# mit-han-lab/TinyChatEngine

Measured on AMD Instinct MI355X. Metric: decode tokens/s (W4A16 linears of one token, M=1) + GEMV GB/s vs HBM roofline, higher is better.
Workload: dtype int4 weights x fp16 activations, fp32 accumulate; 1 GPU; W4A16 decode GEMV M=1, llama3-8b (true shapes, model.h:83): 32 blocks x [qkv [4096, 1024, 1024], o 4096, gate/up 14336, down] + lm_head 128256, group 128; parallelism=single GPU, issue=one hipGraph replay per token (129 launches in stream order)

## Files before the change

include/tce_matmul.h:

```cpp
#ifndef TCE_MATMUL_H
#define TCE_MATMUL_H

#include <stddef.h>
#include <stdint.h>

#ifdef __cplusplus
extern "C" {
#endif

#define TCE_API __attribute__((visibility("default")))

#define TCE_VERSION 113

#define TCE_OK 0
#define TCE_ERR_BAD_ARG (-1)
#define TCE_ERR_UNSUPPORTED_GROUP (-2)
#define TCE_ERR_UNSUPPORTED_SHAPE (-3)
#define TCE_ERR_HIP (-4)
#define TCE_ERR_UNSUPPORTED_KIND (-5)
#define TCE_ERR_RCCL (-6)

#define TCE_W4A16_GEMV_MAX_M 8

typedef struct tce_w4a16_desc {
// ... 103 lines not shown
                                                int v_scale_log2, void *stream);
TCE_API int tce_attention_prefill_paged_fp8(const void *qkv, int ld_qkv, void *k_pool, void *v_pool, const int32_t *block_table, int table_rows, int table_stride,
                                            int page_keys, int num_pages, const void *cos_table, const void *sin_table, int causal, void *out, int ld_out, void *workspace,
                                            int heads, int kv_heads, int head_dim, const tce_prefill_segment *segments, int num_segments, int total_rows,
                                            unsigned short alpha_half_bits, int k_scale_log2, int v_scale_log2, void *stream);
TCE_API int tce_kv_pages_scatter_fp8(const void *k_src, const void *v_src, void *k_pool, void *v_pool, const int32_t *table_row, int table_stride, int page_keys,
                                     int num_pages, int kv_heads, int head_dim, int src_max_keys, int key0, int nkeys, int k_scale_log2, int v_scale_log2, void *stream);
TCE_API int tce_kv_pages_gather_fp8(const void *k_pool, const void *v_pool, void *k_dst, void *v_dst, const int32_t *table_row, int table_stride, int page_keys,
                                    int num_pages, int kv_heads, int head_dim, int dst_max_keys, int key0, int nkeys, int k_scale_log2, int v_scale_log2, void *stream);

#define TCE_SPEC_MAX_ROWS 8
TCE_API int tce_attention_decode_step_paged_rows_f16(const void *qkv, void *k_pool, void *v_pool, const int32_t *block_table, int table_stride, int page_keys, int num_pages,
                                                     const void *cos_table, const void *sin_table, void *out, void *workspace, int batch, int rows_per_seq, int heads,
                                                     int kv_heads, int head_dim, const int32_t *pos_device, int pos_bound, unsigned short alpha_half_bits, void *stream);
TCE_API int tce_attention_decode_step_paged_rows_fp8(const void *qkv, void *k_pool, void *v_pool, const int32_t *block_table, int table_stride, int page_keys, int num_pages,
                                                     const void *cos_table, const void *sin_table, void *out, void *workspace, int batch, int rows_per_seq, int heads,
                                                     int kv_heads, int head_dim, const int32_t *pos_device, int pos_bound, unsigned short alpha_half_bits, int k_scale_log2,
                                                     int v_scale_log2, void *stream);

typedef struct tce_sample_row {
    float temp;
    int32_t top_k;
    float top_p;
    float repeat_penalty;
    float alpha_frequency, alpha_presence;
    int32_t repeat_last_n;
    int32_t max_new;
    uint32_t seed_lo, seed_hi;
    uint32_t generated;
    uint32_t ring_pushed;
    int32_t ring[64];
} tce_sample_row;
typedef struct tce_sample_debug {
    int32_t n, k;
    float u;
    int32_t choice;
    int32_t ids[256];
    float logit[256], p[256], final_p[256];
} tce_sample_debug;
typedef struct tce_sample_call {
    const void *logits;
    int32_t ld, vocab, batch, top_k_bound;
    tce_sample_row *rows;
    int32_t *pos_device;
    int32_t pos_bound, log_stride;
    int32_t *next_token;
    int32_t *out_log;
    const float *uniform_override;
    tce_sample_debug *debug;
    void *workspace;
    int32_t stop_ids[4];
    int32_t n_stop, mirostat;
    float tfs_z, typical_p;
} tce_sample_call;
TCE_API size_t tce_sample_workspace_bytes(int batch, int vocab);
TCE_API int tce_sample_f16(const tce_sample_call *call, void *stream);
typedef struct tce_sample_verify_call {
    tce_sample_call s;
    int32_t rows_per_seq, hist_stride;
    const int32_t *row_token, *row_pos;
    int32_t *history;
    int32_t *emitted;
} tce_sample_verify_call;
TCE_API size_t tce_sample_verify_workspace_bytes(int batch, int rows_per_seq, int vocab);
TCE_API int tce_sample_verify_f16(const tce_sample_verify_call *call, void *stream);
TCE_API int tce_draft_ngram(const int32_t *history, const int32_t *script, int hist_stride, const int32_t *pos_device, int pos_bound, int batch, int rows_per_seq, int ngram,
                            int32_t *row_token, int32_t *row_pos, void *stream);
TCE_API int tce_embed_rows_f16(const void *table, int vocab, int hidden, const int32_t *token, void *out, int batch, const int32_t *pos_device, int pos_bound,
                               void *workspace, void *stream);
TCE_API int tce_prefetch(const void *ptr, long long bytes, int workgroups, void *stream);
TCE_API int tce_add_half(const void *a, const void *b, void *c, long long n, void *stream);
TCE_API int tce_rmsnorm_half(const void *x, const float *gamma, void *out, int m, int n, float eps, void *stream);
TCE_API int tce_w4a16_forward_group_rmsnorm(const tce_w4a16_desc *descs, int count, const float *gamma, float eps, void *stream);
TCE_API int tce_silu_mul_half(void *a, const void *b, long long n, void *stream);

TCE_API int tce_w4a16_check_zero_point_8(const void *zeros, long long n_words);
TCE_API int tce_w4a16_check_zero_point_8_async(const void *zeros, long long n_words, int *verdict, void *stream);

TCE_API size_t tce_w4a16_prepack_bytes(int N, int K, int group_size);
TCE_API size_t tce_w4a16_gemm_scratch_bytes(void);
TCE_API int tce_w4a16_gemm_scratch_faults(const void *scratch, void *stream, uint32_t *faults);
TCE_API int tce_w4a16_prepack(const tce_w4a16_desc *d, void *packed, void *stream);

#define TCE_MAX_GROUP 4
TCE_API int tce_w4a16_forward_group(const tce_w4a16_desc *descs, int count, void *stream);
#define TCE_MAX_INDEPENDENT 8
TCE_API int tce_w4a16_forward_independent(const tce_w4a16_desc *descs, int count, int *launches, void *stream);
TCE_API int tce_w4a16_describe_independent(const tce_w4a16_desc *descs, int count, char *buf, int buf_len);

TCE_API int tce_w4a16_awq_fp16acc(int M, int N, int K, int group_size, const void *A, const void *qweight,
                                  const void *scales, void *C, void *stream);
TCE_API size_t tce_w4a16_awq_workspace_bytes(int N, int K, int group_size);
TCE_API int tce_w4a16_gemm_awq(int M, int N, int K, int group_size, const void *A, const void *qweight,
                               const void *scales, void *C, void *workspace, int repack, void *stream);

#define TCE_BIAS_NONE 0
#define TCE_BIAS_INT8 1
#define TCE_BIAS_FP32 2
#define TCE_OUT_INT8 0
#define TCE_OUT_FP32 1

typedef struct tce_w8a8_desc {
    int32_t M, N, K;
    int32_t batch;
    const void *A;
    const void *B;
    const void *bias;
    void *C;
    int64_t strideA, strideB, strideC;
    float alpha, beta;
    int32_t q_min, q_max;
    int32_t bias_kind, out_kind;
    int32_t b_per_row;
    int32_t accumulate;
    int32_t lda, ldb, ldc;
    int32_t reserved2;
} tce_w8a8_desc;

TCE_API int tce_w8a8_matmul(const tce_w8a8_desc *d, void *stream);
typedef struct tce_w8a8_desc_v2 {
    uint32_t struct_size;
    uint32_t reserved0;
    tce_w8a8_desc desc;
    void *scratch;
} tce_w8a8_desc_v2;
TCE_API int tce_w8a8_matmul_v2(const tce_w8a8_desc_v2 *d, void *stream);
TCE_API size_t tce_w8a8_scratch_bytes(void);

TCE_API int tce_opt_softmax_q(const float *scores, const float *mask, void *probs, int heads, int sq, int tgz, int ld_probs, void *stream);
TCE_API int tce_opt_kv_append(const void *k, const void *v, void *k_cache, void *vt_cache, int heads, int hd, int sq, int pos, int max_keys, void *stream);
TCE_API int tce_opt_attention_decode(const void *q, const void *k_new, const void *v_new, void *k_cache, void *vt_cache, const float *mask, void *out, int heads,
                                     int head_dim, int m, int pos, int max_keys, int ld, float alpha_qk, float alpha_pv, void *stream);

TCE_API int tce_layernorm_q(const float *x, const float *weight, const float *bias, void *out, int m, int n, void *stream);

TCE_API int tce_layernorm_q_w8a8_group(const float *x, const float *ln_weight, const float *ln_bias, int m, int k, const tce_w8a8_desc *linears,
                                       int count, void *ln_out, void *stream);

typedef struct tce_plan tce_plan;
TCE_API int tce_plan_create(const tce_w4a16_desc *descs, const int32_t *group_sizes, int n_launches, tce_plan **out);
#define TCE_PLAN_CHAINED 1
#define TCE_PLAN_TAGGED 2
#define TCE_PLAN_OVERLAPPED 4
#define TCE_PLAN_TUNED 8
#define TCE_PLAN_INDEPENDENT 16
TCE_API int tce_plan_create_ex(const tce_w4a16_desc *descs, const int32_t *group_sizes, int n_launches, int flags, tce_plan **out);
TCE_API int tce_plan_is_chained(const tce_plan *plan);
TCE_API int tce_plan_geometry(const tce_plan *plan, int *rows, int *depth, int *waves, int *workgroups);
TCE_API int tce_plan_launch_geometry(const tce_plan *plan, int launch, int *rows, int *waves_n, int *waves_k, int *depth);
TCE_API int tce_plan_status(tce_plan *plan);
TCE_API int tce_plan_launch(tce_plan *plan, void *stream);
TCE_API int tce_plan_n_launches(const tce_plan *plan);
TCE_API void tce_plan_destroy(tce_plan *plan);

typedef struct tce_comm tce_comm;
#define TCE_COMM_HANDLE_BYTES 64
#define TCE_COMM_MAX_RANKS 8
TCE_API int tce_w4a16_shard(const tce_w4a16_desc *full, int rank, int world, tce_w4a16_desc *shard);
TCE_API int tce_comm_create(int rank, int world, int max_vector_elems, int slots, tce_comm **out);
TCE_API int tce_comm_export(tce_comm *comm, void *handle_out );
TCE_API int tce_comm_connect(tce_comm *comm, const void *handles );
TCE_API int tce_comm_connect_local(tce_comm *comm, tce_comm *const *all_ranks );
TCE_API int tce_allgather_f16(tce_comm *comm, int slot, const void *src_slice, void *dst_full, int n_total, void *stream);
TCE_API int tce_w4a16_forward_independent_gather(const tce_w4a16_desc *descs, int count, int gathered, tce_comm *comm, int slot, void *dst_full, int *launches, void *stream);
#define TCE_RCCL_ID_BYTES 128
TCE_API int tce_comm_rccl_unique_id(void *id_out );
// ... 33 lines not shown
```

tinychatengine_amd/capi.py:

```python
from __future__ import annotations

import ctypes as C
import os

_PKG = os.path.dirname(os.path.abspath(__file__))
LIB_PATH = os.environ.get("TCE_LIB_PATH") or os.path.join(_PKG, "lib", "libtce_hip.so")

TCE_OK = 0
TCE_ERR_BAD_ARG = -1
TCE_ERR_UNSUPPORTED_GROUP = -2
TCE_ERR_UNSUPPORTED_SHAPE = -3
TCE_ERR_HIP = -4
TCE_ERR_UNSUPPORTED_KIND = -5
TCE_W4A16_GEMV_MAX_M = 8
TCE_MAX_GROUP = 4
TCE_W4_FORCE_GEMV = 1
TCE_W4_FORCE_GEMM = 2
TCE_W4_SILU_MUL_PAIRS = 8
TCE_W4_ADD_TO_C = 16
TCE_PLAN_CHAINED = 1
TCE_PLAN_TAGGED = 2
TCE_ABI_VERSION = 113
TCE_PLAN_OVERLAPPED = 4
TCE_PLAN_TUNED = 8
TCE_PLAN_INDEPENDENT = 16
TCE_W4_ZERO_POINT_IS_8 = 4
TCE_BIAS_NONE, TCE_BIAS_INT8, TCE_BIAS_FP32 = 0, 1, 2
TCE_OUT_INT8, TCE_OUT_FP32 = 0, 1

EXPORTS = [
    "tce_w4a16_forward", "tce_w4a16_residual_rmsnorm_workspace_bytes", "tce_w4a16_forward_residual_rmsnorm", "tce_w4a16_prepack_bytes", "tce_w4a16_prepack", "tce_w4a16_gemm_scratch_bytes", "tce_w4a16_gemm_scratch_faults", "tce_w4a16_describe_dispatch", "tce_w8a8_describe_dispatch", "tce_reset_last_error", "tce_bmm_f16t", "tce_rope_half", "tce_softmax_half", "tce_attention_decode_f16", "tce_attention_decode_workspace_bytes", "tce_attention_decode_describe", "tce_attention_decode_step_f16", "tce_attention_decode_step_gqa_f16", "tce_attention_decode_describe_gqa", "tce_attention_decode_step_pos_f16", "tce_attention_decode_batch_workspace_bytes", "tce_attention_decode_describe_batch", "tce_attention_decode_step_batch_f16", "tce_kv_pages_pool_bytes", "tce_attention_decode_describe_paged", "tce_attention_decode_step_paged_f16", "tce_kv_pages_scatter_f16", "tce_kv_pages_gather_f16", "tce_kv_block_table_check", "tce_attention_prefill_f16", "tce_attention_prefill_workspace_bytes", "tce_attention_prefill_paged_workspace_bytes", "tce_attention_prefill_paged_f16", "tce_attention_prefill_describe_paged", "tce_kv_pages_pool_bytes_fp8", "tce_attention_decode_step_paged_fp8", "tce_attention_prefill_paged_fp8", "tce_kv_pages_scatter_fp8", "tce_kv_pages_gather_fp8", "tce_sample_workspace_bytes", "tce_sample_f16", "tce_embed_rows_f16", "tce_attention_decode_step_paged_rows_f16", "tce_attention_decode_step_paged_rows_fp8", "tce_sample_verify_workspace_bytes", "tce_sample_verify_f16", "tce_draft_ngram", "tce_opt_attention_decode", "tce_prefetch", "tce_add_half", "tce_silu_mul_half", "tce_rmsnorm_half", "tce_w4a16_forward_group_rmsnorm", "tce_w4a16_forward_group", "tce_w4a16_forward_independent", "tce_w4a16_describe_independent", "tce_w4a16_forward_independent_gather", "tce_w4a16_check_zero_point_8", "tce_w4a16_awq_fp16acc", "tce_w4a16_awq_workspace_bytes",
    "tce_w4a16_gemm_awq", "tce_w4a16_shard", "tce_comm_create", "tce_comm_export", "tce_comm_connect", "tce_comm_connect_local", "tce_allgather_f16", "tce_comm_rccl_unique_id", "tce_comm_rccl_init", "tce_allgather_rows_workspace_bytes", "tce_allgather_rows_f16", "tce_comm_status", "tce_comm_set_timeout_ms", "tce_comm_reset", "tce_comm_device", "tce_comm_destroy", "tce_w8a8_matmul", "tce_opt_softmax_q", "tce_opt_kv_append", "tce_layernorm_q", "tce_layernorm_q_w8a8_group", "tce_plan_create", "tce_plan_create_ex", "tce_plan_is_chained", "tce_plan_geometry", "tce_plan_status", "tce_plan_launch_geometry", "tce_plan_launch", "tce_plan_n_launches",
    "tce_w4a16_forward_v2", "tce_w8a8_matmul_v2", "tce_w8a8_scratch_bytes", "tce_attention_decode_step_deferred_f16", "tce_w4a16_forward_deferred_attention", "tce_plan_destroy", "tce_version", "tce_last_error", "tce_build_info", "tce_w4a16_set_gemv_config", "tce_w4a16_set_gemv_i8",
    "tce_w4a16_set_gemm_config", "tce_w4a16_algorithmic_bytes", "tce_w4a16_gemv_variant", "tce_w4a16_gemm_variant",
    "tce_w4a16_set_debug_mode", "tce_attention_set_tuning", "tce_w8a8_set_tuning", "tce_w4a16_set_debug_buffer", "tce_w4a16_check_zero_point_8_async", "tce_host_alloc", "tce_host_free", "tce_malloc", "tce_free", "tce_memcpy", "tce_synchronize", "tce_device_count",
]


class W4A16Desc(C.Structure):
    _fields_ = [
        ("M", C.c_int32), ("N", C.c_int32), ("K", C.c_int32), ("group_size", C.c_int32),
        ("A", C.c_void_p), ("qweight", C.c_void_p), ("scales", C.c_void_p), ("zeros", C.c_void_p), ("C", C.c_void_p),
        ("lda", C.c_int32), ("ldc", C.c_int32), ("scales_stride", C.c_int32), ("zeros_stride", C.c_int32),
        ("flags", C.c_int32), ("reserved", C.c_int32),
        ("rmsnorm_gamma", C.c_void_p), ("rmsnorm_eps", C.c_float), ("reserved2", C.c_int32),
        ("prepacked", C.c_void_p), ("scratch", C.c_void_p),
    ]


class W8A8Desc(C.Structure):
    _fields_ = [
        ("M", C.c_int32), ("N", C.c_int32), ("K", C.c_int32), ("batch", C.c_int32),
        ("A", C.c_void_p), ("B", C.c_void_p), ("bias", C.c_void_p), ("C", C.c_void_p),
        ("strideA", C.c_int64), ("strideB", C.c_int64), ("strideC", C.c_int64),
        ("alpha", C.c_float), ("beta", C.c_float), ("q_min", C.c_int32), ("q_max", C.c_int32),
        ("bias_kind", C.c_int32), ("out_kind", C.c_int32), ("b_per_row", C.c_int32), ("accumulate", C.c_int32),
        ("lda", C.c_int32), ("ldb", C.c_int32), ("ldc", C.c_int32), ("reserved2", C.c_int32),
    ]


class AttnDeferred(C.Structure):
    _fields_ = [("slots", C.c_int32), ("chunk", C.c_int32), ("heads", C.c_int32), ("stride", C.c_int32), ("part", C.c_void_p)]


class W4A16DescV2(C.Structure):
    _fields_ = [("struct_size", C.c_uint32), ("reserved0", C.c_uint32), ("desc", W4A16Desc)]


class W8A8DescV2(C.Structure):
    _fields_ = [("struct_size", C.c_uint32), ("reserved0", C.c_uint32), ("desc", W8A8Desc), ("scratch", C.c_void_p)]


def w4a16_forward_v2(desc: W4A16Desc, stream: int | None, extra_zero_bytes: int = 0) -> int:
    buf = (C.c_ubyte * (C.sizeof(W4A16DescV2) + extra_zero_bytes))()
    v2 = W4A16DescV2.from_buffer(buf)
    v2.struct_size = C.sizeof(W4A16DescV2) + extra_zero_bytes
    v2.desc = desc
    return lib().tce_w4a16_forward_v2(C.byref(v2), C.c_void_p(stream or 0))


_w8a8_scratch: dict = {}


def w8a8_scratch(device) -> "torch.Tensor":
    import torch
    key = str(device)
    if key not in _w8a8_scratch:
        L = lib()
        L.tce_w8a8_scratch_bytes.restype = C.c_size_t
        _w8a8_scratch[key] = torch.zeros(int(L.tce_w8a8_scratch_bytes()), dtype=torch.uint8, device=device)
    return _w8a8_scratch[key]


def w8a8_matmul_v2(desc: W8A8Desc, stream: int | None, scratch_ptr: int | None = None) -> int:
    v2 = W8A8DescV2(struct_size=C.sizeof(W8A8DescV2), reserved0=0, desc=desc, scratch=scratch_ptr)
    return lib().tce_w8a8_matmul_v2(C.byref(v2), C.c_void_p(stream or 0))


TCE_SAMPLE_MAX_K = 256
TCE_SAMPLE_RING = 64


class SampleRow(C.Structure):
    _fields_ = [("temp", C.c_float), ("top_k", C.c_int32), ("top_p", C.c_float), ("repeat_penalty", C.c_float), ("alpha_frequency", C.c_float), ("alpha_presence", C.c_float),
                ("repeat_last_n", C.c_int32), ("max_new", C.c_int32), ("seed_lo", C.c_uint32), ("seed_hi", C.c_uint32), ("generated", C.c_uint32), ("ring_pushed", C.c_uint32),
                ("ring", C.c_int32 * 64)]


class SampleDebug(C.Structure):
    _fields_ = [("n", C.c_int32), ("k", C.c_int32), ("u", C.c_float), ("choice", C.c_int32), ("ids", C.c_int32 * 256), ("logit", C.c_float * 256), ("p", C.c_float * 256),
                ("final_p", C.c_float * 256)]


class SampleCall(C.Structure):
    _fields_ = [("logits", C.c_void_p), ("ld", C.c_int32), ("vocab", C.c_int32), ("batch", C.c_int32), ("top_k_bound", C.c_int32), ("rows", C.c_void_p), ("pos_device", C.c_void_p),
                ("pos_bound", C.c_int32), ("log_stride", C.c_int32), ("next_token", C.c_void_p), ("out_log", C.c_void_p), ("uniform_override", C.c_void_p), ("debug", C.c_void_p),
                ("workspace", C.c_void_p), ("stop_ids", C.c_int32 * 4), ("n_stop", C.c_int32), ("mirostat", C.c_int32), ("tfs_z", C.c_float), ("typical_p", C.c_float)]


def sample_f16(call: SampleCall, stream: int | None) -> int:
    return lib().tce_sample_f16(C.byref(call), C.c_void_p(stream or 0))


TCE_SPEC_MAX_ROWS = 8


class SampleVerifyCall(C.Structure):
    _fields_ = [("s", SampleCall), ("rows_per_seq", C.c_int32), ("hist_stride", C.c_int32), ("row_token", C.c_void_p), ("row_pos", C.c_void_p), ("history", C.c_void_p),
                ("emitted", C.c_void_p)]


def sample_verify_f16(call: SampleVerifyCall, stream: int | None) -> int:
    return lib().tce_sample_verify_f16(C.byref(call), C.c_void_p(stream or 0))


class TceError(RuntimeError):
    def __init__(self, code: int, msg: str):
        super().__init__(f"libtce_hip error {code}: {msg}")
        self.code = code


_lib = None


def lib() -> C.CDLL:
    global _lib
    if _lib is None:
        if not os.path.exists(LIB_PATH):
            raise RuntimeError(
                f"{LIB_PATH} is missing: build it with `python -m tinychatengine_amd.build` "
                "(hipcc, gfx950).  tinychatengine_amd has no CPU or PyTorch fallback."
            )
        try:
            import torch
        except ImportError:
            pass
        L = C.CDLL(LIB_PATH)
        L.tce_version.restype = C.c_int
        if int(L.tce_version()) != TCE_ABI_VERSION:
            raise RuntimeError(f"{LIB_PATH} reports ABI version {int(L.tce_version())}, this wrapper mirrors {TCE_ABI_VERSION} (include/tce_matmul.h: TCE_VERSION): rebuild with `python -m tinychatengine_amd.build`")
        L.tce_last_error.restype = C.c_char_p
        L.tce_build_info.restype = C.c_char_p
        L.tce_w4a16_forward.argtypes = [C.POINTER(W4A16Desc), C.c_void_p]
        L.tce_w4a16_forward_group.argtypes = [C.POINTER(W4A16Desc), C.c_int, C.c_void_p]
        L.tce_w4a16_forward_independent.argtypes = [C.POINTER(W4A16Desc), C.c_int, C.POINTER(C.c_int), C.c_void_p]
        L.tce_w4a16_describe_independent.argtypes = [C.POINTER(W4A16Desc), C.c_int, C.c_char_p, C.c_int]
        L.tce_w4a16_forward_independent_gather.argtypes = [C.POINTER(W4A16Desc), C.c_int, C.c_int, C.c_void_p, C.c_int, C.c_void_p, C.POINTER(C.c_int), C.c_void_p]
        L.tce_w4a16_prepack_bytes.argtypes = [C.c_int] * 3
        L.tce_w4a16_prepack_bytes.restype = C.c_size_t
        L.tce_w4a16_gemm_scratch_bytes.argtypes = []
        L.tce_w4a16_gemm_scratch_bytes.restype = C.c_size_t
        L.tce_w4a16_prepack.argtypes = [C.POINTER(W4A16Desc), C.c_void_p, C.c_void_p]
        L.tce_prefetch.argtypes = [C.c_void_p, C.c_longlong, C.c_int, C.c_void_p]
        L.tce_bmm_f16t.argtypes = [C.c_void_p, C.c_void_p, C.c_void_p, C.c_int, C.c_int, C.c_int, C.c_int, C.c_ushort, C.c_void_p]
        L.tce_rope_half.argtypes = [C.c_void_p] * 4 + [C.c_int] * 4 + [C.c_void_p]
        L.tce_softmax_half.argtypes = [C.c_void_p, C.c_void_p, C.c_longlong, C.c_int, C.c_void_p]
        L.tce_attention_decode_f16.argtypes = [C.c_void_p] * 5 + [C.c_int] * 3 + [C.c_ushort, C.c_void_p]
        L.tce_attention_decode_workspace_bytes.argtypes = [C.c_int] * 3
        L.tce_attention_decode_workspace_bytes.restype = C.c_size_t
        L.tce_attention_decode_describe.argtypes = [C.c_int, C.c_int, C.c_char_p, C.c_int]
        L.tce_attention_decode_step_f16.argtypes = [C.c_void_p] * 8 + [C.c_int] * 4 + [C.c_ushort, C.c_void_p]
        L.tce_attention_decode_step_gqa_f16.argtypes = [C.c_void_p] * 8 + [C.c_int] * 5 + [C.c_ushort, C.c_void_p]
        L.tce_attention_decode_step_pos_f16.argtypes = [C.c_void_p] * 8 + [C.c_int] * 4 + [C.c_void_p, C.c_int, C.c_ushort, C.c_void_p]
        L.tce_attention_decode_batch_workspace_bytes.argtypes = [C.c_int] * 4
        L.tce_attention_decode_batch_workspace_bytes.restype = C.c_size_t
        L.tce_attention_decode_describe_batch.argtypes = [C.c_int] * 4 + [C.c_char_p, C.c_int]
        L.tce_attention_decode_step_batch_f16.argtypes = [C.c_void_p] * 7 + [C.c_int] * 5 + [C.c_void_p, C.c_int, C.c_ushort, C.c_void_p]
        L.tce_kv_pages_pool_bytes.argtypes = [C.c_int] * 4
        L.tce_kv_pages_pool_bytes.restype = C.c_size_t
        L.tce_attention_decode_describe_paged.argtypes = [C.c_int] * 5 + [C.c_char_p, C.c_int]
        L.tce_attention_decode_step_paged_f16.argtypes = [C.c_void_p] * 4 + [C.c_int] * 3 + [C.c_void_p] * 4 + [C.c_int] * 4 + [C.c_void_p, C.c_int, C.c_ushort, C.c_void_p]
        L.tce_kv_pages_scatter_f16.argtypes = [C.c_void_p] * 5 + [C.c_int] * 8 + [C.c_void_p]
        L.tce_kv_pages_gather_f16.argtypes = [C.c_void_p] * 5 + [C.c_int] * 8 + [C.c_void_p]
        L.tce_kv_block_table_check.argtypes = [C.c_void_p] + [C.c_int] * 4 + [C.c_void_p, C.c_int, C.c_void_p, C.c_void_p]
        L.tce_kv_pages_pool_bytes_fp8.argtypes = [C.c_int] * 4
        L.tce_kv_pages_pool_bytes_fp8.restype = C.c_size_t
        L.tce_attention_decode_step_paged_fp8.argtypes = [C.c_void_p] * 4 + [C.c_int] * 3 + [C.c_void_p] * 4 + [C.c_int] * 4 + [C.c_void_p, C.c_int, C.c_ushort, C.c_int, C.c_int, C.c_void_p]
        L.tce_kv_pages_scatter_fp8.argtypes = [C.c_void_p] * 5 + [C.c_int] * 10 + [C.c_void_p]
        L.tce_kv_pages_gather_fp8.argtypes = [C.c_void_p] * 5 + [C.c_int] * 10 + [C.c_void_p]
        L.tce_attention_decode_step_deferred_f16.argtypes = [C.c_void_p] * 8 + [C.c_int] * 4 + [C.c_void_p, C.c_int, C.c_ushort, C.POINTER(AttnDeferred), C.c_void_p]
        L.tce_w4a16_forward_deferred_attention.argtypes = [C.POINTER(W4A16Desc), C.POINTER(AttnDeferred), C.c_void_p, C.c_int, C.c_void_p]
        L.tce_opt_attention_decode.argtypes = [C.c_void_p] * 7 + [C.c_int] * 6 + [C.c_float, C.c_float, C.c_void_p]
        L.tce_attention_prefill_workspace_bytes.restype = C.c_size_t
        L.tce_attention_prefill_workspace_bytes.argtypes = [C.c_int] * 3
        L.tce_attention_prefill_f16.argtypes = [C.c_void_p, C.c_int, C.c_void_p, C.c_void_p, C.c_void_p, C.c_void_p, C.c_void_p, C.c_int, C.c_int, C.c_void_p, C.c_int, C.c_void_p] + \
            [C.c_int] * 6 + [C.c_ushort, C.c_void_p]
        L.tce_attention_prefill_paged_workspace_bytes.restype = C.c_size_t
        L.tce_attention_prefill_paged_workspace_bytes.argtypes = [C.c_int] * 3
        L.tce_attention_prefill_paged_f16.argtypes = [C.c_void_p, C.c_int, C.c_void_p, C.c_void_p, C.c_void_p] + [C.c_int] * 4 + [C.c_void_p, C.c_void_p, C.c_int, C.c_void_p, C.c_int, C.c_void_p] + \
            [C.c_int] * 3 + [C.c_void_p, C.c_int, C.c_int, C.c_ushort, C.c_void_p]
        L.tce_attention_prefill_paged_fp8.argtypes = [C.c_void_p, C.c_int, C.c_void_p, C.c_void_p, C.c_void_p] + [C.c_int] * 4 + [C.c_void_p, C.c_void_p, C.c_int, C.c_void_p, C.c_int, C.c_void_p] + \
            [C.c_int] * 3 + [C.c_void_p, C.c_int, C.c_int, C.c_ushort, C.c_int, C.c_int, C.c_void_p]
        L.tce_attention_prefill_describe_paged.restype = C.c_char_p
        L.tce_attention_prefill_describe_paged.argtypes = [C.c_int, C.c_int, C.c_int, C.c_void_p, C.c_int]
        L.tce_sample_workspace_bytes.restype = C.c_size_t
        L.tce_sample_workspace_bytes.argtypes = [C.c_int, C.c_int]
        L.tce_sample_f16.argtypes = [C.POINTER(SampleCall), C.c_void_p]
        L.tce_attention_decode_step_paged_rows_f16.argtypes = [C.c_void_p] * 4 + [C.c_int] * 3 + [C.c_void_p] * 4 + [C.c_int] * 5 + [C.c_void_p, C.c_int, C.c_ushort, C.c_void_p]
        L.tce_attention_decode_step_paged_rows_fp8.argtypes = [C.c_void_p] * 4 + [C.c_int] * 3 + [C.c_void_p] * 4 + [C.c_int] * 5 + [C.c_void_p, C.c_int, C.c_ushort, C.c_int, C.c_int, C.c_void_p]
        L.tce_sample_verify_workspace_bytes.restype = C.c_size_t
        L.tce_sample_verify_workspace_bytes.argtypes = [C.c_int, C.c_int, C.c_int]
        L.tce_sample_verify_f16.argtypes = [C.POINTER(SampleVerifyCall), C.c_void_p]
        L.tce_draft_ngram.argtypes = [C.c_void_p, C.c_void_p, C.c_int, C.c_void_p, C.c_int, C.c_int, C.c_int, C.c_int, C.c_void_p, C.c_void_p, C.c_void_p]
        L.tce_embed_rows_f16.argtypes = [C.c_void_p, C.c_int, C.c_int, C.c_void_p, C.c_void_p, C.c_int, C.c_void_p, C.c_int, C.c_void_p, C.c_void_p]
        L.tce_attention_decode_describe_gqa.argtypes = [C.c_int, C.c_int, C.c_int, C.c_char_p, C.c_int]
        L.tce_add_half.argtypes = [C.c_void_p, C.c_void_p, C.c_void_p, C.c_longlong, C.c_void_p]
        L.tce_silu_mul_half.argtypes = [C.c_void_p, C.c_void_p, C.c_longlong, C.c_void_p]
        L.tce_rmsnorm_half.argtypes = [C.c_void_p, C.c_void_p, C.c_void_p, C.c_int, C.c_int, C.c_float, C.c_void_p]
        L.tce_w4a16_forward_group_rmsnorm.argtypes = [C.POINTER(W4A16Desc), C.c_int, C.c_void_p, C.c_float, C.c_void_p]
        L.tce_w4a16_check_zero_point_8.argtypes = [C.c_void_p, C.c_longlong]
        L.tce_w4a16_awq_fp16acc.argtypes = [C.c_int] * 4 + [C.c_void_p] * 5
        L.tce_w4a16_awq_workspace_bytes.argtypes = [C.c_int] * 3
        L.tce_w4a16_awq_workspace_bytes.restype = C.c_size_t
        L.tce_w4a16_gemm_awq.argtypes = [C.c_int] * 4 + [C.c_void_p] * 5 + [C.c_int, C.c_void_p]
        L.tce_w8a8_matmul.argtypes = [C.POINTER(W8A8Desc), C.c_void_p]
        L.tce_opt_softmax_q.argtypes = [C.c_void_p, C.c_void_p, C.c_void_p, C.c_int, C.c_int, C.c_int, C.c_int, C.c_void_p]
        L.tce_opt_kv_append.argtypes = [C.c_void_p] * 4 + [C.c_int] * 5 + [C.c_void_p]
        L.tce_w4a16_shard.argtypes = [C.POINTER(W4A16Desc), C.c_int, C.c_int, C.POINTER(W4A16Desc)]
        L.tce_comm_create.argtypes = [C.c_int, C.c_int, C.c_int, C.c_int, C.POINTER(C.c_void_p)]
        L.tce_comm_export.argtypes = [C.c_void_p, C.c_void_p]
        L.tce_comm_connect.argtypes = [C.c_void_p, C.c_void_p]
        L.tce_comm_connect_local.argtypes = [C.c_void_p, C.POINTER(C.c_void_p)]
        L.tce_allgather_f16.argtypes = [C.c_void_p, C.c_int, C.c_void_p, C.c_void_p, C.c_int, C.c_void_p]
        L.tce_comm_status.argtypes = [C.c_void_p]
        L.tce_comm_set_timeout_ms.argtypes = [C.c_void_p, C.c_int]
        L.tce_comm_reset.argtypes = [C.c_void_p]
        L.tce_comm_device.argtypes = [C.c_void_p]
        L.tce_comm_destroy.argtypes = [C.c_void_p]
        L.tce_comm_destroy.restype = None
        L.tce_layernorm_q.argtypes = [C.c_void_p, C.c_void_p, C.c_void_p, C.c_void_p, C.c_int, C.c_int, C.c_void_p]
        L.tce_layernorm_q_w8a8_group.argtypes = [C.c_void_p, C.c_void_p, C.c_void_p, C.c_int, C.c_int, C.POINTER(W8A8Desc), C.c_int, C.c_void_p, C.c_void_p]
        L.tce_plan_create.argtypes = [C.POINTER(W4A16Desc), C.POINTER(C.c_int32), C.c_int, C.POINTER(C.c_void_p)]
        L.tce_plan_create_ex.argtypes = [C.POINTER(W4A16Desc), C.POINTER(C.c_int32), C.c_int, C.c_int, C.POINTER(C.c_void_p)]
        L.tce_plan_is_chained.argtypes = [C.c_void_p]
        L.tce_plan_status.argtypes = [C.c_void_p]
# ... 285 lines not shown
```

tinychatengine_amd/csrc/tce_capi.hip:

```cpp
#include <hip/hip_runtime.h>

#include <cstdarg>
#include <cstdio>
#include <cstring>
#include <new>
#include <algorithm>
#include <string>
#include <vector>

#include "tce_common.hpp"
#include "w4a16_kernels.hpp"

namespace tce {
int launch_w8a8(const tce_w8a8_desc &d, hipStream_t stream, hipError_t *hip_err, void *scratch = nullptr, char *describe = nullptr, int describe_len = 0);
size_t w8a8_scratch_bytes();
void set_w8a8_xsplit(int xs);
int sample_chunks(int vocab);
size_t sample_workspace_bytes(int batch, int vocab);
int launch_sample_f16(const tce_sample_call &c, hipStream_t stream, hipError_t *hip_err);
int launch_embed_rows_f16(const void *table, int vocab, int hidden, const int32_t *token, void *out, int batch, const int32_t *pos, int pos_bound, void *workspace,
                          hipStream_t stream, hipError_t *hip_err);
size_t sample_verify_workspace_bytes(int batch, int rows_per_seq, int vocab);
int launch_sample_verify_f16(const tce_sample_verify_call &v, hipStream_t stream, hipError_t *hip_err);
int launch_draft_ngram(const int32_t *history, const int32_t *script, int hist_stride, const int32_t *pos, int pos_bound, int batch, int rows_per_seq, int ngram,
                       int32_t *row_token, int32_t *row_pos, hipStream_t stream, hipError_t *hip_err);
}

namespace {

thread_local char g_err[512] = "";
thread_local int g_gemv_rows = 0, g_gemv_wn = 0, g_gemv_wk = 0, g_gemv_depth = 0;
thread_local int g_gemm_mt = 0, g_gemm_nt = 0;
thread_local int g_debug_mode_capi = 0;
void *g_dbg_buf_capi = nullptr;

int fail(int code, const char *fmt, ...) __attribute__((format(printf, 2, 3)));
int fail(int code, const char *fmt, ...) {
    va_list ap;
    va_start(ap, fmt);
    vsnprintf(g_err, sizeof(g_err), fmt, ap);
    va_end(ap);
    return code;
}

int hip_fail(hipError_t e, const char *what) {
    return fail(TCE_ERR_HIP, "%s: %s", what, hipGetErrorString(e));
}

int check_w4a16(const tce_w4a16_desc *d) {
    if (!d) return fail(TCE_ERR_BAD_ARG, "null descriptor");
    if (!d->A || !d->qweight || !d->scales || !d->zeros || !d->C) return fail(TCE_ERR_BAD_ARG, "null data pointer");
    if (d->M <= 0 || d->N <= 0 || d->K <= 0) return fail(TCE_ERR_BAD_ARG, "non-positive M/N/K (%d,%d,%d)", d->M, d->N, d->K);
    if (d->group_size != 128 && d->group_size != 64 && d->group_size != 32)
        return fail(TCE_ERR_UNSUPPORTED_GROUP, "Unsupported group size: %d", d->group_size);
    if (d->K % d->group_size != 0 || d->K % 32 != 0)
        return fail(TCE_ERR_UNSUPPORTED_SHAPE, "K=%d must be a multiple of the group size and of 32", d->K);
    const int lda = d->lda ? d->lda : d->K;
    if (lda % 8 != 0 || reinterpret_cast<uintptr_t>(d->A) % 16 != 0)
        return fail(TCE_ERR_UNSUPPORTED_SHAPE, "A must be 16-byte aligned with lda %% 8 == 0");
    if (reinterpret_cast<uintptr_t>(d->qweight) % 16 != 0) return fail(TCE_ERR_UNSUPPORTED_SHAPE, "qweight must be 16-byte aligned");
    if (d->flags & TCE_W4_SILU_MUL_PAIRS) {
        if (d->N % 2 != 0) return fail(TCE_ERR_UNSUPPORTED_SHAPE, "TCE_W4_SILU_MUL_PAIRS needs an even N (interleaved gate/up rows), got %d", d->N);
        if (d->flags & (TCE_W4_ADD_TO_C | TCE_W4_FORCE_GEMM)) return fail(TCE_ERR_BAD_ARG, "TCE_W4_SILU_MUL_PAIRS cannot be combined with ADD_TO_C / FORCE_GEMM");
    }
    if (d->rmsnorm_gamma && (d->flags & TCE_W4_FORCE_GEMM)) return fail(TCE_ERR_BAD_ARG, "rmsnorm_gamma cannot be combined with TCE_W4_FORCE_GEMM");
    return TCE_OK;
}

}

extern "C" {

int tce_version(void) { return TCE_VERSION; }
const char *tce_last_error(void) { return g_err; }
const char *tce_build_info(void) { return "tce_hip gfx950 wave64 hipcc " __VERSION__; }

int64_t tce_w4a16_algorithmic_bytes(int M, int N, int K, int G) {
    const int64_t nk = (int64_t)N * K;
    return nk / 2 + 2 * nk / G + nk / (2 * (int64_t)G) + 2 * (int64_t)M * K + 2 * (int64_t)M * N;
}

thread_local int g_pk_mode = 0;
constexpr int kPkMinM = 129;

static bool use_pk(const tce_w4a16_desc *d, bool want_gemm) {
    if (!d->prepacked || g_pk_mode == 9 || !want_gemm || d->K % 128 != 0 || d->rmsnorm_gamma) return false;
    if (g_pk_mode >= 1 && g_pk_mode <= 8) return true;
    if (d->M < kPkMinM || g_gemm_mt != 0) return false;
    if (d->flags & TCE_W4_SILU_MUL_PAIRS) return true;
    if (d->group_size != 128) return true;
    const bool has_scratch = d->scratch != nullptr && (reinterpret_cast<uintptr_t>(d->scratch) & 255) == 0;
    return tce::gemm_pk_estimate_us(d->M, d->N, d->K, nullptr, has_scratch, nullptr, d->group_size, (d->flags & TCE_W4_ZERO_POINT_IS_8) != 0) < tce::gemm_dma_estimate_us(d->M, d->N, d->K) + 1.5f;
}

constexpr long long kPersistentMinWeights = 1LL << 62;
constexpr long long kFusedNormPersistentRows = 16384;
thread_local int g_gemv_kernel = 0;
thread_local int g_skinny_enabled = 1;

int tce_w4a16_set_gemv_config(int rows, int wn, int wk, int depth) {
    if (rows == 0 && wn == 0 && wk == 0) {
        g_gemv_rows = g_gemv_wn = g_gemv_wk = g_gemv_depth = 0;
        g_gemv_kernel = 0;
        tce::set_gemv_stream_config(0, 0, 0);
        return TCE_OK;
    }
    if (wk == 0) {
        if ((rows % 10 != 0 && rows % 10 != 1 && rows % 10 != 2 && rows % 10 != 4) || rows < 0 || rows >= 90 || wn < 1 || wn > 16 || (depth != 0 && depth != 2 && depth != 3))
            return fail(TCE_ERR_BAD_ARG, "stream GEMV config rows=%d waves=%d depth=%d is not available", rows, wn, depth);
        tce::set_gemv_stream_config(rows, wn, depth);
        g_gemv_kernel = 2;
        return TCE_OK;
    }
    const int dd = depth ? depth : 2;
    if (!tce::gemv_variant_exists(rows, wn, wk, dd))
        return fail(TCE_ERR_BAD_ARG, "GEMV variant rows=%d wn=%d wk=%d depth=%d was not compiled", rows, wn, wk, dd);
    g_gemv_rows = rows;
    g_gemv_wn = wn;
    g_gemv_wk = wk;
    g_gemv_depth = dd;
    g_gemv_kernel = 1;
    return TCE_OK;
}

int tce_w4a16_set_gemv_i8(int mode, int rows) {
    if (mode < 0 || mode > 1 || rows < 0 || rows > 2) return fail(TCE_ERR_BAD_ARG, "tce_w4a16_set_gemv_i8: mode %d rows %d", mode, rows);
    tce::set_gemv_i8_mode(mode, rows);
    return TCE_OK;
}

int tce_attention_set_tuning(int waves_per_workgroup, int workgroups, int heads_per_workgroup) {
    const bool ok = (waves_per_workgroup == 0 || waves_per_workgroup == 4 || waves_per_workgroup == 8 || waves_per_workgroup == 16) &&
                    (workgroups == 0 || (workgroups >= 32 && workgroups <= 8192)) &&
                    (heads_per_workgroup == 0 || heads_per_workgroup == 1 || heads_per_workgroup == 2 || heads_per_workgroup == 4);
    if (!ok) return fail(TCE_ERR_BAD_ARG, "tce_attention_set_tuning(%d, %d, %d)", waves_per_workgroup, workgroups, heads_per_workgroup);
    tce::set_attention_fast_waves(waves_per_workgroup);
    tce::set_attention_fast_target(workgroups);
    tce::set_attention_fast_fuse(heads_per_workgroup);
    return TCE_OK;
}

int tce_w8a8_set_tuning(int quartets_per_tile, int big_tiles, int deep_pipeline) {
    const bool ok = (quartets_per_tile == 0 || quartets_per_tile == 1 || quartets_per_tile == 2 || quartets_per_tile == 4) &&
                    ((big_tiles >= 0 && big_tiles <= 4) || big_tiles == 9) &&
                    (deep_pipeline == 0 || deep_pipeline == 1 || deep_pipeline == 2 || deep_pipeline == 4 || deep_pipeline == 9);
    if (!ok) return fail(TCE_ERR_BAD_ARG, "tce_w8a8_set_tuning(%d, %d, %d)", quartets_per_tile, big_tiles, deep_pipeline);
    tce::set_w8a8_ksplit(quartets_per_tile);
    tce::set_w8a8_big(big_tiles);
// ... 466 lines not shown
    if ((d->ldc && d->ldc != d->N)) return fail(TCE_ERR_UNSUPPORTED_SHAPE, "tce_w4a16_forward_residual_rmsnorm: the linear must produce the whole residual row (ldc = N)");
    if (!tce::gemv_i8_supports(d, 1)) return fail(TCE_ERR_UNSUPPORTED_SHAPE, "tce_w4a16_forward_residual_rmsnorm needs the packed copy (desc.prepacked, K %% 128 == 0, group 128): it lives in the int8-contraction kernel");
    hipError_t he = hipSuccess;
    const tce::I8ResidualNorm rn{gamma, eps, xn_out, workspace};
    const int rc = tce::launch_w4a16_gemv_i8(d, 1, static_cast<hipStream_t>(stream), &he, nullptr, 0.f, &rn);
    if (rc == TCE_ERR_HIP) return hip_fail(he, "w4a16 gemv (residual + next rmsnorm) launch");
    if (rc == TCE_ERR_UNSUPPORTED_SHAPE && d->K > 16384 && !(d->flags & TCE_W4_ZERO_POINT_IS_8) && d->N % 8 == 0 && d->N <= 16384 && d->group_size == 128) {
        const int rc1 = tce_w4a16_forward(d, stream);
        if (rc1 != TCE_OK) return rc1;
        return tce_rmsnorm_half(d->C, gamma, xn_out, 1, d->N, eps, stream);
    }
    if (rc != TCE_OK) return fail(rc, "tce_w4a16_forward_residual_rmsnorm: unsupported shape (group 128, N %% 8 == 0, N <= 16384)");
    return TCE_OK;
}

int tce_w4a16_forward(const tce_w4a16_desc *d, void *stream) {
    const int rc0 = check_w4a16(d);
    if (rc0 != TCE_OK) return rc0;
    const bool want_gemm = (d->flags & TCE_W4_FORCE_GEMM) ||
                           (d->M > TCE_W4A16_GEMV_MAX_M && !(d->flags & (TCE_W4_FORCE_GEMV | TCE_W4_SILU_MUL_PAIRS)));
    const bool pairs_on_pk = (d->flags & TCE_W4_SILU_MUL_PAIRS) && d->prepacked && d->M >= kPkMinM && !(d->flags & TCE_W4_FORCE_GEMV);
    hipError_t he = hipSuccess;
    if (use_pk(d, want_gemm || pairs_on_pk)) {
        const int rc = tce::launch_w4a16_gemm_pk(*d, d->prepacked, static_cast<hipStream_t>(stream), &he);
        if (rc == TCE_OK) return TCE_OK;
        if (rc == TCE_ERR_HIP) return hip_fail(he, "w4a16 gemm (pre-packed) launch");
        if (rc != TCE_ERR_UNSUPPORTED_SHAPE) return fail(rc, "w4a16 gemm (pre-packed): unsupported configuration");
    }
    if (g_gemv_kernel == 0 && g_debug_mode_capi == 0 && tce::gemv_i8_supports(d, 1)) return tce_w4a16_forward_group(d, 1, stream);
    if (g_skinny_enabled && !(d->flags & (TCE_W4_FORCE_GEMV | TCE_W4_FORCE_GEMM)) && tce::skinny_supports(*d)) {
        const int rc = tce::launch_w4a16_skinny(*d, static_cast<hipStream_t>(stream), &he);
        if (rc == TCE_OK) return TCE_OK;
        if (rc == TCE_ERR_HIP) return hip_fail(he, "w4a16 skinny launch");
        if (rc != TCE_ERR_UNSUPPORTED_SHAPE) return fail(rc, "w4a16 skinny: unsupported configuration");
    }
    if (d->rmsnorm_gamma && d->M != 1) return fail(TCE_ERR_UNSUPPORTED_SHAPE, "the fused RMSNorm prologue is a decode (M = 1) path; use tce_rmsnorm_half for M = %d", d->M);
    if (want_gemm && d->K % 128 == 0 && d->group_size != 128 && d->M > 16 && g_gemm_mt == 0) {
        const int rc = tce::launch_w4a16_gemm_dma(*d, 0, 0, static_cast<hipStream_t>(stream), &he);
        if (rc == TCE_OK) return TCE_OK;
        if (rc == TCE_ERR_HIP) return hip_fail(he, "w4a16 gemm (dma) launch");
        if (rc != TCE_ERR_UNSUPPORTED_SHAPE) return fail(rc, "w4a16 gemm (dma): no kernel variant for this config");
    }
    if (want_gemm && d->K % 128 == 0 && d->group_size == 128) {
        if (g_gemm_mt >= 200 || g_gemm_mt == 0) {
            const int rc = tce::launch_w4a16_gemm_dma(*d, g_gemm_mt ? g_gemm_mt - 200 : 0, g_gemm_mt ? g_gemm_nt : 0, static_cast<hipStream_t>(stream), &he);
            if (rc == TCE_OK) return TCE_OK;
            if (rc == TCE_ERR_HIP) return hip_fail(he, "w4a16 gemm (dma) launch");
            if (rc != TCE_ERR_UNSUPPORTED_SHAPE) return fail(rc, "w4a16 gemm (dma): no kernel variant for this config");
        }
        const int rc = tce::launch_w4a16_gemm(*d, g_gemm_mt >= 200 ? g_gemm_mt - 200 : g_gemm_mt, g_gemm_nt, static_cast<hipStream_t>(stream), &he);
        if (rc == TCE_ERR_HIP) return hip_fail(he, "w4a16 gemm launch");
        if (rc != TCE_OK) return fail(rc, "w4a16 gemm: no kernel variant for this shape/config");
        return TCE_OK;
    }
    return tce_w4a16_forward_group(d, 1, stream);
}

int tce_w4a16_describe_dispatch(const tce_w4a16_desc *d, char *buf, int buf_len) {
    if (!buf || buf_len <= 0) return fail(TCE_ERR_BAD_ARG, "tce_w4a16_describe_dispatch: no buffer");
    const int rc0 = check_w4a16(d);
    if (rc0 != TCE_OK) return rc0;
    const bool want_gemm = (d->flags & TCE_W4_FORCE_GEMM) ||
                           (d->M > TCE_W4A16_GEMV_MAX_M && !(d->flags & (TCE_W4_FORCE_GEMV | TCE_W4_SILU_MUL_PAIRS)));
    const bool pairs_on_pk = (d->flags & TCE_W4_SILU_MUL_PAIRS) && d->prepacked && d->M >= kPkMinM && !(d->flags & TCE_W4_FORCE_GEMV);
    if (use_pk(d, want_gemm || pairs_on_pk)) {
        int form = 1, split = 1;
        tce::gemm_pk_estimate_us(d->M, d->N, d->K, &form, d->scratch != nullptr && (reinterpret_cast<uintptr_t>(d->scratch) & 255) == 0, &split, d->group_size, (d->flags & TCE_W4_ZERO_POINT_IS_8) != 0);
        if (form == 15) std::snprintf(buf, (size_t)buf_len, "gemm-pk tile=128x512 wave=128x64 quartets=2-side-by-side group=%d", d->group_size);
        else if (form == 13 || form == 14) std::snprintf(buf, (size_t)buf_len, "gemm-pk tile=128x192 wave=128x48 quartets=%d group=%d", form - 12, d->group_size);
        else if (form == 10) std::snprintf(buf, (size_t)buf_len, "gemm-pk tile=128x256 wave=128x64 quartets=1 group=%d", d->group_size);
        else if (form == 11) std::snprintf(buf, (size_t)buf_len, "gemm-pk tile=128x256 wave=128x64 quartets=2 group=%d", d->group_size);
        else if (form == 12) std::snprintf(buf, (size_t)buf_len, "gemm-pk tile=128x256 wave=128x64 quartets=1 ksplit=%d group=%d", split, d->group_size);
        else if (form == 4) std::snprintf(buf, (size_t)buf_len, "gemm-pk tile=128x128 quartets=1 ksplit=%d group=%d", split, d->group_size);
        else if (form == 16) std::snprintf(buf, (size_t)buf_len, "gemm-pk tile=128x128 quartets=2 ksplit=2 group=%d", d->group_size);
        else if (form == 5) std::snprintf(buf, (size_t)buf_len, "gemm-pk tile=128x128 quartets=1 ksplit=%d-of-the-tiles-past-256 group=%d", split, d->group_size);
        else if (form == 6) std::snprintf(buf, (size_t)buf_len, "gemm-pk tile=256x128 quartets=1 group=%d", d->group_size);
        else if (form == 7) std::snprintf(buf, (size_t)buf_len, "gemm-pk tile=256x128 quartets=1 ksplit=%d group=%d", split, d->group_size);
        else if (form == 8) std::snprintf(buf, (size_t)buf_len, "gemm-pk tile=256x128 quartets=2 group=%d", d->group_size);
        else if (form == 9) std::snprintf(buf, (size_t)buf_len, "gemm-pk tile=256x256 quartets=2 group=%d", d->group_size);
        else std::snprintf(buf, (size_t)buf_len, "gemm-pk tile=128x%d quartets=%d group=%d", form == 3 ? 256 : 128, form == 1 ? 1 : 2, d->group_size);
        return TCE_OK;
    }
    if (g_gemv_kernel == 0 && g_debug_mode_capi == 0 && tce::gemv_i8_supports(d, 1)) {
        std::snprintf(buf, (size_t)buf_len, "gemv-i8 rows-per-pass=%d group=%d", tce::gemv_i8_rows_per_pass(d->M, d->K, d->group_size), d->group_size);
        return TCE_OK;
    }
    if (g_skinny_enabled && !(d->flags & (TCE_W4_FORCE_GEMV | TCE_W4_FORCE_GEMM)) && tce::skinny_supports(*d)) {
        std::snprintf(buf, (size_t)buf_len, "small-batch slices=%d", (d->M + 15) / 16);
        return TCE_OK;
    }
    if (want_gemm && d->K % 128 == 0 && (d->group_size == 128 || (d->M > 16 && g_gemm_mt == 0))) {
        if (g_gemm_mt == 0 || g_gemm_mt >= 200) {
            int mt = g_gemm_mt ? g_gemm_mt - 200 : 0, nt = g_gemm_nt, ks = 0;
            if (mt == 0) tce::gemm_dma_describe(d->M, d->N, d->group_size == 128, &mt, &nt, &ks);
            std::snprintf(buf, (size_t)buf_len, "gemm-dma tile=%dx%d quartets=%d group=%d", mt * 16, nt * 64, ks, d->group_size);
        } else {
            std::snprintf(buf, (size_t)buf_len, "gemm tile=%dx%d", (g_gemm_mt % 100) * 16, g_gemm_nt * 64);
        }
        return TCE_OK;
    }
    const bool persistent = g_gemv_kernel == 2 || (d->rmsnorm_gamma ? (g_gemv_kernel == 0 && d->N >= kFusedNormPersistentRows)
                                                                     : (g_gemv_kernel == 0 && d->M == 1 && (long long)d->N * d->K >= kPersistentMinWeights && g_debug_mode_capi == 0));
    std::snprintf(buf, (size_t)buf_len, "gemv passes=%d kernel=%s", (d->M + 3) / 4, persistent && d->M == 1 ? "persistent" : "row-block");
    return TCE_OK;
}

size_t tce_w4a16_prepack_bytes(int N, int K, int G) { return tce::prepack_bytes(N, K, G); }

size_t tce_w4a16_gemm_scratch_bytes(void) { return tce::gemm_pk_scratch_bytes(); }

int tce_w4a16_gemm_scratch_faults(const void *scratch, void *stream, uint32_t *faults) {
    if (!scratch || !faults) return fail(TCE_ERR_BAD_ARG, "tce_w4a16_gemm_scratch_faults: null argument");
    hipError_t e = hipStreamSynchronize(static_cast<hipStream_t>(stream));
    if (e != hipSuccess) return hip_fail(e, "hipStreamSynchronize");
    e = hipMemcpy(faults, static_cast<const unsigned char *>(scratch) + 4096 - 4, sizeof(uint32_t), hipMemcpyDeviceToHost);
    if (e != hipSuccess) return hip_fail(e, "hipMemcpy");
    return TCE_OK;
}

int tce_w4a16_prepack(const tce_w4a16_desc *d, void *packed, void *stream) {
    if (!d || !packed) return fail(TCE_ERR_BAD_ARG, "tce_w4a16_prepack: null argument");
    if (!d->qweight || !d->scales || !d->zeros || d->N <= 0 || d->K <= 0) return fail(TCE_ERR_BAD_ARG, "tce_w4a16_prepack: null weights / non-positive N, K");
    if (d->group_size != 128 && d->group_size != 64 && d->group_size != 32) return fail(TCE_ERR_UNSUPPORTED_GROUP, "Unsupported group size: %d", d->group_size);
    if (d->K % 128 != 0) return fail(TCE_ERR_UNSUPPORTED_SHAPE, "tce_w4a16_prepack: K=%d must be a multiple of 128", d->K);
    if (reinterpret_cast<uintptr_t>(packed) % 256 != 0) return fail(TCE_ERR_UNSUPPORTED_SHAPE, "tce_w4a16_prepack: the packed buffer must be 256-byte aligned");
    hipError_t he = hipSuccess;
    const int rc = tce::launch_w4a16_prepack(*d, packed, static_cast<hipStream_t>(stream), &he);
    if (rc == TCE_ERR_HIP) return hip_fail(he, "prepack launch");
    if (rc != TCE_OK) return fail(rc, "tce_w4a16_prepack: unsupported shape");
    return TCE_OK;
}

int tce_w4a16_check_zero_point_8(const void *zeros, long long n_words) {
    if (!zeros || n_words <= 0) return fail(TCE_ERR_BAD_ARG, "tce_w4a16_check_zero_point_8: bad argument");
    hipError_t he = hipSuccess;
    const int rc = tce::check_zero_point_8(zeros, n_words, &he);
    return rc == TCE_ERR_HIP ? hip_fail(he, "zero-point check") : rc;
}

int tce_w4a16_check_zero_point_8_async(const void *zeros, long long n_words, int *verdict, void *stream) {
    if (!zeros || n_words <= 0 || !verdict) return fail(TCE_ERR_BAD_ARG, "tce_w4a16_check_zero_point_8_async: bad argument");
    hipError_t he = hipSuccess;
    const int rc = tce::check_zero_point_8_async(zeros, n_words, verdict, static_cast<hipStream_t>(stream), &he);
    return rc == TCE_ERR_HIP ? hip_fail(he, "zero-point check (async)") : rc;
}

int tce_w4a16_awq_fp16acc(int M, int N, int K, int G, const void *A, const void *qweight, const void *scales, void *C,
                          void *stream) {
    if (!A || !qweight || !scales || !C || M <= 0 || N <= 0 || K <= 0) return fail(TCE_ERR_BAD_ARG, "bad argument");
    if (G <= 0 || K % G != 0 || N % 8 != 0) return fail(TCE_ERR_UNSUPPORTED_SHAPE, "need K %% G == 0 and N %% 8 == 0");
    hipError_t he = hipSuccess;
    const int rc = tce::launch_awq_fp16acc(M, N, K, G, A, qweight, scales, C, static_cast<hipStream_t>(stream), &he);
    return rc == TCE_ERR_HIP ? hip_fail(he, "awq fp16acc launch") : rc;
}

size_t tce_w4a16_awq_workspace_bytes(int N, int K, int G) {
    if (N <= 0 || K <= 0 || (G != 128 && G != 64 && G != 32)) return 0;
    const size_t zw = (size_t)tce::zeros_width(K, G);
    return (size_t)N * (K / 8) * 4 + (size_t)N * zw * 4 + (size_t)N * zw * 8 * 2;
}

int tce_w4a16_gemm_awq(int M, int N, int K, int G, const void *A, const void *qweight, const void *scales, void *C,
                       void *workspace, int repack, void *stream) {
    if (!A || !qweight || !scales || !C || !workspace || M <= 0 || N <= 0 || K <= 0) return fail(TCE_ERR_BAD_ARG, "bad argument");
    if (G != 128 && G != 64 && G != 32) return fail(TCE_ERR_UNSUPPORTED_GROUP, "Unsupported group size: %d", G);
    if (K % G != 0 || K % 32 != 0 || N % 8 != 0 || ((size_t)N * (K / 8)) % 4 != 0)
        return fail(TCE_ERR_UNSUPPORTED_SHAPE, "need K %% G == 0, K %% 32 == 0, N %% 8 == 0");
    hipError_t he = hipSuccess;
    if (repack) {
        const int rc = tce::launch_awq_repack(N, K, G, qweight, scales, workspace, static_cast<hipStream_t>(stream), &he);
        if (rc != TCE_OK) return rc == TCE_ERR_HIP ? hip_fail(he, "awq repack launch") : rc;
    }
    const int zw = tce::zeros_width(K, G);
    tce_w4a16_desc d;
    std::memset(&d, 0, sizeof(d));
    d.M = M;
    d.N = N;
    d.K = K;
    d.group_size = G;
    d.A = A;
    d.qweight = workspace;
    d.zeros = static_cast<const unsigned *>(workspace) + (size_t)N * (K / 8);
    d.scales = static_cast<const unsigned *>(d.zeros) + (size_t)N * zw;
    d.C = C;
    return tce_w4a16_forward(&d, stream);
}

int tce_layernorm_q(const float *x, const float *weight, const float *bias, void *out, int m, int n, void *stream) {
    if (!x || !weight || !bias || !out || m <= 0 || n <= 0) return fail(TCE_ERR_BAD_ARG, "tce_layernorm_q: bad argument");
    if (n % 4 != 0 || n > 8192 || reinterpret_cast<uintptr_t>(x) % 16 != 0)
        return fail(TCE_ERR_UNSUPPORTED_SHAPE, "tce_layernorm_q: n %% 4 == 0, n <= 8192 and x 16-byte aligned");
    hipError_t he = hipSuccess;
    const int rc = tce::launch_layernorm_q(x, weight, bias, out, m, n, static_cast<hipStream_t>(stream), &he);
    return rc == TCE_ERR_HIP ? hip_fail(he, "layernorm_q launch") : rc;
}

int tce_opt_softmax_q(const float *scores, const float *mask, void *probs, int heads, int sq, int tgz, int ld_probs, void *stream) {
    if (!scores || !mask || !probs || heads <= 0 || sq <= 0 || tgz <= 0) return fail(TCE_ERR_BAD_ARG, "tce_opt_softmax_q: bad argument");
    if (ld_probs == 0) ld_probs = tgz;
    if (ld_probs < tgz) return fail(TCE_ERR_BAD_ARG, "tce_opt_softmax_q: ld_probs < tgz");
    if (tgz > 8000) return fail(TCE_ERR_UNSUPPORTED_SHAPE, "tce_opt_softmax_q: rows of at most 8192 keys (five rows in LDS per workgroup)");
    hipError_t he = hipSuccess;
    const int rc = tce::launch_opt_softmax_q(scores, mask, probs, heads, sq, tgz, ld_probs, static_cast<hipStream_t>(stream), &he);
    return rc == TCE_ERR_HIP ? hip_fail(he, "opt softmax launch") : rc;
}

int tce_opt_kv_append(const void *k, const void *v, void *k_cache, void *vt_cache, int heads, int hd, int sq, int pos, int max_keys, void *stream) {
    if (!k || !v || !k_cache || !vt_cache || heads <= 0 || hd <= 0 || sq <= 0 || pos < 0 || pos + sq > max_keys)
        return fail(TCE_ERR_BAD_ARG, "tce_opt_kv_append: bad argument (need pos + sq <= max_keys)");
    hipError_t he = hipSuccess;
    const int rc = tce::launch_opt_kv_append(k, v, k_cache, vt_cache, heads, hd, sq, pos, max_keys, static_cast<hipStream_t>(stream), &he);
    return rc == TCE_ERR_HIP ? hip_fail(he, "opt kv append launch") : rc;
// ... 1162 lines not shown
```

tinychatengine_amd/csrc/w4a16_gemm_pk.hip:

```cpp
#include "tce_common.hpp"
#include "w4a16_kernels.hpp"
#include "w4a16_mfma_layout.hpp"

namespace tce {

namespace {

struct PrepackArgs {
    const unsigned *qweight;
    const half_t *scales;
    const unsigned *zeros;
    unsigned *words;
    uint2_t *consts;
    float *last;
    half_t *dscales;
    unsigned *dzeros;
    int N, K, log2g, scales_stride, zeros_stride;
};

__global__ __launch_bounds__(64) void prepack_words_kernel(const PrepackArgs a) {
    const int jt = blockIdx.x, kb = blockIdx.y, lane = threadIdx.x;
    const int q = lane >> 4, n16 = lane & 15;
    const int n = jt * 16 + n16;
    const bool live = n < a.N;
// ... 932 lines not shown
template <int LG, int ABL = 0>
hipError_t launch_pkw(PkGemmArgs &g, hipStream_t stream) {
    const size_t lds = (size_t)4 * pk::kHalfBytes;
    auto kfn = w4a16_gemm_pkw_kernel<LG, ABL>;
    hipError_t e = hipFuncSetAttribute(reinterpret_cast<const void *>(kfn), hipFuncAttributeMaxDynamicSharedMemorySize, (int)lds);
    if (e != hipSuccess) return e;
    const int per = 8 * g.m_per * g.n_per;
    hipLaunchKernelGGL(kfn, dim3(g.split_s > 1 ? per + (per - 8 * g.full_slots) * (g.split_s - 1) : per), dim3(256), lds, stream, g);
    return hipGetLastError();
}
template <int LG, int ABL = 0>
hipError_t launch_pkwx2(PkGemmArgs &g, hipStream_t stream) {
    const size_t lds = (size_t)2 * 4 * pk::kHalfBytes;
    auto kfn = w4a16_gemm_pkwx2_kernel<LG, ABL>;
    hipError_t e = hipFuncSetAttribute(reinterpret_cast<const void *>(kfn), hipFuncAttributeMaxDynamicSharedMemorySize, (int)lds);
    if (e != hipSuccess) return e;
    hipLaunchKernelGGL(kfn, dim3(8 * g.m_per * g.n_per), dim3(512), lds, stream, g);
    return hipGetLastError();
}

hipError_t launch_pkw512(PkGemmArgs &g, hipStream_t stream) {
    const size_t lds = (size_t)128 * 512 * 2;
    auto kfn = w4a16_gemm_pkw512_kernel<7, 0>;
    hipError_t e = hipFuncSetAttribute(reinterpret_cast<const void *>(kfn), hipFuncAttributeMaxDynamicSharedMemorySize, (int)lds);
    if (e != hipSuccess) return e;
    hipLaunchKernelGGL(kfn, dim3(8 * g.m_per * g.n_per), dim3(512), lds, stream, g);
    return hipGetLastError();
}

template <int KS>
hipError_t launch_pkw3(PkGemmArgs &g, hipStream_t stream) {
    const size_t lds = (size_t)KS * 4 * pk::kHalfBytes;
    hipError_t e;
    if constexpr (KS == 2) {
        auto kfn = w4a16_gemm_pkw3x2_kernel<7, 0>;
        e = hipFuncSetAttribute(reinterpret_cast<const void *>(kfn), hipFuncAttributeMaxDynamicSharedMemorySize, (int)lds);
        if (e != hipSuccess) return e;
        hipLaunchKernelGGL(kfn, dim3(8 * g.m_per * g.n_per), dim3(512), lds, stream, g);
    } else {
        auto kfn = w4a16_gemm_pkw3_kernel<7, 0>;
        e = hipFuncSetAttribute(reinterpret_cast<const void *>(kfn), hipFuncAttributeMaxDynamicSharedMemorySize, (int)lds);
        if (e != hipSuccess) return e;
        hipLaunchKernelGGL(kfn, dim3(8 * g.m_per * g.n_per), dim3(256), lds, stream, g);
    }
    return hipGetLastError();
}

template <int LG, int ABL = 0>
hipError_t launch_pk256(PkGemmArgs &g, hipStream_t stream) {
    const size_t lds = (size_t)4 * 256 * pk::kHalfK * 2;
    auto kfn = w4a16_gemm_pk256_kernel<LG, ABL>;
    hipError_t e = hipFuncSetAttribute(reinterpret_cast<const void *>(kfn), hipFuncAttributeMaxDynamicSharedMemorySize, (int)lds);
    if (e != hipSuccess) return e;
    const int per = 8 * g.m_per * g.n_per;
    hipLaunchKernelGGL(kfn, dim3(g.split_s > 1 ? per + (per - 8 * g.full_slots) * (g.split_s - 1) : per), dim3(256), lds, stream, g);
    return hipGetLastError();
}

}

#ifdef TCE_LAB
void set_gemm_pk_ablation(int abl) { g_pk_abl = abl; }
#else
void set_gemm_pk_ablation(int) { g_pk_abl = 0; }
#endif
void set_gemm_pk256_auto(int on) { g_pk256_auto = on ? 1 : 0; }
void set_gemm_pk_wide_auto(int on) { g_pk_wide_auto = on ? 1 : 0; }
void set_gemm_pk_form16_auto(int on) { g_pk_form16_auto = on ? 1 : 0; }
void set_gemm_pk_handoff(int on) { g_pk_handoff = on ? 1 : 0; }
void set_gemm_pk_prio(int on) { g_pk_prio = on >= 0 && on <= 4 ? on : -1; }
void set_gemm_pk_handoff_delta(int d) { g_pk_handoff_delta = d >= 0 && d <= 8 ? d : 2; }
void set_gemm_pk_split(int s) { g_pk_split_force = s >= 2 && s <= 4 ? s : 0; }

void set_gemm_pk_mode(int form, int xm) {
    g_pk_ks = (form >= 1 && form <= 16) ? form : 0;
    g_pk_xm = (xm == 1 || xm == 2 || xm == 4 || xm == 8) ? xm : 0;
}

size_t prepack_bytes(int N, int K, int G) {
    if (N <= 0 || K <= 0 || K % 128 != 0 || (G != 128 && G != 64 && G != 32)) return 0;
    return pk::total_bytes(N, K, G);
}

int launch_w4a16_prepack(const tce_w4a16_desc &d, void *out, hipStream_t stream, hipError_t *hip_err) {
    if (d.K % 128 != 0) return TCE_ERR_UNSUPPORTED_SHAPE;
    const int zw = zeros_width(d.K, d.group_size);
    PrepackArgs a{};
    a.qweight = static_cast<const unsigned *>(d.qweight);
    a.scales = static_cast<const half_t *>(d.scales);
    a.zeros = static_cast<const unsigned *>(d.zeros);
    unsigned char *base = static_cast<unsigned char *>(out);
    a.words = reinterpret_cast<unsigned *>(base);
    a.consts = reinterpret_cast<uint2_t *>(base + pk::consts_offset(d.N, d.K));
    a.last = reinterpret_cast<float *>(base + pk::last_offset(d.N, d.K, d.group_size));
    a.dscales = reinterpret_cast<half_t *>(base + pk::dscales_offset(d.N, d.K, d.group_size));
    a.dzeros = reinterpret_cast<unsigned *>(base + pk::dzeros_offset(d.N, d.K, d.group_size));
    a.N = d.N;
    a.K = d.K;
    a.log2g = d.group_size == 128 ? 7 : (d.group_size == 64 ? 6 : 5);
    a.scales_stride = d.scales_stride ? d.scales_stride : zw * 8;
    a.zeros_stride = d.zeros_stride ? d.zeros_stride : zw;
    const int nt = pk::nt16(d.N);
    hipLaunchKernelGGL(prepack_words_kernel, dim3(nt, d.K >> 7), dim3(64), 0, stream, a);
    hipLaunchKernelGGL(prepack_consts_kernel, dim3((nt * 16 + 63) / 64), dim3(64), 0, stream, a);
    hipLaunchKernelGGL(prepack_decode_kernel, dim3((unsigned)(((long long)nt * (d.K / d.group_size) + 63) / 64)), dim3(64), 0, stream, a);
    const hipError_t e = hipGetLastError();
    if (e != hipSuccess) {
        if (hip_err) *hip_err = e;
        return TCE_ERR_HIP;
    }
    return TCE_OK;
}

constexpr int kPkSplitMaxUnits = 512;

size_t gemm_pk_scratch_bytes() { return 4096 + (size_t)kPkSplitMaxUnits * 65536; }

static int pk_split_factor(long tiles1, int nkb, bool has_scratch, float *cost_out) {
    int best_s = 1;
    float best = 1e30f;
    if (has_scratch && tiles1 <= 1024)
        for (int s = 2; s <= 4; ++s) {
            if (tiles1 * s > kPkSplitMaxUnits || nkb / s < 4 || (g_pk_split_force && s != g_pk_split_force)) continue;
            const float run = (float)((nkb + s - 1) / s);
            float c = (tiles1 * s <= 256 ? run * 1.06f : 1.8f * run + 1.5f) + 8.0f + 1.3f * (float)s;
            if (s == 2 && g_pk_handoff && nkb >= 6) c = (tiles1 * s <= 256 ? (run + 1.f) * 1.06f : 1.8f * (run + 1.f) + 1.5f) + 3.0f + kPkHandoffUs;
            if (c < best) best = c, best_s = s;
        }
    if (cost_out) *cost_out = best;
    return best_s;
}

float gemm_pk_estimate_us(int M, int N, int K, int *form_out, bool has_scratch, int *split_out, int group_size, bool zero_point_8) {
    const long mt = (M + 127) / 128;
    const long tiles1 = mt * ((N + 127) / 128), tiles3 = mt * ((N + 255) / 256);
    const float nkb = (float)(K / 128);
    auto rounds = [](long tiles, long slots) {
        const float r = (float)tiles / (float)slots;
        return r <= 3.f ? (float)(int)(r + 0.999f) : r + 0.5f;
    };
    auto load = [](long waves) { return waves >= 2048 ? 1.0f : (float)waves / 2048.f; };
    const float cost1 = (tiles1 <= 256 ? nkb * 1.06f : 0.5f * rounds(tiles1, 256) * nkb * (1.25f + 0.73f * load(tiles1 * 4))) + 3.0f;
    const float cost2 = rounds(tiles1, 256) * (nkb * 0.5f) * (1.7f + 0.4f * load(tiles1 * 8)) + 3.0f;
    const float cost3 = rounds(tiles3, 256) * nkb * (1.5f + 0.4f * load(tiles3 * 8)) + 3.0f;
    float cost4 = 1e30f;
    int split = pk_split_factor(tiles1, (int)nkb, has_scratch, &cost4);
    float cost5 = 1e30f;
    int split5 = 1;
    if (has_scratch && tiles1 > 256 && tiles1 <= 256 + kPkSplitMaxUnits / 2) {
        const long tail = tiles1 - 256;
        for (int s5 = 2; s5 <= 4; ++s5) {
            if ((tail + 7) / 8 * 8 * s5 > 256 || (int)nkb / s5 < 4 || (g_pk_split_force && s5 != g_pk_split_force)) continue;
            const float run = (float)(((int)nkb + s5 - 1) / s5);
            const float c = run * 1.9f + (nkb - run) * 1.06f + 4.0f;
            if (c < cost5) cost5 = c, split5 = s5;
        }
    }
    int form = 1;
    float best = cost1;
    if (cost2 < best) best = cost2, form = 2;
    if (cost3 < best) best = cost3, form = 3;
    if (cost4 < best) best = cost4, form = 4;
    if (cost5 < best) best = cost5, form = 5;
    const long mt6 = (M + 255) / 256;
    const long tiles6 = mt6 * ((N + 127) / 128);
    float cost6 = 1e30f, cost7 = 1e30f;
    int split7 = 1;
    if (M > 128 && group_size == 128) {
        cost6 = rounds(tiles6, 256) * nkb * kPk256UsPerKBlock + 4.0f;
        if (has_scratch)
            for (int s7 = 2; s7 <= 4; ++s7) {
                if (tiles6 * s7 * 2 > kPkSplitMaxUnits || (int)nkb / s7 < 4 || (g_pk_split_force && s7 != g_pk_split_force)) continue;
                const float run = (float)(((int)nkb + s7 - 1) / s7);
                const float c = rounds(tiles6 * s7, 256) * run * kPk256UsPerKBlock + 9.0f + 2.0f * (float)s7;
                if (c < cost7) cost7 = c, split7 = s7;
            }
    }
    float cost9 = 1e30f;
    const long tiles9 = mt6 * ((N + 255) / 256);
    if (M > 128 && group_size == 128) cost9 = rounds(tiles9, 256) * nkb * kPk256wUsPerKBlock + 5.0f;
    float cost8 = 1e30f;
    if (M > 128 && group_size == 128 && nkb >= 2.f && ((int)nkb & 1) == 0) cost8 = rounds(tiles6, 256) * (float)(((int)nkb + 1) / 2) * kPk256x2UsPerPair + 5.0f;
    if (g_pk256_auto && cost8 < best) best = cost8, form = 8;
    const long tilesw = mt * ((N + 255) / 256);
    float cost10 = 1e30f, cost11 = 1e30f, cost12 = 1e30f;
    int split12 = 1;
    if (M > 128 && group_size == 128 && zero_point_8) {
        cost10 = (tilesw <= 256 ? nkb * kPkWideAloneUs : 0.5f * rounds(tilesw, 256) * nkb * kPkWidePairUs) + 3.5f;
        if (((int)nkb & 1) == 0 && nkb >= 2.f) cost11 = rounds(tilesw, 256) * (nkb * 0.5f) * kPkWideX2PairUs + 4.5f;
        if (has_scratch)
            for (int s = 2; s <= 4; ++s) {
                if (tilesw * s * 2 > kPkSplitMaxUnits || (int)nkb / s < 4 || (g_pk_split_force && s != g_pk_split_force)) continue;
                const float run = (float)(((int)nkb + s - 1) / s);
                const float c = (tilesw * s <= 256 ? run * kPkWideAloneUs : 0.5f * rounds(tilesw * s, 256) * run * kPkWidePairUs) + 9.0f + 2.0f * (float)s;
                if (c < cost12) cost12 = c, split12 = s;
            }
    }
    const long tilesw3 = mt * ((N + 191) / 192);
    float cost13 = 1e30f, cost14 = 1e30f;
    if (M > 128 && group_size == 128 && zero_point_8) {
        cost13 = (tilesw3 <= 256 ? nkb * kPkWideAloneUs : 0.5f * rounds(tilesw3, 256) * nkb * kPkWidePairUs) * 0.78f + 3.5f;
        if (((int)nkb & 1) == 0 && nkb >= 2.f) cost14 = rounds(tilesw3, 256) * (nkb * 0.5f) * kPkWideX2PairUs * 0.78f + 4.5f;
    }
    const long tilesw512 = mt * ((N + 511) / 512);
    float cost15 = 1e30f;
    if (M > 128 && group_size == 128 && zero_point_8) cost15 = rounds(tilesw512, 256) * nkb * kPkWide512Us + 5.0f;
    if (g_pk_wide_auto) {
        if (cost15 < best) best = cost15, form = 15;
        if (cost13 < best) best = cost13, form = 13;
        if (cost14 < best) best = cost14, form = 14;
        if (cost10 < best) best = cost10, form = 10;
        if (cost11 < best) best = cost11, form = 11;
        if (cost12 < best) best = cost12, form = 12;
    }
    float cost16 = 1e30f;
    if (has_scratch && tiles1 * 2 <= 256 && nkb >= 8.f && g_pk_handoff && group_size == 128)
        cost16 = (float)(((int)nkb / 2 + 1 + 1) / 2) * (1.7f + 0.4f * load(tiles1 * 2 * 8)) + 3.0f + kPkHandoffUs + kPk16ExtraUs;
    if (g_pk_form16_auto && cost16 < best) best = cost16, form = 16;
    if (g_pk_ks) {
        form = g_pk_ks;
        if (form == 16 && cost16 > 1e29f) form = 2;
        if (form == 4 && split == 1) form = split5 > 1 ? 5 : 1;
        if (form == 7 && split7 == 1) form = 6;
        if ((form >= 6 && form <= 9) && (M <= 128 || group_size != 128)) form = 1;
        if (form == 8 && (nkb < 2.f || ((int)nkb & 1))) form = 6;
        if (form >= 10 && form <= 15 && (M <= 128 || group_size != 128 || !zero_point_8)) form = 1;
        if (form == 11 && (nkb < 2.f || ((int)nkb & 1))) form = 10;
        if (form == 12 && split12 == 1) form = 10;
        if (form == 14 && (nkb < 2.f || ((int)nkb & 1))) form = 13;
        if (form == 16) best = cost16;
        else if (form >= 10) best = form == 10 ? cost10 : (form == 11 ? cost11 : (form == 12 ? cost12 : (form == 13 ? cost13 : (form == 14 ? cost14 : cost15))));
        else
        best = form == 1 ? cost1 : (form == 2 ? cost2 : (form == 3 ? cost3 : (form == 4 ? cost4 : (form == 5 ? cost5 : (form == 6 ? cost6 : (form == 7 ? cost7 : (form == 8 ? cost8 : cost9)))))));
    }
    if (form_out) *form_out = form;
    if (split_out) *split_out = form == 4 ? split : (form == 5 ? split5 : (form == 7 ? split7 : (form == 12 ? split12 : (form == 16 ? 2 : 1))));
    return best;
}

int launch_w4a16_gemm_pk(const tce_w4a16_desc &d, const void *packed, hipStream_t stream, hipError_t *hip_err) {
    if (d.K % 128 != 0 || !packed) return TCE_ERR_UNSUPPORTED_SHAPE;
    const int lda = d.lda ? d.lda : d.K;
    if ((lda * 2) % 16 != 0 || (reinterpret_cast<uintptr_t>(d.A) & 15)) return TCE_ERR_UNSUPPORTED_SHAPE;
    if ((unsigned long long)d.M * (unsigned long long)lda * 2ull >= (1ull << 32)) return TCE_ERR_UNSUPPORTED_SHAPE;
    PkGemmArgs g{};
    const unsigned char *base = static_cast<const unsigned char *>(packed);
    g.A = static_cast<const half_t *>(d.A);
    g.words = reinterpret_cast<const uint4_t *>(base);
    g.consts = reinterpret_cast<const uint2_t *>(base + pk::consts_offset(d.N, d.K));
    g.C = static_cast<half_t *>(d.C);
    g.M = d.M;
    g.N = d.N;
    g.K = d.K;
    g.lda = lda;
    g.pairs = (d.flags & TCE_W4_SILU_MUL_PAIRS) ? 1 : 0;
    g.ldc = d.ldc ? d.ldc : (g.pairs ? d.N / 2 : d.N);
    g.add_to_c = (d.flags & TCE_W4_ADD_TO_C) ? 1 : 0;
    int form = 1, split = 1;
    const bool has_scratch = d.scratch != nullptr && (reinterpret_cast<uintptr_t>(d.scratch) & 255) == 0;
    gemm_pk_estimate_us(d.M, d.N, d.K, &form, has_scratch, &split, d.group_size, (d.flags & TCE_W4_ZERO_POINT_IS_8) != 0);
    const bool cut_tail_only = form == 5;
    const bool rows256 = form >= 6 && form <= 9;
    const bool rows256x2 = form == 8, rows256w = form == 9;
    const bool two_quartets_cut = form == 16;
    const bool wide = form >= 10 && form <= 15, widex2 = form == 11, wide3 = form == 13 || form == 14, wide512 = form == 15;
    const bool handoff_form = (form == 4 || form == 16) && split == 2 && g_pk_handoff;
    g.prio = g_pk_prio >= 0 ? g_pk_prio : ((form == 10 || form == 12) ? 1 : 0);
    if (form == 4 || form == 5 || form == 7 || form == 12 || form == 16) {
        form = two_quartets_cut ? 2 : 1;
        g.split_s = split;
        g.handoff = handoff_form ? 1 + g_pk_handoff_delta : 0;
        g.counters = static_cast<unsigned *>(d.scratch);
        g.partials = reinterpret_cast<float4_t *>(static_cast<unsigned char *>(d.scratch) + 4096);
    } else {
        g.split_s = 1;
    }
    const int bn = wide512 ? 512 : (wide3 ? 192 : ((form == 3 || form == 9 || wide) ? 256 : 128));
    g.n_blocks = (d.N + bn - 1) / bn;
    g.m_blocks = rows256 ? (d.M + 255) / 256 : (d.M + 127) / 128;
    int best_xm = 1;
    long best_grid = -1;
    for (int xm = 8; xm >= 1; xm >>= 1) {
        const long grid = 8L * ((g.m_blocks + xm - 1) / xm) * ((g.n_blocks + 8 / xm - 1) / (8 / xm));
        if (best_grid < 0 || grid < best_grid) {
            best_grid = grid;
            best_xm = xm;
        }
    }
    g.xm = g_pk_xm ? g_pk_xm : best_xm;
    g.m_per = (g.m_blocks + g.xm - 1) / g.xm;
    g.n_per = (g.n_blocks + 8 / g.xm - 1) / (8 / g.xm);
    if (g.split_s > 1) {
        g.full_slots = cut_tail_only ? 32 : 0;
        const int cut_wgs = 8 * (g.m_per * g.n_per - g.full_slots);
        if (cut_wgs <= 0 || (long)cut_wgs * g.split_s * ((rows256 || wide) ? 2 : 1) > kPkSplitMaxUnits || cut_wgs > 1024) g.split_s = 1;
    }
    const int ks = form;
    hipError_t e;
    const int lg = d.group_size == 128 ? 7 : (d.group_size == 64 ? 6 : 5);
#ifdef TCE_LAB
    if (wide && lg == 7 && g_pk_abl && !widex2 && !wide3 && !wide512) {
        switch (g_pk_abl) {
#define TCE_ABL(X) case X: e = launch_pkw<7, X>(g, stream); break;
            TCE_ABL(1) TCE_ABL(2) TCE_ABL(4) TCE_ABL(8) TCE_ABL(16) TCE_ABL(32) TCE_ABL(7) TCE_ABL(55) TCE_ABL(128) TCE_ABL(256)
#undef TCE_ABL
            default: return TCE_ERR_BAD_ARG;
        }
        if (e != hipSuccess) {
            if (hip_err) *hip_err = e;
            return TCE_ERR_HIP;
        }
        return TCE_OK;
    }
#endif
#ifdef TCE_LAB
    if (g_pk_abl && lg == 7 && !rows256 && !wide) {
        switch (g_pk_abl) {
#define TCE_ABL(X) case X: e = launch_pk<1, 7, X>(g, stream); break;
            TCE_ABL(1) TCE_ABL(2) TCE_ABL(4) TCE_ABL(8) TCE_ABL(16) TCE_ABL(32) TCE_ABL(6) TCE_ABL(7) TCE_ABL(23) TCE_ABL(55) TCE_ABL(47) TCE_ABL(48) TCE_ABL(64)
#undef TCE_ABL
            default: return TCE_ERR_BAD_ARG;
        }
        if (e != hipSuccess) {
            if (hip_err) *hip_err = e;
            return TCE_ERR_HIP;
        }
        return TCE_OK;
    }
#endif
    if (wide512) e = launch_pkw512(g, stream);
    else if (wide3) e = form == 14 ? launch_pkw3<2>(g, stream) : launch_pkw3<1>(g, stream);
    else if (wide) e = widex2 ? launch_pkwx2<7>(g, stream) : launch_pkw<7>(g, stream);
// ... 25 lines not shown
```

tinychatengine_amd/csrc/w4a16_gemv_i8.hip:

```cpp
#include "tce_common.hpp"
#include "w4a16_kernels.hpp"
#include "w4a16_mfma_layout.hpp"

namespace tce {

namespace {

struct I8SegHead {
    const void *words;
    const half_t *dscales;
    int bytes_w, bytes_s, N;
    int block_begin;
};
struct I8SegRest {
    half_t *C;
    const unsigned *dzeros;
    int ldc, epilogue, bytes_z, pad_;
};
struct I8Tail {
    I8SegRest rest[TCE_MAX_GROUP];
    I8SegHead head[TCE_MAX_GROUP - 1];
    const float *gamma;
    float eps;
    float out_eps;
    const float *out_gamma;
    half_t *xn_out;
    float *ws;
    const float *comb_part;
    const int *comb_pos_dev;
    int comb_pos, comb_slots, comb_chunk, comb_stride, comb_heads;
    unsigned long long *dbg;
};

struct I8Stamps {
    unsigned long long t[7];
};

struct I8Seg {
    const void *words;
    const half_t *dscales;
    const unsigned *dzeros;
    half_t *C;
    int N, ldc, epilogue;
    int bytes_w, bytes_s, bytes_z;
    int block_begin;
};

constexpr int kI8MixMax = 8;
struct I8MixSeg {
    const half_t *A;
    int lda, K;
    I8Seg seg;
};
struct I8MixArgs {
    int nseg, M;
    const float *gamma = nullptr;
    float eps = 0.f;
    const float *out_gamma = nullptr;
    float out_eps = 0.f;
    half_t *xn_out = nullptr;
    float *ws = nullptr;
    const float *comb_part = nullptr;
    const int *comb_pos_dev = nullptr;
    int comb_pos = 0, comb_slots = 0, comb_chunk = 0, comb_stride = 0, comb_heads = 0;
    int g_seg = -1;
    unsigned g_tiles = 0;
    PeerGatherEpi g;
    I8MixSeg s[kI8MixMax];
};

template <int DPP_CTRL, int ROW_MASK = 0xF>
__device__ __forceinline__ unsigned dpp_max_u32(unsigned v) {
    const unsigned t = (unsigned)__builtin_amdgcn_update_dpp(0, (int)v, DPP_CTRL, ROW_MASK, 0xF, false);
    return v > t ? v : t;
}
template <int DPP_CTRL>
__device__ __forceinline__ float dpp_add_f32(float v) {
    const int t = __builtin_amdgcn_update_dpp(0, __builtin_bit_cast(int, v), DPP_CTRL, 0xF, 0xF, false);
    return v + __builtin_bit_cast(float, t);
}

template <typename T>
__device__ __forceinline__ void keep_scalar(T &v) {
    asm volatile("" : "+s"(v));
}

template <int MB, int GPU, int ROWS, int UW, bool Z8, bool NORM, bool RNORM, int COMB, bool MIX, typename ARGS, bool STAMPS = false>
__device__ __forceinline__ void w4a16_gemv_i8_body(const ARGS &args, unsigned char *smem, int tid, const int WK, const int U, const int K_, const int lda_, int M_, const half_t *A_,
                                                   I8Seg seg, const int tile0, const bool gathers, const unsigned g_epoch, I8Stamps *st = nullptr) {
    static_assert(!MIX || (MB == 1 && GPU == 1 && ROWS == 1 && UW == 8 && !NORM && !RNORM && !COMB), "the mixed launch: one decode row, groups of 128, one tile per wave group");
    static_assert(!COMB || (MB == 1 && ROWS == 1 && GPU == 1 && UW == 8 && !NORM && !RNORM), "the deferred-attention prologue: one decode row, groups of 128, K a multiple of 1024");
    static_assert(MB * GPU <= 4, "sixteen output columns: rows x groups-per-unit x 4 planes");
    static_assert(!RNORM || (MB == 1 && ROWS == 1 && !NORM), "the residual + next-norm epilogue: one decode row, one tile per workgroup");
    static_assert(!NORM || MB == 1, "the fused RMSNorm prologue is a decode (M = 1) feature");
    constexpr int UPP = 4 / (MB * GPU);
    static_assert(UW % UPP == 0 && UW % 4 == 0, "whole passes; whole 16-byte x loads per lane");
    constexpr int NP = UW / UPP;
    constexpr int XC = UW / 4;
    constexpr int SPG = 4 / GPU;
    const int NG = U * GPU;
    const int lane = tid & 63;
    const int wk = __builtin_amdgcn_readfirstlane(tid >> 6);
    const int u0 = wk * UW;
    const int kq = lane >> 4, j = lane & 15;
    const int m0 = blockIdx.y * MB;
    const int ntiles = (seg.N + 15) >> 4;
    auto tile_of = [&](int r) { return tile0 + r < ntiles ? tile0 + r : ntiles - 1; };

    const __amdgpu_buffer_rsrc_t rs_w = __builtin_amdgcn_make_buffer_rsrc(const_cast<void *>(seg.words), 0, seg.bytes_w, 0x00020000);
    const __amdgpu_buffer_rsrc_t rs_s = __builtin_amdgcn_make_buffer_rsrc(const_cast<half_t *>(seg.dscales), 0, seg.bytes_s, 0x00020000);
    const __amdgpu_buffer_rsrc_t rs_z = __builtin_amdgcn_make_buffer_rsrc(const_cast<unsigned *>(seg.dzeros), 0, seg.bytes_z, 0x00020000);
    const __amdgpu_buffer_rsrc_t rs_none = __builtin_amdgcn_make_buffer_rsrc(const_cast<void *>(seg.words), 0, 0, 0x00020000);

    const int p_l = j & 3;
    const int m_l = (j >> 2) % MB;
    const int gi_l = ((j >> 2) / MB) % GPU;
    const int uu_l = (j >> 2) / (MB * GPU);

    uint4_t xv[MB][XC];
    int nact = 1;
    if constexpr (COMB) {
        const int pos = args.comb_pos_dev ? __builtin_amdgcn_readfirstlane(*args.comb_pos_dev) : args.comb_pos;
        nact = (pos + args.comb_chunk) / args.comb_chunk;
        nact = nact < args.comb_slots ? nact : args.comb_slots;
    }
    constexpr int kSlots = COMB ? COMB : 1;
    uint2_t cml[COMB ? XC : 1][kSlots];
    uint4_t co[COMB ? XC : 1][kSlots][2];
    if constexpr (COMB) {
        if (nact > 1) {
            const __amdgpu_buffer_rsrc_t rs_p = __builtin_amdgcn_make_buffer_rsrc(const_cast<float *>(args.comb_part), 0, args.comb_heads * args.comb_slots * args.comb_stride * 4, 0x00020000);
#pragma unroll
            for (int c = 0; c < XC; ++c) {
                const int kpos = u0 * 128 + (lane + 64 * c) * 8;
                const int hbase = ((kpos >> 7) * args.comb_slots) * args.comb_stride * 4 + (kpos & 127) * 4;
#pragma unroll
                for (int i = 0; i < kSlots; ++i) {
                    const int ii = i < nact ? i : 0;
                    const unsigned char *src = reinterpret_cast<const unsigned char *>(args.comb_part) + hbase + ii * args.comb_stride * 4;
                    cml[c][i] = *reinterpret_cast<const uint2_t *>(src - (kpos & 127) * 4);
                    co[c][i][0] = *reinterpret_cast<const uint4_t *>(src + 16);
                    co[c][i][1] = *reinterpret_cast<const uint4_t *>(src + 32);
                }
                (void)rs_p;
            }
        }
    }
#pragma unroll
    for (int m = 0; m < MB; ++m) {
        if (COMB && nact > 1) break;
        int mrow = m0 + m;
        mrow = mrow < M_ ? mrow : M_ - 1;
        const __amdgpu_buffer_rsrc_t rs_x = __builtin_amdgcn_make_buffer_rsrc(const_cast<half_t *>(A_ + (size_t)mrow * lda_), 0, K_ * 2, 0x00020000);
#pragma unroll
        for (int c = 0; c < XC; ++c) xv[m][c] = __builtin_amdgcn_raw_buffer_load_b128(rs_x, u0 * 256 + (lane + 64 * c) * 16, 0, 0);
    }
    float4_t gm[NORM ? XC : 1][2];
    if constexpr (NORM) {
        const __amdgpu_buffer_rsrc_t rs_g = __builtin_amdgcn_make_buffer_rsrc(const_cast<float *>(args.gamma), 0, K_ * 4, 0x00020000);
#pragma unroll
        for (int c = 0; c < XC; ++c) {
            gm[c][0] = __builtin_bit_cast(float4_t, __builtin_amdgcn_raw_buffer_load_b128(rs_g, u0 * 512 + (lane + 64 * c) * 32, 0, 0));
            gm[c][1] = __builtin_bit_cast(float4_t, __builtin_amdgcn_raw_buffer_load_b128(rs_g, u0 * 512 + (lane + 64 * c) * 32 + 16, 0, 0));
        }
    }
    uint2_t sc[ROWS][NP];
    unsigned zq[ROWS][(NP + 1) / 2];
#pragma unroll
    for (int r = 0; r < ROWS; ++r)
#pragma unroll
        for (int ps = 0; ps < NP; ++ps) {
            const int g = (ps * UPP + uu_l) * GPU + gi_l;
// ... 61 lines not shown
        const int nc = pieces >= 1024 ? 16 : (pieces + 63) >> 6;
        if (pieces <= 1024 && (pieces & 63) == 0) {
            const float *sl = slots + lane;
            for (int c = 0; c < nc; ++c) tot += sl[c * 64];
        } else {
            for (int c = 0; c < nc; ++c) {
                const int q = c * 64 + lane;
                float slot = 0.f;
                slot += q < pieces ? slots[q] : 0.f;
                if (q + 1024 < pieces) slot += slots[q + 1024];
                tot += slot;
            }
        }
        tot = wave_sum_dpp_lane63(tot);
        tot = __builtin_bit_cast(float, __builtin_amdgcn_readlane(__builtin_bit_cast(int, tot), 63));
        const float rs = 1.0f / sqrtf(tot / (float)K_ + args.eps);
#pragma unroll
        for (int c = 0; c < XC; ++c) {
            const half8_t v = __builtin_bit_cast(half8_t, xv[0][c]);
            half8_t y;
#pragma unroll
            for (int e = 0; e < 8; ++e) {
                const float f = ((float)v[e] * rs) * (e < 4 ? gm[c][0][e] : gm[c][1][e - 4]);
                y[e] = (half_t)__builtin_amdgcn_fmed3f(f, -(65504.f - 1000.f), 65504.f - 1000.f);
            }
            xv[0][c] = __builtin_bit_cast(uint4_t, y);
        }
    }
    int sh[MB];
    bool bad[MB];
#pragma unroll
    for (int m = 0; m < MB; ++m) {
        unsigned mx = 0;
#pragma unroll
        for (int c = 0; c < XC; ++c)
#pragma unroll
            for (int q = 0; q < 4; ++q) {
                const unsigned v = xv[m][c][q] & 0x7FFF7FFFu;
                const unsigned v2 = v << 16;
                const unsigned m2 = v > v2 ? v : v2;
                mx = mx > m2 ? mx : m2;
            }
        mx = dpp_max_u32<0x111>(mx);
        mx = dpp_max_u32<0x112>(mx);
        mx = dpp_max_u32<0x114>(mx);
        mx = dpp_max_u32<0x118>(mx);
        mx = dpp_max_u32<0x142, 0xA>(mx);
        mx = dpp_max_u32<0x143, 0xC>(mx);
        const int E = (int)((unsigned)__builtin_amdgcn_readlane((int)mx, 63) >> 26);
        bad[m] = E == 31;
        sh[m] = 44 - E;
        const float scale = __builtin_bit_cast(float, (unsigned)(127 + sh[m]) << 23);
#pragma unroll
        for (int c = 0; c < XC; ++c) {
            unsigned d[8];
#pragma unroll
            for (int q = 0; q < 4; ++q) {
                const half_t lo = __builtin_bit_cast(half_t, (unsigned short)(xv[m][c][q] & 0xFFFFu));
                const half_t hi = __builtin_bit_cast(half_t, (unsigned short)(xv[m][c][q] >> 16));
                d[2 * q] = ((unsigned)(int)__builtin_fmaf((float)lo, scale, 0.0f) + 0x00808080u) ^ 0x00808080u;
                d[2 * q + 1] = ((unsigned)(int)__builtin_fmaf((float)hi, scale, 0.0f) + 0x00808080u) ^ 0x00808080u;
            }
            const int cc = lane + 64 * c;
            const int tu = cc >> 4, s = (cc >> 2) & 3, q4 = cc & 3;
#pragma unroll
            for (int h = 0; h < 2; ++h) {
                const unsigned a0 = d[2 * h], a1 = d[2 * h + 4], a2 = d[2 * h + 1], a3 = d[2 * h + 5];
                const unsigned t0 = __builtin_amdgcn_perm(a1, a0, 0x05010400u);
                const unsigned t1 = __builtin_amdgcn_perm(a1, a0, 0x07030602u);
                const unsigned t2 = __builtin_amdgcn_perm(a3, a2, 0x05010400u);
                const unsigned t3 = __builtin_amdgcn_perm(a3, a2, 0x07030602u);
                const int base = ((((tu * 2 + h) * MB + m) * 4) * 4 + q4) * 4 + s;
                planes[base + 0] = __builtin_amdgcn_perm(t2, t0, 0x05040100u);
                planes[base + 16] = __builtin_amdgcn_perm(t2, t0, 0x07060302u);
                planes[base + 32] = __builtin_amdgcn_perm(t3, t1, 0x05040100u);
                planes[base + 48] = __builtin_amdgcn_perm(t3, t1, 0x07060302u);
            }
        }
    }
    __builtin_amdgcn_fence(__ATOMIC_RELEASE, "wavefront");
    __builtin_amdgcn_wave_barrier();
    if constexpr (STAMPS) st->t[2] = __builtin_amdgcn_s_memrealtime();

    half_t c_old = (half_t)0.0f;
    if constexpr (!RNORM) {
        if (wk == 0 && (seg.epilogue & TCE_W4_ADD_TO_C) && tid < ROWS * MB * 16) {
            const int i16 = tid & 15, m = (tid >> 4) % MB, r = tid / (16 * MB);
            const int row = (tile0 + r) * 16 + i16;
            if (m0 + m < M_ && row < seg.N) c_old = seg.C[(size_t)(m0 + m) * seg.ldc + row];
        }
    }

    int4_t B[UPP][2];
#pragma unroll
    for (int uu = 0; uu < UPP; ++uu) B[uu][0] = B[uu][1] = int4_t{0, 0, 0, 0};
    auto read_b = [&](int ps) {
#pragma unroll
        for (int uu = 0; uu < UPP; ++uu)
#pragma unroll
            for (int gi = 0; gi < GPU; ++gi)
                if (uu_l == uu && gi_l == gi) {
#pragma unroll
                    for (int h = 0; h < 2; ++h) {
                        const unsigned *src = planes + ((((((ps * UPP + uu) * 2 + h) * MB + m_l) * 4 + p_l) * 4 + kq) * 4 + gi * SPG);
                        if constexpr (GPU == 1) {
                            B[uu][h] = __builtin_bit_cast(int4_t, *reinterpret_cast<const uint4_t *>(src));
                        } else if constexpr (GPU == 2) {
                            const uint2_t v = *reinterpret_cast<const uint2_t *>(src);
                            B[uu][h][gi * 2] = (int)v[0];
                            B[uu][h][gi * 2 + 1] = (int)v[1];
                        } else {
                            B[uu][h][gi] = (int)*src;
                        }
                    }
                }
    };
    read_b(0);

    float acc[ROWS][4];
#pragma unroll
    for (int r = 0; r < ROWS; ++r)
#pragma unroll
        for (int q = 0; q < 4; ++q) acc[r][q] = 0.f;
    const int4_t zero4 = int4_t{0, 0, 0, 0};
    const int4_t sixteens = int4_t{0x10101010, 0x10101010, 0x10101010, 0x10101010};
#pragma unroll
    for (int ps = 0; ps < NP; ++ps) {
        if constexpr (!Z8) __builtin_amdgcn_sched_barrier(0);
        int4_t dd[ROWS][2];
#pragma unroll
        for (int r = 0; r < ROWS; ++r) dd[r][0] = dd[r][1] = zero4;
        int4_t dz = zero4;
#pragma unroll
        for (int uu = 0; uu < UPP; ++uu) {
            const int t = ps * UPP + uu;
            if constexpr (!Z8) {
                dz = __builtin_amdgcn_mfma_i32_16x16x64_i8(sixteens, B[uu][0], dz, 0, 0, 0);
                dz = __builtin_amdgcn_mfma_i32_16x16x64_i8(sixteens, B[uu][1], dz, 0, 0, 0);
            }
#pragma unroll
            for (int r = 0; r < ROWS; ++r) {
                int4_t alo, ahi;
#pragma unroll
                for (int q = 0; q < 4; ++q) {
                    const unsigned wq = w[r][t][q];
                    ahi[q] = (int)((wq & 0xF0F0F0F0u) ^ 0x80808080u);
                    alo[q] = (int)(((wq << 4) & 0xF0F0F0F0u) ^ 0x80808080u);
                }
                dd[r][0] = __builtin_amdgcn_mfma_i32_16x16x64_i8(alo, B[uu][0], dd[r][0], 0, 0, 0);
                if constexpr (Z8) dd[r][1] = __builtin_amdgcn_mfma_i32_16x16x64_i8(ahi, B[uu][1], dd[r][1], 0, 0, 0);
                else dd[r][0] = __builtin_amdgcn_mfma_i32_16x16x64_i8(ahi, B[uu][1], dd[r][0], 0, 0, 0);
            }
        }
#pragma unroll
        for (int r = 0; r < ROWS; ++r) {
            const half_t s0 = __builtin_bit_cast(half_t, (unsigned short)(sc[r][ps][0] & 0xFFFFu));
            const half_t s1 = __builtin_bit_cast(half_t, (unsigned short)(sc[r][ps][0] >> 16));
            const half_t s2 = __builtin_bit_cast(half_t, (unsigned short)(sc[r][ps][1] & 0xFFFFu));
            const half_t s3 = __builtin_bit_cast(half_t, (unsigned short)(sc[r][ps][1] >> 16));
            int4_t tot = dd[r][0] + dd[r][1];
            if constexpr (!Z8) {
#pragma unroll
                for (int q = 0; q < 4; ++q) tot[q] += __mul24(8 - (int)((zq[r][ps >> 1] >> (16 * (ps & 1) + 4 * q)) & 0xFu), dz[q]);
            }
            acc[r][0] = __builtin_fmaf((float)tot[0], (float)s0, acc[r][0]);
            acc[r][1] = __builtin_fmaf((float)tot[1], (float)s1, acc[r][1]);
            acc[r][2] = __builtin_fmaf((float)tot[2], (float)s2, acc[r][2]);
            acc[r][3] = __builtin_fmaf((float)tot[3], (float)s3, acc[r][3]);
        }
        if (ps + 1 < NP) read_b(ps + 1);
    }

    if constexpr (STAMPS) {
        asm volatile("" ::"v"(acc[ROWS - 1][3]));
        st->t[3] = __builtin_amdgcn_s_memrealtime();
    }
    int sh_l = sh[0];
    bool bad_l = bad[0];
#pragma unroll
    for (int m = 1; m < MB; ++m) {
        sh_l = m_l == m ? sh[m] : sh_l;
        bad_l = m_l == m ? bad[m] : bad_l;
    }
    const float cj = bad_l ? __builtin_nanf("") : __builtin_bit_cast(float, (unsigned)(127 + 8 * p_l - sh_l - 4) << 23);
    float *red = reinterpret_cast<float *>(smem + (size_t)WK * UW * MB * 512);
#pragma unroll
    for (int r = 0; r < ROWS; ++r)
#pragma unroll
        for (int q = 0; q < 4; ++q) {
            float v = acc[r][q] * cj;
            v = dpp_add_f32<0xB1>(v);
            v = dpp_add_f32<0x4E>(v);
            if constexpr (MB <= 2) v = dpp_add_f32<0x128>(v);
            if constexpr (MB == 1) v = dpp_add_f32<0x124>(v);
            if (p_l == 0 && (j >> 2) < MB) red[((wk * ROWS + r) * MB + m_l) * 16 + kq * 4 + q] = v;
        }
    keep_scalar(seg.C);
    keep_scalar(seg.ldc);
    keep_scalar(seg.epilogue);
    keep_scalar(seg.N);
    keep_scalar(M_);
    float *ws_ = nullptr, *out_gamma_ = nullptr;
    half_t *xn_out_ = nullptr;
    unsigned out_eps_ = 0, last_wg_ = 0;
    if constexpr (RNORM) {
        ws_ = args.ws;
        out_gamma_ = const_cast<float *>(args.out_gamma);
        xn_out_ = args.xn_out;
        out_eps_ = __builtin_bit_cast(unsigned, args.out_eps);
        last_wg_ = gridDim.x - 1;
        keep_scalar(ws_);
        keep_scalar(out_gamma_);
        keep_scalar(xn_out_);
        keep_scalar(out_eps_);
        keep_scalar(last_wg_);
    }
    __syncthreads();
    if (tid < ROWS * MB * 16) {
        float part[16];
#pragma unroll
        for (int k2 = 0; k2 < 16; ++k2) part[k2] = red[(k2 < WK ? k2 : 0) * (ROWS * MB * 16) + tid];
        float v = 0.f;
#pragma unroll
        for (int k2 = 0; k2 < 16; ++k2) v += k2 < WK ? part[k2] : 0.f;
        const int i16 = tid & 15, m = (tid >> 4) % MB, r = tid / (16 * MB);
        const int row = (tile0 + r) * 16 + i16;
        const half_t y = (half_t)v;
        const half_t y_other = __builtin_bit_cast(half_t, (unsigned short)__builtin_amdgcn_update_dpp(0, (int)__builtin_bit_cast(unsigned short, y), 0xB1, 0xF, 0xF, false));
        half_t hnew = (half_t)0.0f;
        (void)hnew;
        if (m0 + m < M_ && row < seg.N) {
            half_t *crow = seg.C + (size_t)(m0 + m) * seg.ldc;
            if (seg.epilogue & TCE_W4_SILU_MUL_PAIRS) {
                if ((i16 & 1) == 0) crow[row >> 1] = silu_mul_half(y, y_other);
            } else if (seg.epilogue & TCE_W4_ADD_TO_C) {
                if constexpr (RNORM) hnew = crow[row] + y;
                else crow[row] = c_old + y;
            } else {
                crow[row] = y;
            }
            if constexpr (MIX) {
                if (gathers) {
                    const half_t outv = (seg.epilogue & TCE_W4_ADD_TO_C) ? (half_t)(c_old + y) : y;
                    const size_t off = ((size_t)args.g.slot * 2 + (g_epoch & 1u)) * args.g.vec_bytes + ((size_t)args.g.rank * args.g.slice_elems + (size_t)row) * 2;
#pragma unroll
                    for (int p = 0; p < kCommMaxRanks; ++p)
                        if (p < args.g.world)
                            __hip_atomic_store(reinterpret_cast<unsigned short *>(args.g.peer[p] + off), __builtin_bit_cast(unsigned short, outv), __ATOMIC_RELAXED, __HIP_MEMORY_SCOPE_SYSTEM);
                }
            }
        }
        if constexpr (RNORM) {
            if (row < seg.N) __hip_atomic_store(reinterpret_cast<unsigned short *>(seg.C) + row, __builtin_bit_cast(unsigned short, hnew), __ATOMIC_RELAXED, __HIP_MEMORY_SCOPE_SYSTEM);
            const float hf = row < seg.N ? (float)hnew : 0.f;
            float s0 = 0.f, s1 = 0.f;
#pragma unroll
            for (int e = 0; e < 8; ++e) {
                const float v0 = __builtin_bit_cast(float, __builtin_amdgcn_readlane(__builtin_bit_cast(int, hf), e));
                const float v1 = __builtin_bit_cast(float, __builtin_amdgcn_readlane(__builtin_bit_cast(int, hf), 8 + e));
                s0 = __builtin_fmaf(v0, v0, s0);
                s1 = __builtin_fmaf(v1, v1, s1);
            }
            if (tid < 2) __hip_atomic_store(ws_ + 2 * tile0 + tid, tid == 0 ? s0 : s1, __ATOMIC_RELAXED, __HIP_MEMORY_SCOPE_SYSTEM);
        }
    }
    if constexpr (STAMPS) {
        if (tid < 64 && args.dbg) {
            asm volatile("s_waitcnt vmcnt(0)" ::: "memory");
            st->t[4] = __builtin_amdgcn_s_memrealtime();
#pragma unroll
            for (int i = 0; i < 7; ++i)
                if (tid == i) args.dbg[(size_t)blockIdx.x * 8 + i] = st->t[i];
        }
    }
    if constexpr (MIX) {
        if (gathers && tid < 64) {
            asm volatile("s_waitcnt vmcnt(0)" ::: "memory");
            unsigned *const counter = args.g.epochs + args.g.slots + 1 + args.g.slot;
            unsigned last = 0;
            if (tid == 0) last = __hip_atomic_fetch_add(counter, 1u, __ATOMIC_RELAXED, __HIP_MEMORY_SCOPE_AGENT) == args.g_tiles - 1u ? 1u : 0u;
            last = (unsigned)__builtin_amdgcn_readfirstlane((int)last);
            if (last) {
                const unsigned e = g_epoch, par = e & 1u;
                __threadfence_system();
                if (tid < args.g.world) {
                    unsigned *flag = reinterpret_cast<unsigned *>(args.g.peer[tid] + args.g.flags_off) + (((size_t)args.g.slot * 2 + par) * kCommMaxRanks + args.g.rank) * kCommFlagStride;
                    __hip_atomic_store(flag, e, __ATOMIC_RELAXED, __HIP_MEMORY_SCOPE_SYSTEM);
                }
                if (tid < args.g.world) {
                    const unsigned *flag = reinterpret_cast<const unsigned *>(args.g.peer[args.g.rank] + args.g.flags_off) + (((size_t)args.g.slot * 2 + par) * kCommMaxRanks + tid) * kCommFlagStride;
                    const unsigned long long t0 = wall_clock64();
                    const bool dead = __hip_atomic_load(args.g.epochs + args.g.slots, __ATOMIC_RELAXED, __HIP_MEMORY_SCOPE_AGENT) != 0u;
                    while (!dead && (int)(__hip_atomic_load(flag, __ATOMIC_RELAXED, __HIP_MEMORY_SCOPE_SYSTEM) - e) < 0) {
                        __builtin_amdgcn_s_sleep(8);
                        if (wall_clock64() - t0 > args.g.timeout_ticks) {
                            __hip_atomic_store(args.g.epochs + args.g.slots, 1u, __ATOMIC_RELAXED, __HIP_MEMORY_SCOPE_AGENT);
                            break;
                        }
                    }
                }
                __builtin_amdgcn_wave_barrier();
                __threadfence_system();
                const unsigned char *full = args.g.peer[args.g.rank] + ((size_t)args.g.slot * 2 + par) * args.g.vec_bytes;
                const unsigned total16 = args.g.slice_elems * (unsigned)args.g.world / 8u;
                for (unsigned base = 0; base < total16; base += 64 * 8) {
                    uint4_t v[8];
#pragma unroll
                    for (int q = 0; q < 8; ++q) {
                        const unsigned i = base + q * 64 + tid;
                        const unsigned ic = i < total16 ? i : total16 - 1;
                        asm volatile("global_load_dwordx4 %0, %1, off sc0 sc1" : "=v"(v[q]) : "v"(full + (size_t)ic * 16) : "memory");
                    }
                    asm volatile("s_waitcnt vmcnt(0)" ::: "memory");
#pragma unroll
                    for (int q = 0; q < 8; ++q) {
                        const unsigned i = base + q * 64 + tid;
                        if (i < total16) reinterpret_cast<uint4_t *>(args.g.dst)[i] = v[q];
                    }
                }
                if (tid == 0) {
                    __hip_atomic_store(counter, 0u, __ATOMIC_RELAXED, __HIP_MEMORY_SCOPE_AGENT);
                    __hip_atomic_store(args.g.epochs + args.g.slot, e, __ATOMIC_RELAXED, __HIP_MEMORY_SCOPE_AGENT);
                }
            }
        }
    }
    if constexpr (RNORM) {
        unsigned *flag = reinterpret_cast<unsigned *>(smem);
        if (tid < 64) {
            asm volatile("s_waitcnt vmcnt(0)" ::: "memory");
            if (tid == 0) {
                const unsigned old = __hip_atomic_fetch_add(reinterpret_cast<unsigned *>(ws_) + 2048, 1u, __ATOMIC_RELAXED, __HIP_MEMORY_SCOPE_AGENT);
                flag[0] = old == last_wg_ ? 1u : 0u;
            }
        }
        __syncthreads();
        if (flag[0] == 0u) return;
        if (tid == 0) reinterpret_cast<unsigned *>(ws_)[2048] = 0u;
        const int n = seg.N, pieces = n >> 3;
        auto sys_load_f32 = [](const float *p) { return __hip_atomic_load(p, __ATOMIC_RELAXED, __HIP_MEMORY_SCOPE_SYSTEM); };
        float tot = 0.f;
#pragma unroll
        for (int c = 0; c < 16; ++c) {
            const int q = c * 64 + lane;
            float slot = 0.f;
            slot += q < pieces ? sys_load_f32(ws_ + q) : 0.f;
            if (q + 1024 < pieces) slot += sys_load_f32(ws_ + q + 1024);
            tot += slot;
        }
        tot = wave_sum_dpp_lane63(tot);
        tot = __builtin_bit_cast(float, __builtin_amdgcn_readlane(__builtin_bit_cast(int, tot), 63));
        const float rs = 1.0f / sqrtf(tot / (float)n + __builtin_bit_cast(float, out_eps_));
        const half_t *hrow = seg.C;
        for (int p = tid; p < pieces; p += WK * 64) {
            uint4_t raw;
            asm volatile("global_load_dwordx4 %0, %1, off sc0 sc1\n\ts_waitcnt vmcnt(0)" : "=v"(raw) : "v"(hrow + p * 8) : "memory");
            const half8_t hv = __builtin_bit_cast(half8_t, raw);
            const float4_t g0 = *reinterpret_cast<const float4_t *>(out_gamma_ + p * 8), g1 = *reinterpret_cast<const float4_t *>(out_gamma_ + p * 8 + 4);
            half8_t o;
#pragma unroll
            for (int e = 0; e < 4; ++e) {
                o[e] = rmsnorm_out(hv[e], rs, g0[e]);
                o[4 + e] = rmsnorm_out(hv[4 + e], rs, g1[e]);
            }
            *reinterpret_cast<half8_t *>(xn_out_ + p * 8) = o;
        }
    }
}

template <int MB, int GPU, int ROWS, int UW, bool Z8, int MAXT, bool NORM = false, bool RNORM = false, int COMB = 0, bool STAMPS = false>
__global__ __launch_bounds__(MAXT) void w4a16_gemv_i8_kernel(const void *words, int bytes_w, int U, const void *A_, int lda, int K, const void *dscales_, int bytes_s, int N, int M,
                                                            int geom, const I8Tail t) {
    const half_t *A = static_cast<const half_t *>(A_), *dscales = static_cast<const half_t *>(dscales_);
    extern __shared__ __attribute__((aligned(16))) unsigned char smem_wg[];
    I8Stamps st;
    if constexpr (STAMPS) {
        st.t[0] = __builtin_amdgcn_s_memrealtime();
        st.t[5] = __builtin_amdgcn_s_memtime();
        __builtin_amdgcn_sched_barrier(0);
    }
    const int WK = geom & 0xFF, nseg = geom >> 8;
    int si = 0, block_begin = 0;
    if (nseg > 1) {
        static_assert(TCE_MAX_GROUP == 4, "the batch below names three further linears");
        I8SegHead h[TCE_MAX_GROUP - 1] = {t.head[0], t.head[1], t.head[2]};
        asm volatile("" : "+s"(h[0].words), "+s"(h[0].dscales), "+s"(h[0].bytes_w), "+s"(h[0].bytes_s), "+s"(h[0].N), "+s"(h[0].block_begin),
                          "+s"(h[1].words), "+s"(h[1].dscales), "+s"(h[1].bytes_w), "+s"(h[1].bytes_s), "+s"(h[1].N), "+s"(h[1].block_begin),
                          "+s"(h[2].words), "+s"(h[2].dscales), "+s"(h[2].bytes_w), "+s"(h[2].bytes_s), "+s"(h[2].N), "+s"(h[2].block_begin));
#pragma unroll
        for (int s = 1; s < TCE_MAX_GROUP; ++s) {
            const bool mine = s < nseg && (int)blockIdx.x >= h[s - 1].block_begin;
            si = mine ? s : si;
            words = mine ? h[s - 1].words : words;
            dscales = mine ? h[s - 1].dscales : dscales;
            bytes_w = mine ? h[s - 1].bytes_w : bytes_w;
            bytes_s = mine ? h[s - 1].bytes_s : bytes_s;
            N = mine ? h[s - 1].N : N;
            block_begin = mine ? h[s - 1].block_begin : block_begin;
        }
    }
    const I8SegRest &r = t.rest[si];
    const I8Seg seg{words, dscales, r.dzeros, r.C, N, r.ldc, r.epilogue, bytes_w, bytes_s, r.bytes_z, block_begin};
    w4a16_gemv_i8_body<MB, GPU, ROWS, UW, Z8, NORM, RNORM, COMB, false, I8Tail, STAMPS>(t, smem_wg, (int)threadIdx.x, WK, U, K, lda, M, A, seg, ((int)blockIdx.x - block_begin) * ROWS, false, 0u, &st);
}

template <bool Z8>
__global__ __launch_bounds__(1024) void w4a16_gemv_i8_mixed_kernel(const I8MixArgs args) {
    extern __shared__ __attribute__((aligned(16))) unsigned char smem_wg[];
    unsigned char *smem = smem_wg;
    int tid = threadIdx.x;
    int si = 0;
#pragma unroll
    for (int s = 1; s < kI8MixMax; ++s)
        if (s < args.nseg && (int)blockIdx.x >= args.s[s].seg.block_begin) si = s;
    const half_t *A_ = args.s[si].A;
    const int lda_ = args.s[si].lda;
    const int K_ = args.s[si].K;
    const I8Seg seg = args.s[si].seg;
    const int U = K_ >> 7;
    const int wl = blockDim.x >> 6;
    const int WK = (U + 8 - 1) / 8;
    const int nsub = wl / WK;
    const int sub = __builtin_amdgcn_readfirstlane(tid >> 6) / WK;
    const int tile0 = ((int)blockIdx.x - seg.block_begin) * nsub + sub;
    if (sub >= nsub || tile0 >= ((seg.N + 15) >> 4)) return;
    tid -= sub * WK * 64;
    smem += (size_t)sub * ((size_t)WK * 8 * 512 + (size_t)WK * 16 * sizeof(float));
    const bool gathers = si == args.g_seg;
    unsigned g_epoch = 0;
    if (gathers) g_epoch = __hip_atomic_load(args.g.epochs + args.g.slot, __ATOMIC_RELAXED, __HIP_MEMORY_SCOPE_AGENT) + 1u;
    w4a16_gemv_i8_body<1, 1, 1, 8, Z8, false, false, 0, true>(args, smem, tid, WK, U, K_, lda_, args.M, A_, seg, tile0, gathers, g_epoch);
}

static int i8_units_per_wave(int U) { return U <= 128 ? 8 : (U <= 256 ? 16 : 0); }
thread_local int g_i8_mode = 0;
thread_local int g_i8_rows = 0;
thread_local unsigned long long *g_i8_stamps = nullptr;

struct I8Launch {
    const void *words;
    const half_t *dscales, *A;
    int bytes_w, bytes_s, U, lda, K, N, M, nseg;
    I8Tail t;
};

template <int MB, int GPU, int ROWS, int UW, bool Z8, int MAXT, bool NORM = false, bool RNORM = false, int COMB = 0, bool STAMPS = false>
hipError_t launch_i8(const I8Launch &a, int blocks, int m_blocks, int wk, hipStream_t stream) {
    const size_t lds = (size_t)wk * UW * MB * 512 + (size_t)wk * ROWS * MB * 16 * sizeof(float) + (NORM ? (size_t)(a.K >> 3) * sizeof(float) + 1024 : 0);
    auto kfn = w4a16_gemv_i8_kernel<MB, GPU, ROWS, UW, Z8, MAXT, NORM, RNORM, COMB, STAMPS>;
    if (lds > 64 * 1024) {
        const hipError_t e = hipFuncSetAttribute(reinterpret_cast<const void *>(kfn), hipFuncAttributeMaxDynamicSharedMemorySize, (int)lds);
        if (e != hipSuccess) return e;
    }
    hipLaunchKernelGGL(kfn, dim3(blocks, m_blocks, 1), dim3(64 * wk, 1, 1), lds, stream, a.words, a.bytes_w, a.U, static_cast<const void *>(a.A), a.lda, a.K, static_cast<const void *>(a.dscales), a.bytes_s, a.N, a.M, wk | (a.nseg << 8), a.t);
    return hipGetLastError();
}

}

int gemv_i8_rows_per_pass(int M, int K, int group_size) {
    const int U = K / 128, gpu = 128 / group_size;
    const int uw = i8_units_per_wave(U);
    const int wk = (U + uw - 1) / uw;
    int mb = M >= 3 ? 4 : M;
    while (mb > 1 && (mb * gpu > 4 || (size_t)wk * uw * mb * 512 > 72 * 1024)) mb >>= 1;
    return mb;
}

void set_gemv_i8_stamps(void *buf) { g_i8_stamps = static_cast<unsigned long long *>(buf); }

void set_gemv_i8_mode(int mode, int rows) {
    g_i8_mode = mode == 1 ? 1 : 0;
    g_i8_rows = rows == 1 || rows == 2 ? rows : 0;
}


bool gemv_i8_supports(const tce_w4a16_desc *descs, int count, bool with_norm) {
    if (g_i8_mode == 1) return false;
    const tce_w4a16_desc &d0 = descs[0];
    if (d0.M < 1 || d0.M > 4 || d0.K % 128 != 0) return false;
    if ((d0.rmsnorm_gamma || with_norm) && (d0.M != 1 || d0.group_size != 128 || d0.K > 16384)) return false;
    if (d0.group_size != 128 && d0.M > (d0.group_size == 64 ? 2 : 1)) return false;
    const int uw = i8_units_per_wave(d0.K / 128);
    if (uw == 0 || (uw == 16 && (d0.M > 1 || d0.group_size != 128))) return false;
    for (int i = 0; i < count; ++i) {
        const tce_w4a16_desc &d = descs[i];
        if (!d.prepacked || (reinterpret_cast<uintptr_t>(d.prepacked) & 255)) return false;
        if ((long long)pk::nt16(d.N) * (d.K / 2) * 16 >= (1LL << 31)) return false;
        if (d.flags & TCE_W4_FORCE_GEMM) return false;
    }
    return true;
}

int launch_w4a16_gemv_i8(const tce_w4a16_desc *descs, int count, hipStream_t stream, hipError_t *hip_err, const float *gamma, float eps, const I8ResidualNorm *rn,
                         const AttnDeferred *comb, const int *comb_pos_dev, int comb_pos) {
    const tce_w4a16_desc &d0 = descs[0];
    if (!gamma && d0.rmsnorm_gamma) {
        gamma = static_cast<const float *>(d0.rmsnorm_gamma);
        eps = d0.rmsnorm_eps;
    }
    I8Launch a{};
    a.t.gamma = gamma;
    a.t.eps = eps;
    a.A = static_cast<const half_t *>(d0.A);
    a.lda = d0.lda ? d0.lda : d0.K;
    a.M = d0.M;
    a.K = d0.K;
    a.U = d0.K / 128;
    a.nseg = count;
    const int gpu = 128 / d0.group_size;
    const int uw = i8_units_per_wave(a.U);
    const int wk = (a.U + uw - 1) / uw;
    bool z8 = true;
    long long total_tiles = 0;
    for (int i = 0; i < count; ++i) {
        z8 = z8 && (descs[i].flags & TCE_W4_ZERO_POINT_IS_8);
        total_tiles += pk::nt16(descs[i].N);
    }
    const int mb = gemv_i8_rows_per_pass(d0.M, d0.K, d0.group_size);
    const int m_blocks = (d0.M + mb - 1) / mb;
    int rows = 1;
    const bool two_ok = mb == 1 && gpu == 1 && uw == 8 && wk <= 8;
    const long long resident = 256LL * (20 / wk);
    if (gamma && two_ok && total_tiles > resident && total_tiles * 5 <= resident * 6) rows = 2;
    if (g_i8_rows && two_ok) rows = g_i8_rows;
    int blocks = 0;
    for (int i = 0; i < count; ++i) {
        const tce_w4a16_desc &d = descs[i];
        const unsigned char *base = static_cast<const unsigned char *>(d.prepacked);
        I8SegHead h{};
        h.words = base;
        h.dscales = reinterpret_cast<const half_t *>(base + pk::dscales_offset(d.N, d.K, d.group_size));
        h.bytes_w = (int)pk::words_bytes(d.N, d.K);
        h.bytes_s = (int)pk::dscales_bytes(d.N, d.K, d.group_size);
        h.N = d.N;
        h.block_begin = blocks;
        if (i == 0) {
            a.words = h.words;
            a.dscales = h.dscales;
            a.bytes_w = h.bytes_w;
            a.bytes_s = h.bytes_s;
            a.N = h.N;
        } else {
            a.t.head[i - 1] = h;
        }
        I8SegRest &r = a.t.rest[i];
        r.C = static_cast<half_t *>(d.C);
        r.dzeros = reinterpret_cast<const unsigned *>(base + pk::dzeros_offset(d.N, d.K, d.group_size));
        r.epilogue = d.flags & (TCE_W4_SILU_MUL_PAIRS | TCE_W4_ADD_TO_C);
        r.ldc = d.ldc ? d.ldc : ((r.epilogue & TCE_W4_SILU_MUL_PAIRS) ? d.N / 2 : d.N);
        r.bytes_z = (int)pk::dzeros_bytes(d.N, d.K, d.group_size);
        blocks += (pk::nt16(d.N) + rows - 1) / rows;
    }
    for (int i = count; i < TCE_MAX_GROUP; ++i) {
        a.t.rest[i] = a.t.rest[0];
        a.t.head[i - 1] = I8SegHead{a.words, a.dscales, a.bytes_w, a.bytes_s, a.N, 0};
    }
    hipError_t e = hipErrorInvalidConfiguration;
    if (rn) {
        if (count != 1 || gamma || mb != 1 || gpu != 1 || d0.M != 1 || !(d0.flags & TCE_W4_ADD_TO_C) || d0.N > 16384 || d0.N % 8 != 0) return TCE_ERR_UNSUPPORTED_SHAPE;
        a.t.out_gamma = rn->gamma;
        a.t.out_eps = rn->eps;
        a.t.xn_out = static_cast<half_t *>(rn->xn_out);
        a.t.ws = static_cast<float *>(rn->workspace);
        if (uw == 8) e = z8 ? launch_i8<1, 1, 1, 8, true, 1024, false, true>(a, blocks, m_blocks, wk, stream) : launch_i8<1, 1, 1, 8, false, 1024, false, true>(a, blocks, m_blocks, wk, stream);
        else if (z8) e = launch_i8<1, 1, 1, 16, true, 1024, false, true>(a, blocks, m_blocks, wk, stream);
        else return TCE_ERR_UNSUPPORTED_SHAPE;
        if (e != hipSuccess) {
            if (hip_err) *hip_err = e;
            return TCE_ERR_HIP;
        }
        return TCE_OK;
    }
    if (comb && comb->slots > 1) {
        if (count != 1 || gamma || mb != 1 || gpu != 1 || uw != 8 || d0.M != 1 || d0.K != comb->heads * 128 || d0.K % 1024 != 0 || comb->slots > kAttnDeferMaxSlots || comb->stride != 132)
            return TCE_ERR_UNSUPPORTED_SHAPE;
        a.t.comb_part = comb->part;
        a.t.comb_pos_dev = comb_pos_dev;
        a.t.comb_pos = comb_pos;
        a.t.comb_slots = comb->slots;
        a.t.comb_chunk = comb->chunk;
        a.t.comb_stride = comb->stride;
        a.t.comb_heads = comb->heads;
        if (wk > 4) return TCE_ERR_UNSUPPORTED_SHAPE;
        if (comb->slots <= 4) e = z8 ? launch_i8<1, 1, 1, 8, true, 256, false, false, 4>(a, blocks, m_blocks, wk, stream) : launch_i8<1, 1, 1, 8, false, 256, false, false, 4>(a, blocks, m_blocks, wk, stream);
        else e = z8 ? launch_i8<1, 1, 1, 8, true, 256, false, false, 8>(a, blocks, m_blocks, wk, stream) : launch_i8<1, 1, 1, 8, false, 256, false, false, 8>(a, blocks, m_blocks, wk, stream);
        if (e != hipSuccess) {
            if (hip_err) *hip_err = e;
            return TCE_ERR_HIP;
        }
        return TCE_OK;
    }
    if (gamma) {
        if (mb != 1 || gpu != 1 || uw != 8) return TCE_ERR_UNSUPPORTED_SHAPE;
        if (rows == 2) e = z8 ? launch_i8<1, 1, 2, 8, true, 512, true>(a, blocks, m_blocks, wk, stream) : launch_i8<1, 1, 2, 8, false, 512, true>(a, blocks, m_blocks, wk, stream);
        else e = z8 ? launch_i8<1, 1, 1, 8, true, 1024, true>(a, blocks, m_blocks, wk, stream) : launch_i8<1, 1, 1, 8, false, 1024, true>(a, blocks, m_blocks, wk, stream);
        if (e != hipSuccess) {
            if (hip_err) *hip_err = e;
            return TCE_ERR_HIP;
        }
        return TCE_OK;
    }
#ifdef TCE_LAB
    if (g_i8_stamps && z8 && mb == 1 && gpu == 1 && rows == 1 && uw == 8) {
        a.t.dbg = g_i8_stamps;
        e = launch_i8<1, 1, 1, 8, true, 1024, false, false, 0, true>(a, blocks, m_blocks, wk, stream);
        if (e != hipSuccess) {
            if (hip_err) *hip_err = e;
            return TCE_ERR_HIP;
        }
        return TCE_OK;
    }
#endif
#define TCE_I8(MB_, GPU_, ROWS_, UW_, MAXT_)                                                                                        \
    if (mb == MB_ && gpu == GPU_ && rows == ROWS_ && uw == UW_) {                                                                   \
        e = z8 ? launch_i8<MB_, GPU_, ROWS_, UW_, true, MAXT_>(a, blocks, m_blocks, wk, stream)                                     \
               : launch_i8<MB_, GPU_, ROWS_, UW_, false, MAXT_>(a, blocks, m_blocks, wk, stream);                                   \
    } else
    TCE_I8(1, 1, 1, 8, 1024)
    TCE_I8(1, 1, 2, 8, 512)
    TCE_I8(1, 1, 1, 16, 1024)
    TCE_I8(2, 1, 1, 8, 1024)
    TCE_I8(4, 1, 1, 8, 1024)
    TCE_I8(1, 2, 1, 8, 1024)
    TCE_I8(2, 2, 1, 8, 1024)
    TCE_I8(1, 4, 1, 8, 1024)
    return TCE_ERR_UNSUPPORTED_SHAPE;
#undef TCE_I8
    if (e != hipSuccess) {
        if (hip_err) *hip_err = e;
        return TCE_ERR_HIP;
    }
    return TCE_OK;
}

static_assert(kI8MixMax == TCE_MAX_INDEPENDENT, "include/tce_matmul.h");

bool gemv_i8_mixed_supports(const tce_w4a16_desc *descs, int count) {
    if (g_i8_mode == 1 || count < 1 || count > kI8MixMax) return false;
    for (int i = 0; i < count; ++i) {
        const tce_w4a16_desc &d = descs[i];
        if (d.M != 1 || d.group_size != 128 || d.K % 128 != 0 || d.K > 16384 || d.rmsnorm_gamma) return false;
        if (!d.prepacked || (reinterpret_cast<uintptr_t>(d.prepacked) & 255)) return false;
        if ((long long)pk::nt16(d.N) * (d.K / 2) * 16 >= (1LL << 31)) return false;
        if (d.flags & TCE_W4_FORCE_GEMM) return false;
    }
    return true;
}

thread_local int g_i8_mix_waves = 0;
void set_gemv_i8_mixed_waves(int w) { g_i8_mix_waves = w >= 1 && w <= 16 ? w : 0; }

void gemv_i8_mixed_geometry(const tce_w4a16_desc *descs, int count, int *waves, int *workgroups) {
    struct Memo {
        int count = 0, forced = -1, n[kI8MixMax], k[kI8MixMax], waves = 0, workgroups = 0;
    };
    thread_local Memo memo;
    bool hit = memo.count == count && memo.forced == g_i8_mix_waves;
    for (int i = 0; i < count && hit; ++i) hit = memo.n[i] == descs[i].N && memo.k[i] == descs[i].K;
    if (hit) {
        *waves = memo.waves;
        *workgroups = memo.workgroups;
        return;
    }
    int need = 1;
    for (int i = 0; i < count; ++i) need = need > (descs[i].K / 128 + 7) / 8 ? need : (descs[i].K / 128 + 7) / 8;
    auto blocks_at = [&](int wl) {
        int blocks = 0;
        for (int i = 0; i < count; ++i) {
            const int nsub = wl / ((descs[i].K / 128 + 7) / 8);
            blocks += (pk::nt16(descs[i].N) + nsub - 1) / nsub;
        }
        return blocks;
    };
    auto max_load = [&](int wl) {
        int load[256] = {0};
        int b0 = 0;
        for (int i = 0; i < count; ++i) {
            const int wk = (descs[i].K / 128 + 7) / 8, nsub = wl / wk, tiles = pk::nt16(descs[i].N);
            const int n = (tiles + nsub - 1) / nsub, units = nsub * wk, last_units = (tiles - (n - 1) * nsub) * wk;
            const int every = n / 256, extra = n % 256;
            for (int c = 0; c < 256; ++c) load[c] += every * units;
            for (int e = 0; e < extra; ++e) load[(b0 + every * 256 + e) & 255] += units;
            load[(b0 + n - 1) & 255] -= units - last_units;
            b0 += n;
        }
        int worst = 0;
        for (int c = 0; c < 256; ++c) worst = worst > load[c] ? worst : load[c];
        return worst;
    };
    int best_load = 1 << 30;
    for (int w = need; w <= 16; ++w) best_load = best_load < max_load(w) ? best_load : max_load(w);
    int wl = need;
    long best_blocks = 1L << 40;
    for (int w = need; w <= 16; ++w)
        if (max_load(w) * 20 <= best_load * 21 && blocks_at(w) < best_blocks) best_blocks = blocks_at(w), wl = w;
    if (g_i8_mix_waves >= need) wl = g_i8_mix_waves;
    *waves = wl;
    *workgroups = blocks_at(wl);
    memo.count = count;
    memo.forced = g_i8_mix_waves;
    for (int i = 0; i < count; ++i) memo.n[i] = descs[i].N, memo.k[i] = descs[i].K;
    memo.waves = wl;
    memo.workgroups = *workgroups;
}

int launch_w4a16_gemv_i8_mixed(const tce_w4a16_desc *descs, int count, hipStream_t stream, hipError_t *hip_err, const PeerGatherEpi *gather, int gathered) {
    if (!gemv_i8_mixed_supports(descs, count)) return TCE_ERR_UNSUPPORTED_SHAPE;
    I8MixArgs a{};
    a.nseg = count;
    a.M = 1;
    if (gather) {
        if (gathered < 0 || gathered >= count) return TCE_ERR_BAD_ARG;
        const tce_w4a16_desc &dg = descs[gathered];
        if ((dg.flags & TCE_W4_SILU_MUL_PAIRS) || (unsigned)dg.N != gather->slice_elems) return TCE_ERR_UNSUPPORTED_SHAPE;
        a.g = *gather;
        a.g_seg = gathered;
        a.g_tiles = (unsigned)pk::nt16(dg.N);
    }
    int wl = 1, total = 0;
    gemv_i8_mixed_geometry(descs, count, &wl, &total);
    bool z8 = true;
    int blocks = 0;
    for (int i = 0; i < count; ++i) {
        const tce_w4a16_desc &d = descs[i];
        z8 = z8 && (d.flags & TCE_W4_ZERO_POINT_IS_8);
        I8MixSeg &m = a.s[i];
        m.A = static_cast<const half_t *>(d.A);
        m.lda = d.lda ? d.lda : d.K;
        m.K = d.K;
        I8Seg &s = m.seg;
        const unsigned char *base = static_cast<const unsigned char *>(d.prepacked);
        s.words = base;
        s.dscales = reinterpret_cast<const half_t *>(base + pk::dscales_offset(d.N, d.K, d.group_size));
        s.dzeros = reinterpret_cast<const unsigned *>(base + pk::dzeros_offset(d.N, d.K, d.group_size));
        s.C = static_cast<half_t *>(d.C);
        s.N = d.N;
        s.epilogue = d.flags & (TCE_W4_SILU_MUL_PAIRS | TCE_W4_ADD_TO_C);
        s.ldc = d.ldc ? d.ldc : ((s.epilogue & TCE_W4_SILU_MUL_PAIRS) ? d.N / 2 : d.N);
        s.bytes_w = (int)pk::words_bytes(d.N, d.K);
        s.bytes_s = (int)pk::dscales_bytes(d.N, d.K, d.group_size);
        s.bytes_z = (int)pk::dzeros_bytes(d.N, d.K, d.group_size);
        s.block_begin = blocks;
        const int nsub = wl / ((d.K / 128 + 7) / 8);
        blocks += (pk::nt16(d.N) + nsub - 1) / nsub;
    }
    for (int i = count; i < kI8MixMax; ++i) a.s[i] = a.s[0];
    const size_t lds = (size_t)wl * 8 * 512 + (size_t)wl * 16 * sizeof(float);
    auto launch = [&](auto kfn) -> hipError_t {
        if (lds > 64 * 1024) {
            const hipError_t e = hipFuncSetAttribute(reinterpret_cast<const void *>(kfn), hipFuncAttributeMaxDynamicSharedMemorySize, (int)lds);
            if (e != hipSuccess) return e;
        }
        hipLaunchKernelGGL(kfn, dim3(blocks, 1, 1), dim3(64 * wl, 1, 1), lds, stream, a);
        return hipGetLastError();
    };
    const hipError_t e = z8 ? launch(w4a16_gemv_i8_mixed_kernel<true>) : launch(w4a16_gemv_i8_mixed_kernel<false>);
    if (e != hipSuccess) {
        if (hip_err) *hip_err = e;
        return TCE_ERR_HIP;
    }
    return TCE_OK;
}

}
```

tinychatengine_amd/csrc/w4a16_gemv_i8_token.hip:

```cpp
#include "tce_common.hpp"
#include "w4a16_kernels.hpp"
#include "w4a16_mfma_layout.hpp"

#include <new>
#include <vector>

namespace tce {

namespace {

constexpr int kTokWaves = 16;
constexpr int kTokMaxChunks = 15;
constexpr int kTokMaxUnits = 512;
constexpr int kTokMaxTiles = 128;

struct TokSeg {
    const void *words;
    const half_t *dscales;
    half_t *C;
    unsigned *C_tag;
    int N, epilogue, tile_begin, bytes_w, bytes_s, pad;
};
static_assert(sizeof(TokSeg) == 56, "record layout");
struct TokStage {
// ... 347 lines not shown
                        const unsigned w1 = tok_dpp_u32<0x101>(word), w2 = tok_dpp_u32<0x102>(word), w3 = tok_dpp_u32<0x103>(word);
                        if (lane < 16 && (lane & 3) == 0 && row + 3 < N) {
                            __builtin_amdgcn_raw_buffer_store_b128(uint4_t{word, w1, w2, w3}, rs_c, idx * 4, 0,  17);
                        } else if (lane < 16 && row < N && !(((row & ~3) + 3) < N)) {
                            __hip_atomic_store(C_tag + idx, word, __ATOMIC_RELAXED, __HIP_MEMORY_SCOPE_AGENT);
                        }
                    }
                }
            }
            u_cur += kTokWaves;
            if (u_cur < nunits) request(u_cur);
        }
    }
}

__global__ void i8_token_epoch_kernel(unsigned *epoch) { *epoch = *epoch % 65535u + 1u; }

int tok_num_cus() {
    int dev = 0, cus = 0;
    if (hipGetDevice(&dev) != hipSuccess) return 0;
    if (hipDeviceGetAttribute(&cus, hipDeviceAttributeMultiprocessorCount, dev) != hipSuccess) return 0;
    return cus;
}

thread_local unsigned long long *g_tok_stamps = nullptr;
thread_local int g_tok_mode = 0;
thread_local int g_tok_max_units = kTokMaxUnits;

}

struct I8TokenPlan {
    TokStage *stages = nullptr;
    unsigned *sync = nullptr;
    unsigned *shadow = nullptr;
    int n = 0, blocks = 0;
    unsigned long long *stamps = nullptr;
};

void set_i8_token_stamps(void *buf) { g_tok_stamps = static_cast<unsigned long long *>(buf); }
void set_i8_token_mode(int mode) { g_tok_mode = mode == 1 ? 1 : 0; }
void set_i8_token_max_units(int u) { g_tok_max_units = u >= 1 && u <= kTokMaxUnits ? u : kTokMaxUnits; }

void i8_token_plan_destroy(I8TokenPlan *tp) {
    if (!tp) return;
    if (tp->stages) (void)hipFree(tp->stages);
    if (tp->sync) (void)hipFree(tp->sync);
    if (tp->shadow) (void)hipFree(tp->shadow);
    delete tp;
}

int i8_token_plan_stages(const I8TokenPlan *tp) { return tp ? tp->n : 0; }
int i8_token_plan_blocks(const I8TokenPlan *tp) { return tp ? tp->blocks : 0; }

int i8_token_plan_create(const tce_w4a16_desc *descs, const int32_t *groups, int n_launches, I8TokenPlan **out, int *n_taken, hipError_t *hip_err) {
    if (g_tok_mode == 1) return TCE_ERR_UNSUPPORTED_SHAPE;
    const int cus = tok_num_cus();
    if (cus == 0) return TCE_ERR_HIP;
#ifdef TCE_LAB
    const void *kfn = g_tok_stamps ? reinterpret_cast<const void *>(w4a16_gemv_i8_token_kernel<true>) : reinterpret_cast<const void *>(w4a16_gemv_i8_token_kernel<false>);
#else
    const void *kfn = reinterpret_cast<const void *>(w4a16_gemv_i8_token_kernel<false>);
#endif
    hipError_t e = hipFuncSetAttribute(kfn, hipFuncAttributeMaxDynamicSharedMemorySize, kLdsBytes);
    int per_cu = 0;
    if (e == hipSuccess) e = hipOccupancyMaxActiveBlocksPerMultiprocessor(&per_cu, kfn, 64 * kTokWaves, kLdsBytes);
    if (e != hipSuccess) {
        if (hip_err) *hip_err = e;
        return TCE_ERR_HIP;
    }
    if (per_cu < 1) return TCE_ERR_UNSUPPORTED_SHAPE;
    const int P = cus;

    std::vector<TokStage> host;
    std::vector<int> first_desc;
    for (int l = 0, off = 0; l < n_launches; off += groups[l], ++l) {
        const tce_w4a16_desc &d0 = descs[off];
        bool ok = d0.M == 1 && d0.group_size == 128 && d0.K % 128 == 0 && d0.K >= 128 && (d0.K + 1023) / 1024 <= kTokMaxChunks && !d0.rmsnorm_gamma &&
                  (d0.lda == 0 || d0.lda == d0.K) && groups[l] <= TCE_MAX_GROUP;
        TokStage st{};
        int tiles = 0;
        for (int i = 0; i < groups[l] && ok; ++i) {
            const tce_w4a16_desc &d = descs[off + i];
            ok = d.M == 1 && d.K == d0.K && d.group_size == 128 && d.A == d0.A && d.prepacked && !(reinterpret_cast<uintptr_t>(d.prepacked) & 255) && (d.flags & TCE_W4_ZERO_POINT_IS_8) &&
                 !(d.flags & TCE_W4_FORCE_GEMM) && !d.rmsnorm_gamma && (long long)pk::nt16(d.N) * (d.K / 2) * 16 < (1LL << 31) && !(d.flags & ~(TCE_W4_ZERO_POINT_IS_8 | TCE_W4_SILU_MUL_PAIRS | TCE_W4_ADD_TO_C));
            if ((d.flags & TCE_W4_SILU_MUL_PAIRS) && (d.N % 2 != 0 || (d.flags & TCE_W4_ADD_TO_C))) ok = false;
            if (!ok) break;
            TokSeg &sg = st.seg[i];
            const unsigned char *base = static_cast<const unsigned char *>(d.prepacked);
            sg.words = base;
            sg.dscales = reinterpret_cast<const half_t *>(base + pk::dscales_offset(d.N, d.K, d.group_size));
            sg.C = static_cast<half_t *>(d.C);
            sg.C_tag = nullptr;
            sg.N = d.N;
            sg.epilogue = d.flags & (TCE_W4_SILU_MUL_PAIRS | TCE_W4_ADD_TO_C);
            sg.tile_begin = tiles;
            sg.bytes_w = (int)pk::words_bytes(d.N, d.K);
            sg.bytes_s = (int)pk::dscales_bytes(d.N, d.K, d.group_size);
            tiles += pk::nt16(d.N);
        }
        if (ok) {
            st.A = static_cast<const half_t *>(d0.A);
            st.A_tag = nullptr;
            st.K = d0.K;
            st.U = d0.K / 128;
            st.nch = (st.U + 7) / 8;
            st.nseg = groups[l];
            st.ntiles = tiles;
            for (int i = groups[l]; i < TCE_MAX_GROUP; ++i) st.seg[i] = st.seg[0];
            const int tiles_wg = (tiles + P - 1) / P;
            ok = tiles_wg <= kTokMaxTiles && tiles_wg * st.nch <= g_tok_max_units;
        }
        if (!ok) break;
        host.push_back(st);
        first_desc.push_back(off);
    }
    const int n = (int)host.size();
    if (n < 2) return TCE_ERR_UNSUPPORTED_SHAPE;

    I8TokenPlan *tp = new (std::nothrow) I8TokenPlan();
    if (!tp) return TCE_ERR_BAD_ARG;
    tp->n = n;
    tp->blocks = P;
#ifdef TCE_LAB
    tp->stamps = g_tok_stamps;
#endif
    auto n_out_of = [&](const TokStage &L, int i) { return (L.seg[i].epilogue & TCE_W4_SILU_MUL_PAIRS) ? L.seg[i].N / 2 : L.seg[i].N; };
    size_t words = 0;
    std::vector<size_t> base((size_t)n * TCE_MAX_GROUP, 0);
    for (int l = 0; l < n; ++l)
        for (int i = 0; i < host[l].nseg; ++i) {
            base[(size_t)l * TCE_MAX_GROUP + i] = words;
            words += ((size_t)n_out_of(host[l], i) + 63) & ~(size_t)63;
        }
    e = hipMalloc(reinterpret_cast<void **>(&tp->shadow), words * sizeof(unsigned));
    if (e == hipSuccess) e = hipMemset(tp->shadow, 0, words * sizeof(unsigned));
    std::vector<int> producer(n, -1);
    std::vector<std::vector<char>> consumed((size_t)n, std::vector<char>(TCE_MAX_GROUP, 0));
    bool refuse = false;
    for (int l = 0; l < n && e == hipSuccess && !refuse; ++l) {
        TokStage &L = host[l];
        const char *a0 = reinterpret_cast<const char *>(L.A), *a1 = a0 + (size_t)L.K * 2;
        for (int q = l - 1; q >= 0 && producer[l] < 0 && !refuse; --q)
            for (int i = 0; i < host[q].nseg; ++i) {
                const char *c0 = reinterpret_cast<const char *>(host[q].seg[i].C), *c1 = c0 + (size_t)n_out_of(host[q], i) * 2;
                if (a0 >= c0 && a1 <= c1) {
                    if ((a0 - c0) % 16 != 0) {
                        refuse = true;
                        break;
                    }
                    L.A_tag = tp->shadow + base[(size_t)q * TCE_MAX_GROUP + i] + (a0 - c0) / 2;
                    producer[l] = q;
                    consumed[q][i] = 1;
                    break;
                }
                if (a0 < c1 && a1 > c0) {
                    refuse = true;
                    break;
                }
            }
    }
    for (int l = 0; l < n; ++l)
        for (int i = 0; i < host[l].nseg; ++i) host[l].seg[i].C_tag = tp->shadow + base[(size_t)l * TCE_MAX_GROUP + i];
    if (e == hipSuccess && !refuse) {
        const size_t nw64 = ((size_t)n + 63) / 64;
        std::vector<uint64_t> anc((size_t)n * nw64, 0);
        for (int l = 0; l < n; ++l)
            if (producer[l] >= 0) {
                const int q = producer[l];
                for (size_t k = 0; k < nw64; ++k) anc[l * nw64 + k] = anc[q * nw64 + k];
                anc[l * nw64 + (size_t)q / 64] |= 1ull << (q % 64);
            }
        for (int l = 1; l < n && !refuse; ++l)
            for (int i = 0; i < host[l].nseg && !refuse; ++i) {
// ... 72 lines not shown
```

tinychatengine_amd/csrc/w4a16_kernels.hpp:

```cpp
#pragma once
#include "tce_common.hpp"

namespace tce {

struct GemvSeg {
    const uint4_t *qweight;
    const half_t *scales;
    const unsigned *zeros;
    half_t *C;
    int N, ldc, scales_stride, zeros_stride;
    int bytes_w, bytes_s, bytes_z;
    int block_begin;
    int epilogue;
};

struct GemvArgs {
    const half_t *A;
    int lda, M, K, log2g;
    int nseg;
    unsigned long long *dbg;
    int zeros_are_8;
    const float *gamma;
    float eps;
    int shared_xsum;
    GemvSeg seg[TCE_MAX_GROUP];
};

#define TCE_GEMV_VARIANTS(X) \
    X(1, 4, 1, 1)            \
    X(2, 4, 1, 1)            \
    X(4, 4, 1, 1)            \
    X(1, 4, 1, 2)            \
    X(2, 4, 1, 2)            \
    X(4, 4, 1, 2)            \
    X(2, 4, 1, 3)            \
    X(3, 4, 1, 1)            \
    X(3, 4, 1, 2)            \
    X(2, 8, 1, 2)            \
    X(4, 8, 1, 1)            \
    X(1, 2, 2, 1)            \
    X(2, 2, 2, 1)            \
    X(2, 2, 2, 2)            \
    X(1, 2, 4, 1)

bool gemv_variant_exists(int rows, int wn, int wk, int depth);
void set_gemv_debug_mode(int mode);
void set_gemv_order(int force);
void set_w8a8_deep(int d);
void set_w8a8_rows32(int r);
void set_w8a8_kslice(int code);
void set_w8a8_big(int b);
void set_lnq_stamps(void *p);
void set_lnq_form(int f);
void set_gemv_shared_xsum(int on);
void set_gemv_debug_buffer(void *p);

struct StreamLaunch {
    const half_t *A;
    int K, log2g;
    int nseg;
    int n_rg;
    GemvSeg seg[TCE_MAX_GROUP];
    const float *gamma;
    float eps;
    const unsigned *A_tag;
    unsigned *C_tag[TCE_MAX_GROUP];
};
void set_gemv_stream_config(int rows, int nw, int depth);
void set_gemv_stream_debug(int mode, void *buf);
bool gemv_stream_supports(const tce_w4a16_desc *descs, int count);
int launch_w4a16_gemv_stream(const tce_w4a16_desc *descs, int count, hipStream_t stream, hipError_t *hip_err,
                             const float *gamma = nullptr, float eps = 0.f);
struct TokenPlan;
int token_plan_create(const tce_w4a16_desc *descs, const int32_t *groups, int n_launches, TokenPlan **out, hipError_t *hip_err, int mode = 0);
int token_plan_mode(const TokenPlan *tp);
struct OvlGeom {
    int wn, xb, depth, rows_per_block, grid, per_cu;
    bool z8;
    size_t lds;
};
int ovl_chains();
int ovl_geometry(const tce_w4a16_desc *descs, int count, int cus, int chains, OvlGeom *g, hipError_t *hip_err);
hipError_t ovl_enqueue(const StreamLaunch *L, const OvlGeom &g, const unsigned *epoch, unsigned *status, int launch_index, hipStream_t stream);
void set_gemv_ovl_config(int depth, int chains);
void set_gemv_ovl_stamps(void *buf);
int token_plan_enqueue(TokenPlan *tp, hipStream_t stream, hipError_t *hip_err);
int token_plan_status(TokenPlan *tp, unsigned *status, hipError_t *hip_err);
void token_plan_geometry(const TokenPlan *tp, int *rows, int *depth, int *waves, int *blocks);
void token_plan_destroy(TokenPlan *tp);
int launch_w4a16_gemv(const tce_w4a16_desc *descs, int count, int forced_rows, int forced_wn, int forced_wk,
                      int forced_depth, hipStream_t stream, hipError_t *hip_err, const float *gamma = nullptr, float eps = 0.f);

bool gemv_i8_supports(const tce_w4a16_desc *descs, int count, bool with_norm = false);
int gemv_i8_rows_per_pass(int M, int K, int group_size);
void set_gemv_i8_mode(int mode, int rows);
struct I8ResidualNorm {
    const float *gamma;
    float eps;
    void *xn_out;
    void *workspace;
};
struct AttnDeferred;
int launch_w4a16_gemv_i8(const tce_w4a16_desc *descs, int count, hipStream_t stream, hipError_t *hip_err, const float *gamma = nullptr, float eps = 0.f, const I8ResidualNorm *rn = nullptr,
                         const AttnDeferred *comb = nullptr, const int *comb_pos_dev = nullptr, int comb_pos = 0);

struct PeerGatherEpi;
bool gemv_i8_mixed_supports(const tce_w4a16_desc *descs, int count);
void gemv_i8_mixed_geometry(const tce_w4a16_desc *descs, int count, int *waves, int *workgroups);
void set_gemv_i8_mixed_waves(int w);
int launch_w4a16_gemv_i8_mixed(const tce_w4a16_desc *descs, int count, hipStream_t stream, hipError_t *hip_err, const PeerGatherEpi *gather = nullptr, int gathered = -1);
struct I8TokenPlan;
int i8_token_plan_create(const tce_w4a16_desc *descs, const int32_t *groups, int n_launches, I8TokenPlan **out, int *n_taken, hipError_t *hip_err);
int i8_token_plan_enqueue(I8TokenPlan *tp, hipStream_t stream, hipError_t *hip_err);
int i8_token_plan_status(I8TokenPlan *tp, unsigned *status, hipError_t *hip_err);
int i8_token_plan_stages(const I8TokenPlan *tp);
int i8_token_plan_blocks(const I8TokenPlan *tp);
void i8_token_plan_destroy(I8TokenPlan *tp);
void set_gemv_i8_stamps(void *buf);
void set_i8_token_stamps(void *buf);
void set_i8_token_max_units(int u);
void set_i8_token_mode(int mode);

#define TCE_GEMM_VARIANTS(X) \
    X(8, 1)                  \
    X(8, 2)                  \
    X(4, 2)                  \
    X(4, 1)                  \
    X(2, 2)                  \
    X(4, 4)                  \
    X(2, 4)
bool gemm_variant_exists(int m_tiles, int n_tiles);
void set_gemm_xcd_rows(int xm);
void set_gemm_dma_xcd_rows(int xm);
float gemm_dma_estimate_us(int M, int N, int K);
void gemm_dma_describe(int M, int N, bool g128, int *mt, int *nt, int *ks);
void set_gemm_dma_mode(int mode);
void set_w8a8_ksplit(int ks);
int launch_w4a16_gemm_dma(const tce_w4a16_desc &d, int m_tiles, int n_tiles, hipStream_t stream, hipError_t *hip_err);
int launch_w4a16_gemm(const tce_w4a16_desc &d, int forced_mt, int forced_nt, hipStream_t stream, hipError_t *hip_err);

size_t prepack_bytes(int N, int K, int G);
int launch_w4a16_prepack(const tce_w4a16_desc &d, void *out, hipStream_t stream, hipError_t *hip_err);
int launch_w4a16_gemm_pk(const tce_w4a16_desc &d, const void *packed, hipStream_t stream, hipError_t *hip_err);
void set_gemm_pk256_auto(int on);
void set_gemm_pk_wide_auto(int on);
void set_gemm_pk_form16_auto(int on);
void set_gemm_pk_handoff_delta(int d);
void set_gemm_pk_prio(int on);
void set_gemm_pk_handoff(int on);
float gemm_pk_estimate_us(int M, int N, int K, int *form_out, bool has_scratch = false, int *split_out = nullptr, int group_size = 128, bool zero_point_8 = false);
size_t gemm_pk_scratch_bytes();
void set_gemm_pk_split(int s);
void set_gemm_pk_mode(int ks, int xm);
void set_gemm_pk_ablation(int abl);

int check_zero_point_8(const void *zeros, long long n_words, hipError_t *hip_err);
int check_zero_point_8_async(const void *zeros, long long n_words, int *verdict, hipStream_t stream, hipError_t *hip_err);

int launch_awq_fp16acc(int M, int N, int K, int G, const void *A, const void *qweight, const void *scales, void *C,
                       hipStream_t stream, hipError_t *hip_err);
int launch_awq_repack(int N, int K, int G, const void *qweight, const void *scales, void *workspace, hipStream_t stream,
                      hipError_t *hip_err);

bool skinny_supports(const tce_w4a16_desc &d);
void set_skinny_config(int ks);
void set_skinny_max_m(int m);
int launch_w4a16_skinny(const tce_w4a16_desc &d, hipStream_t stream, hipError_t *hip_err);

int launch_layernorm_q(const float *x, const float *w, const float *b, void *out, int m, int n, hipStream_t stream, hipError_t *hip_err);
int launch_lnq_w8a8_group(const float *x, const float *ln_w, const float *ln_b, int m, int k, const tce_w8a8_desc *lin, int count, void *ln_out,
                          hipStream_t stream, hipError_t *hip_err);
int launch_opt_softmax_q(const float *scores, const float *mask, void *probs, int heads, int sq, int tgz, int ldp, hipStream_t stream, hipError_t *hip_err);
int launch_opt_kv_append(const void *k, const void *v, void *kc, void *vt, int heads, int hd, int sq, int pos, int max_keys, hipStream_t stream, hipError_t *hip_err);
int launch_rmsnorm_half(const void *x, const float *gamma, void *out, int m, int n, float eps, hipStream_t stream, hipError_t *hip_err);
int launch_bmm_f16t(const void *A, const void *B, void *C, int batch, int M, int N, int K, unsigned short alpha_bits, hipStream_t stream, hipError_t *hip_err);
int launch_attention_decode(const void *q, const void *K, const void *Vt, const void *mask, void *out, int heads, int t, int hd, unsigned short alpha_bits,
                            hipStream_t stream, hipError_t *hip_err);
struct Comm;
int comm_create(int rank, int world, int max_vector_elems, int slots, Comm **out, hipError_t *he);
int comm_export(Comm *c, void *handle64, hipError_t *he);
int comm_connect_ipc(Comm *c, const void *handles, hipError_t *he);
int comm_connect_local(Comm *c, Comm *const *all, hipError_t *he);
int comm_set_timeout_ms(Comm *c, int ms);
int comm_reset(Comm *c, hipError_t *he);
int comm_device(const Comm *c);
int comm_status(Comm *c, hipError_t *he);
void comm_destroy(Comm *c);
int launch_allgather_f16(Comm *c, int slot, const void *src_slice, void *dst_full, int n_total, hipStream_t stream, hipError_t *he);
int comm_world_of(const Comm *c);
constexpr int kCommMaxRanks = 8, kCommFlagStride = 16;
struct PeerGatherEpi {
    unsigned char *peer[8];
    unsigned *epochs;
    void *dst;
    int rank, world, slot, slots;
    unsigned slice_elems;
    size_t vec_bytes, flags_off;
    unsigned long long timeout_ticks;
};
int comm_peer_gather_epi(Comm *c, int slot, void *dst_full, int n_total, PeerGatherEpi *out);
int comm_rccl_unique_id(void *id128);
int comm_rccl_init(Comm *c, const void *id128);
bool comm_has_rccl(const Comm *c);
const char *comm_rccl_last_error();
bool comm_peer_regime(const Comm *c, int n_total);
int launch_allgather_rccl(Comm *c, const void *src_slice, void *dst_full, size_t n_per_rank, hipStream_t stream);
size_t allgather_rows_workspace_bytes(int M, int n_total);
int launch_allgather_rows_f16(Comm *c, int slot, const void *src, void *dst, int M, int n_total, int ldd, void *workspace, hipStream_t stream, hipError_t *he);
void set_attention_fast_target(int wgs);
void set_attention_fast_waves(int nw);
void set_attention_fast_fuse(int r);
void set_attention_fast_probe_no_combine(int on);
void describe_attention_decode_fast(int heads, int keys, int *chunk, int *chunks, int *waves, int kv_heads = 0);
size_t attention_decode_workspace_bytes(int heads, int max_keys, int hd);
int launch_opt_attention_decode(const void *q, const void *kn, const void *vn, void *kc, void *vtc, const float *mask, void *out, int heads, int hd, int m, int pos,
                                int max_keys, int ld, float a_qk, float a_pv, hipStream_t stream, hipError_t *hip_err);
size_t attention_prefill_workspace_bytes(int heads, int m, int hd);
void set_attention_prefill_waves(int w);
int launch_attention_prefill(const void *qkv, int ld_qkv, void *kc, void *vc, const void *cosv, const void *sinv, const void *mask, int ld_mask, int causal,
                             void *out, int ld_out, void *workspace, int heads, int kv_heads, int max_keys, int pos, int m, float alpha, hipStream_t stream,
                             hipError_t *hip_err);
size_t attention_prefill_paged_workspace_bytes(int heads, int total_rows, int hd);
int describe_attention_prefill_paged(int heads, int causal, const int *segments, int nseg, int *form, int *pair, int *nblocks, int *workgroups);
int launch_attention_prefill_paged(const void *qkv, int ld_qkv, void *k_pool, void *v_pool, const int *table, int table_stride, int page_keys, const void *cosv,
                                   const void *sinv, int causal, void *out, int ld_out, void *workspace, int heads, int kv_heads, const int *segments, int nseg,
// ... 45 lines not shown
```

tinychatengine_amd/csrc/w4a16_mfma_layout.hpp:

```cpp
#pragma once
#include <stddef.h>
#include <stdint.h>

#if defined(__HIPCC__)
#define TCE_HD __host__ __device__ inline
#else
#define TCE_HD inline
#endif

namespace tce {
namespace pk {

constexpr int kBM = 128;
constexpr int kHalfK = 64;
constexpr int kHalfBytes = kBM * kHalfK * 2;

TCE_HD int nt16(int N) { return (N + 15) / 16; }
TCE_HD size_t words_bytes(int N, int K) { return (size_t)nt16(N) * (K / 128) * 64 * 4 * 4; }
TCE_HD size_t consts_bytes(int N, int K, int G) { return (size_t)nt16(N) * (K / G) * 16 * 8; }
TCE_HD size_t last_bytes(int N) { return (size_t)nt16(N) * 16 * 4; }
TCE_HD size_t align256(size_t x) { return (x + 255) & ~(size_t)255; }
TCE_HD size_t consts_offset(int N, int K) { return align256(words_bytes(N, K)); }
TCE_HD size_t last_offset(int N, int K, int G) { return consts_offset(N, K) + align256(consts_bytes(N, K, G)); }
TCE_HD size_t dscales_bytes(int N, int K, int G) { return (size_t)nt16(N) * (K / G) * 16 * 2; }
TCE_HD size_t dzeros_bytes(int N, int K, int G) { return (size_t)nt16(N) * (K / G) * 8; }
TCE_HD size_t dscales_offset(int N, int K, int G) { return last_offset(N, K, G) + align256(last_bytes(N)); }
TCE_HD size_t dzeros_offset(int N, int K, int G) { return dscales_offset(N, K, G) + align256(dscales_bytes(N, K, G)); }
TCE_HD size_t total_bytes(int N, int K, int G) { return dzeros_offset(N, K, G) + align256(dzeros_bytes(N, K, G)); }

TCE_HD size_t word_index(int n, int k, int K) {
    const int jt = n >> 4, n16 = n & 15, kb = k >> 7, kk = k & 127;
    const int s = kk >> 5, q = (kk >> 3) & 3;
    return (((size_t)jt * (K >> 7) + kb) * 64 + (q * 16 + n16)) * 4 + s;
}
TCE_HD int nibble_index(int k) {
    const int e = k & 7;
    return (e >> 1) + 4 * (e & 1);
}
TCE_HD void unpack_word_codes(uint32_t w, int out[8]) {
    const uint32_t sh = w >> 8;
    const uint32_t d0 = w & 0x000F000Fu, d1 = w & 0x00F000F0u, d2 = sh & 0x000F000Fu, d3 = sh & 0x00F000F0u;
    out[0] = d0 & 0xFFFF;          out[1] = d0 >> 16;
    out[2] = (d1 & 0xFFFF) >> 4;   out[3] = d1 >> 20;
    out[4] = d2 & 0xFFFF;          out[5] = d2 >> 16;
    out[6] = (d3 & 0xFFFF) >> 4;   out[7] = d3 >> 20;
}
TCE_HD size_t const_index(int n, int g, int K, int G) { return ((size_t)(n >> 4) * (K / G) + g) * 16 + (n & 15); }
TCE_HD uint32_t zc_word(unsigned z) { return ((0xD400u | (z << 4)) << 16) | (0xE400u | z); }

TCE_HD int swz(int row) { return (row >> 1) & 7; }
TCE_HD int lds_piece_offset(int row, int p) { return row * 128 + ((p ^ swz(row)) << 4); }
TCE_HD int dma_row(int w, int ii, int lane, int nw = 4) { return (ii * nw + w) * 8 + (lane >> 3); }
TCE_HD int dma_src_piece(int row, int lane) { return (lane & 7) ^ swz(row); }
TCE_HD int dma_lds_base(int w, int ii, int nw = 4) { return (ii * nw + w) * 1024; }
TCE_HD int frag_offset(int i, int n16, int q, int sl) { return lds_piece_offset(i * 16 + n16, sl * 4 + q); }

}
}
```

tinychatengine_amd/decode.py:

```python
from __future__ import annotations

import os
from dataclasses import dataclass

import torch

from . import capi, quantize
from .linear import Linear_half_int4
from .matmul import _stream


@dataclass(frozen=True)
class ModelShape:
    name: str
    hidden: int
    qkv: tuple[int, ...]
    ffn: int
    vocab: int
    layers: int


SHAPES = {
    "baseline-named": ModelShape("baseline-named (Llama-2-7B-shaped, as BASELINE.json spells it)", 4096, (12288,), 11008, 32000, 32),
    "llama3-8b": ModelShape("llama3-8b (true shapes, model.h:83)", 4096, (4096, 1024, 1024), 14336, 128256, 32),
    "llama2-13b": ModelShape("llama2-13b (model.h:72)", 5120, (15360,), 13824, 32000, 40),
    "tiny": ModelShape("tiny (tests)", 256, (256, 128, 128), 512, 1024, 2),
}


def _synthetic_linear(n: int, k: int, seed: int, device, group_size: int, rank: int, world: int, std: float = 0.02) -> Linear_half_int4:
    n_loc = n // world
    blocks = 8 if (n % 8 == 0 and 8 % world == 0) else 1
    if blocks == 1:
        g = torch.Generator(device=device).manual_seed(seed)
        w = torch.empty((n, k), dtype=torch.float32, device=device).normal_(0.0, std, generator=g)[rank * n_loc:(rank + 1) * n_loc]
    else:
        rows = n // blocks
        per_rank = blocks // world
        w = torch.empty((n_loc, k), dtype=torch.float32, device=device)
        for j in range(per_rank):
            g = torch.Generator(device=device).manual_seed(seed * 8 + rank * per_rank + j)
            w[j * rows:(j + 1) * rows].normal_(0.0, std, generator=g)
    lin = Linear_half_int4.from_float(w.contiguous(), group_size)
    del w
    return lin


class DecodeLinears:

    def __init__(self, shape: ModelShape, device="cuda", group_size: int = 128, rank: int = 0, world: int = 1,
                 m: int = 1, seed: int = 1234, layers: int | None = None, dataflow: bool = False, prepack: bool = False):
        self.shape, self.rank, self.world, self.m, self.group_size = shape, rank, world, m, group_size
        self.dataflow = dataflow
        if dataflow and (world != 1 or m != 1 or shape.qkv[0] < shape.hidden):
            raise ValueError("dataflow wiring: world 1, M = 1, and a first qkv linear at least `hidden` wide")
        self.device = torch.device(device)
        self._host_ok = self.device.type != "cuda"
        L = shape.layers if layers is None else layers
        self.n_layers = L
        h, f = shape.hidden, shape.ffn
        for n in (*shape.qkv, h, f, shape.vocab):
            if n % world or (n // world) % 16:
                raise ValueError(f"N={n} does not shard {world}-way into multiples of 16 rows")
        mk = lambda n, k, s: _synthetic_linear(n, k, seed + s, self.device, group_size, rank, world, std=(k ** -0.5 if dataflow else 0.02))
        self.blocks = []
        for li in range(L):
            s = li * 16
            self.blocks.append(dict(
                qkv=[mk(n, h, s + i) for i, n in enumerate(shape.qkv)],
                o=mk(h, h, s + 4), gate=mk(f, h, s + 5), up=mk(f, h, s + 6), down=mk(h, f, s + 7)))
        self.lm_head = mk(shape.vocab, h, 999_983)
        self.prepacked = bool(prepack)
        if prepack:
            for l in self.all_linears():
                l.prepack()
        gx = torch.Generator(device=self.device).manual_seed(4321)
        rnd = lambda *sz: torch.empty(sz, dtype=torch.float32, device=self.device).normal_(0, 1, generator=gx).to(torch.float16)
        self.x = rnd(m, h)
        self.attn = rnd(m, h)
        self.h2 = rnd(m, h)
        self.act = rnd(m, f)
        W = world
        e = lambda n: torch.empty((m, n), dtype=torch.float16, device=self.device)
        self.out_qkv = [e(n // W) for n in shape.qkv]
        self.out_o, self.out_gate, self.out_up, self.out_down = e(h // W), e(f // W), e(f // W), e(h // W)
        self.logits = e(shape.vocab // W)
        if dataflow:
            self.attn, self.h2, self.act = self.out_qkv[0][:, :h], self.out_o, self.out_gate
        if W > 1 or os.environ.get("TCE_FORCE_GATHER_BUFFERS"):
            self.g_qkv = [e(n) for n in shape.qkv]
            self.g_o, self.g_gate, self.g_up, self.g_down, self.g_logits = e(h), e(f), e(f), e(h), e(shape.vocab)

    def block_launches(self, li: int) -> list[list[capi.W4A16Desc]]:
        b = self.blocks[li]
        x = self.out_down if self.dataflow and li > 0 else self.x
        return [
            [l.desc(x, o, allow_host=self._host_ok) for l, o in zip(b["qkv"], self.out_qkv)],
            [b["o"].desc(self.attn, self.out_o, allow_host=self._host_ok)],
            [b["gate"].desc(self.h2, self.out_gate, allow_host=self._host_ok), b["up"].desc(self.h2, self.out_up, allow_host=self._host_ok)],
            [b["down"].desc(self.act, self.out_down, allow_host=self._host_ok)],
        ]

    def token_launches(self, grouped: bool = True) -> list[list[capi.W4A16Desc]]:
        out = []
        for li in range(self.n_layers):
            out += self.block_launches(li)
        out.append([self.lm_head.desc(self.out_down if self.dataflow else self.x, self.logits, allow_host=self._host_ok)])
        if not grouped:
            out = [[d] for g in out for d in g]
        return out

    def all_linears(self) -> list[Linear_half_int4]:
        ls = []
        for b in self.blocks:
            ls += [*b["qkv"], b["o"], b["gate"], b["up"], b["down"]]
        return ls + [self.lm_head]

    def token_bytes(self) -> int:
        return sum(capi.algorithmic_bytes(self.m, l.out_features, l.in_features, self.group_size) for l in self.all_linears())

    def token_launches_one_per_block(self) -> list[list[capi.W4A16Desc]]:
        if self.dataflow:
            raise ValueError("the data-flow wiring orders the linears of a block: they are not independent")
        return [[d for g in self.block_launches(li) for d in g] for li in range(self.n_layers)] + \
               [[self.lm_head.desc(self.x, self.logits, allow_host=self._host_ok)]]

    def make_plan(self, grouped: bool = True, tagged: bool = False, overlapped: bool = False, tuned: bool = False, one_launch_per_block: bool = False) -> capi.Plan:
        if one_launch_per_block:
            return capi.Plan(self.token_launches_one_per_block(), independent=True)
        return capi.Plan(self.token_launches(grouped), tagged=tagged, overlapped=overlapped, tuned=tuned)

    @staticmethod
    def _hip_launch(group: list[capi.W4A16Desc]) -> None:
        st = _stream()
        capi.check(capi.w4a16_forward_group(group, st) if len(group) > 1 else capi.w4a16_forward(group[0], st))

    @staticmethod
    def _hip_launch_independent(group: list[capi.W4A16Desc]) -> None:
        capi.w4a16_forward_independent(group, _stream())

    def run_block(self, li: int, launch=None) -> None:
        launch = launch or self._hip_launch
        for g in self.block_launches(li):
            launch(g)

    def run_lm_head(self, launch=None) -> None:
        (launch or self._hip_launch)([self.lm_head.desc(self.x, self.logits, allow_host=self._host_ok)])

    def attach_peer_comm(self, exchange) -> None:
        n_max = max(*self.shape.qkv, self.shape.hidden, self.shape.ffn, self.shape.vocab)
        self.comm = capi.Comm(self.rank, self.world, n_max * self.m, slots=8)
        self.comm.connect(exchange(self.comm.export()))

    def _rows_workspace(self, full: torch.Tensor) -> torch.Tensor:
        if getattr(self, "_rows_ws", None) is None or self._rows_ws.numel() < full.numel():
            n_max = max(*self.shape.qkv, self.shape.hidden, self.shape.ffn, self.shape.vocab)
# ... 63 lines not shown
```

tinychatengine_amd/linear.py:

```python
from __future__ import annotations

import torch

from . import capi, quantize
from .matmul import MatmulOperator, matmul_params, matrix, _ptr, _stream


_gemm_scratch: dict = {}


def gemm_scratch(device) -> torch.Tensor:
    key = str(device)
    if key not in _gemm_scratch:
        _gemm_scratch[key] = torch.zeros(int(capi.lib().tce_w4a16_gemm_scratch_bytes()), dtype=torch.uint8, device=device)
    return _gemm_scratch[key]


class Linear_half_int4:

    def __init__(self, qweight: torch.Tensor, scales: torch.Tensor, zeros: torch.Tensor, group_size: int = quantize.QK4_6):
        self.weight, self.scale, self.zero_point = qweight, scales, zeros
        self.out_features, self.in_features = qweight.shape[0], qweight.shape[1] * 8
        self.group_size = group_size
        zw = quantize.calculate_zeros_width(self.in_features, group_size)
        if tuple(scales.shape) != (self.out_features, zw * 8) or tuple(zeros.shape) != (self.out_features, zw):
            raise ValueError("scales/zeros do not have the padded q4_6 shapes (quantize_methods.py:431-440)")
        self.zeros_are_8 = bool((zeros == -2004318072).all().item())
        self.packed = None
        self._op = MatmulOperator()

    def prepack(self) -> "Linear_half_int4":
        if self.packed is None:
            need = int(capi.lib().tce_w4a16_prepack_bytes(self.out_features, self.in_features, self.group_size))
            if need:
                buf = torch.empty(need + 256, dtype=torch.uint8, device=self.weight.device)
                off = (-buf.data_ptr()) % 256
                self._packed_storage = buf
                self.packed = buf[off:off + need]
                d = capi.W4A16Desc(M=1, N=self.out_features, K=self.in_features, group_size=self.group_size, qweight=_ptr(self.weight),
                                   scales=_ptr(self.scale), zeros=_ptr(self.zero_point))
                capi.check(capi.lib().tce_w4a16_prepack(d, self.packed.data_ptr(), _stream()))
        return self

    @classmethod
    def from_float(cls, w: torch.Tensor, group_size: int = quantize.QK4_6):
        return cls(*quantize.quantize_q4_6(w, group_size), group_size=group_size)

    @classmethod
    def load(cls, dirname: str, out_features: int, in_features: int, group_size: int = quantize.QK4_6, device="cuda"):
        return cls(*quantize.load_linear_q4_6(dirname, out_features, in_features, group_size, device), group_size=group_size)

    def desc(self, x: torch.Tensor, out: torch.Tensor, ldc: int = 0, flags: int = 0, gamma: torch.Tensor | None = None, eps: float = 0.0,
             allow_host: bool = False) -> capi.W4A16Desc:
        m = x.numel() // self.in_features
        pairs = bool(flags & capi.TCE_W4_SILU_MUL_PAIRS)
        n_out = self.out_features // 2 if pairs else self.out_features
        for name, t, dt in (("x", x, torch.float16), ("out", out, torch.float16), ("gamma", gamma, torch.float32)):
            if t is None:
                continue
            if t.dtype != dt:
                raise ValueError(f"{name} must be {dt}, got {t.dtype}")
            if not t.is_contiguous():
                raise ValueError(f"{name} must be contiguous")
            if not allow_host and not t.is_cuda:
                raise ValueError(f"{name} must be a device tensor (no CPU fallback)")
        if x.numel() != m * self.in_features or m < 1:
            raise ValueError("x is not [M][in_features]")
        if out.numel() < (m - 1) * (ldc or n_out) + n_out:
            raise ValueError("out is too small for [M][N] with this ldc")
        if gamma is not None and gamma.numel() != self.in_features:
            raise ValueError("gamma must be fp32 [in_features]")
        return capi.W4A16Desc(M=m, N=self.out_features, K=self.in_features, group_size=self.group_size, A=x.data_ptr(),
                              qweight=self.weight.data_ptr(), scales=self.scale.data_ptr(), zeros=self.zero_point.data_ptr(),
                              C=out.data_ptr(), ldc=ldc, flags=flags | (capi.TCE_W4_ZERO_POINT_IS_8 if self.zeros_are_8 else 0),
                              rmsnorm_gamma=gamma.data_ptr() if gamma is not None else None, rmsnorm_eps=float(eps),
                              prepacked=self.packed.data_ptr() if self.packed is not None else None,
                              scratch=gemm_scratch(self.weight.device).data_ptr() if self.packed is not None and m > 128 else None)

    @classmethod
    def interleave(cls, gate: "Linear_half_int4", up: "Linear_half_int4") -> "Linear_half_int4":
        assert gate.weight.shape == up.weight.shape and gate.group_size == up.group_size
        il = lambda a, b: torch.stack((a, b), dim=1).reshape(2 * a.shape[0], *a.shape[1:]).contiguous()
        return cls(il(gate.weight, up.weight), il(gate.scale, up.scale), il(gate.zero_point, up.zero_point), gate.group_size)

    def forward_silu_mul(self, x: torch.Tensor, out: torch.Tensor | None = None) -> torch.Tensor:
        if out is None:
            out = torch.empty((*x.shape[:-1], self.out_features // 2), dtype=torch.float16, device=x.device)
        capi.check(capi.w4a16_forward(self.desc(x, out, flags=capi.TCE_W4_SILU_MUL_PAIRS), _stream()))
        return out

    def forward_add(self, x: torch.Tensor, residual_inout: torch.Tensor) -> torch.Tensor:
        capi.check(capi.w4a16_forward(self.desc(x, residual_inout, flags=capi.TCE_W4_ADD_TO_C), _stream()))
        return residual_inout

    def forward(self, x: torch.Tensor, out: torch.Tensor | None = None) -> torch.Tensor:
        m = x.numel() // self.in_features
        assert self.out_features > 8 and self.out_features % 16 == 0
        if out is None:
            out = torch.empty((*x.shape[:-1], self.out_features), dtype=torch.float16, device=x.device)
        if self.packed is not None:
            capi.check(capi.w4a16_forward(self.desc(x, out), _stream()))
            return out
        p = matmul_params(A=matrix(m, self.in_features, x), B=matrix(self.in_features // 8, self.out_features, self.weight),
                          C=matrix(m, self.out_features, out), half_scales=self.scale,
                          int32_zero_point=self.zero_point, block_size=self.group_size)
        self._op.gemv_forward_cuda(p)
        return out

    __call__ = forward

    def shard(self, rank: int, world: int) -> "Linear_half_int4":
        n = self.out_features
        if n % world or (n // world) % 16:
            raise ValueError(f"N={n} does not shard {world}-way into multiples of 16 rows (Linear_half_int4::forward's own requirement)")
        lo, hi = rank * (n // world), (rank + 1) * (n // world)
        return Linear_half_int4(self.weight[lo:hi].contiguous(), self.scale[lo:hi].contiguous(),
                                self.zero_point[lo:hi].contiguous(), self.group_size)

    def weight_bytes(self) -> int:
        return capi.algorithmic_bytes(1, self.out_features, self.in_features, self.group_size)


def forward_group(linears: list[Linear_half_int4], x: torch.Tensor, outs: list[torch.Tensor]) -> None:
    capi.check(capi.w4a16_forward_group([l.desc(x, o) for l, o in zip(linears, outs)], _stream()))


def rmsnorm_half(x: torch.Tensor, gamma: torch.Tensor, eps: float, out: torch.Tensor | None = None) -> torch.Tensor:
    if out is None:
        out = torch.empty_like(x)
    n = x.shape[-1]
    if x.dtype != torch.float16 or out.dtype != torch.float16 or gamma.dtype != torch.float32 or gamma.numel() != n:
        raise ValueError("rmsnorm_half: x / out fp16 [..., n], gamma fp32 [n]")
    capi.check(capi.lib().tce_rmsnorm_half(_ptr(x), _ptr(gamma), _ptr(out), x.numel() // n, n, float(eps), _stream()))
    return out


def forward_group_rmsnorm(linears: list[Linear_half_int4], x: torch.Tensor, outs: list[torch.Tensor], gamma: torch.Tensor, eps: float) -> None:
    import ctypes as C
    descs = [l.desc(x, o) for l, o in zip(linears, outs)]
    arr = (capi.W4A16Desc * len(descs))(*descs)
    if gamma.dtype != torch.float32 or gamma.numel() != x.shape[-1]:
        raise ValueError("gamma must be fp32 [in_features]")
    capi.check(capi.lib().tce_w4a16_forward_group_rmsnorm(arr, len(descs), _ptr(gamma), float(eps), C.c_void_p(_stream() or 0)))


class W8A8B8O8Linear:

    def __init__(self, weight: torch.Tensor, bias_int8: torch.Tensor, alpha: float, beta: float, relu: bool = False):
        self.weight, self.bias, self.alpha, self.beta = weight, bias_int8, float(alpha), float(beta)
        self.q_min = 0 if relu else -128
        self._op = MatmulOperator()

    def forward(self, x: torch.Tensor) -> torch.Tensor:
        n, k = self.weight.shape
        m = x.numel() // k
        out = torch.empty((*x.shape[:-1], n), dtype=torch.int8, device=x.device)
        p = matmul_params(A=matrix(m, k, x), B=matrix(k, n, self.weight), C=matrix(m, n, out), bias=matrix(1, n, self.bias),
# ... 60 lines not shown
```

Baseline: 1079 tokens/s.

## Prepack grouped linears (qkv, gate/up) into one contiguous packed copy

Adds a group prepack that lays q/k/v and gate/up weights into a single packed buffer with shared tile indexing, and teaches the GEMV/GEMM/token kernels to address members by first tile and total rows. A grouped GEMV can then treat members as one contiguous matrix, with a per-tile lookup picking each member's output pointer and epilogue. The aim is to cut per-member segment overhead and keep weight streaming contiguous across members. It adds per-row member selection logic to the kernel epilogue and changes how packed offsets are computed, which could cost registers.

```diff
diff --git a/include/tce_matmul.h b/include/tce_matmul.h
--- a/include/tce_matmul.h
+++ b/include/tce_matmul.h
@@ -209,6 +209,9 @@
 TCE_API int tce_w4a16_gemm_scratch_faults(const void *scratch, void *stream, uint32_t *faults);
 TCE_API int tce_w4a16_prepack(const tce_w4a16_desc *d, void *packed, void *stream);
 
+TCE_API size_t tce_w4a16_prepack_group_bytes(const tce_w4a16_desc *descs, int count);
+TCE_API int tce_w4a16_prepack_group(const tce_w4a16_desc *descs, int count, void *packed, void *stream);
+
 #define TCE_MAX_GROUP 4
 TCE_API int tce_w4a16_forward_group(const tce_w4a16_desc *descs, int count, void *stream);
 #define TCE_MAX_INDEPENDENT 8
diff --git a/tinychatengine_amd/capi.py b/tinychatengine_amd/capi.py
--- a/tinychatengine_amd/capi.py
+++ b/tinychatengine_amd/capi.py
@@ -29,7 +29,7 @@
 TCE_OUT_INT8, TCE_OUT_FP32 = 0, 1
 
 EXPORTS = [
-    "tce_w4a16_forward", "tce_w4a16_residual_rmsnorm_workspace_bytes", "tce_w4a16_forward_residual_rmsnorm", "tce_w4a16_prepack_bytes", "tce_w4a16_prepack", "tce_w4a16_gemm_scratch_bytes", "tce_w4a16_gemm_scratch_faults", "tce_w4a16_describe_dispatch", "tce_w8a8_describe_dispatch", "tce_reset_last_error", "tce_bmm_f16t", "tce_rope_half", "tce_softmax_half", "tce_attention_decode_f16", "tce_attention_decode_workspace_bytes", "tce_attention_decode_describe", "tce_attention_decode_step_f16", "tce_attention_decode_step_gqa_f16", "tce_attention_decode_describe_gqa", "tce_attention_decode_step_pos_f16", "tce_attention_decode_batch_workspace_bytes", "tce_attention_decode_describe_batch", "tce_attention_decode_step_batch_f16", "tce_kv_pages_pool_bytes", "tce_attention_decode_describe_paged", "tce_attention_decode_step_paged_f16", "tce_kv_pages_scatter_f16", "tce_kv_pages_gather_f16", "tce_kv_block_table_check", "tce_attention_prefill_f16", "tce_attention_prefill_workspace_bytes", "tce_attention_prefill_paged_workspace_bytes", "tce_attention_prefill_paged_f16", "tce_attention_prefill_describe_paged", "tce_kv_pages_pool_bytes_fp8", "tce_attention_decode_step_paged_fp8", "tce_attention_prefill_paged_fp8", "tce_kv_pages_scatter_fp8", "tce_kv_pages_gather_fp8", "tce_sample_workspace_bytes", "tce_sample_f16", "tce_embed_rows_f16", "tce_attention_decode_step_paged_rows_f16", "tce_attention_decode_step_paged_rows_fp8", "tce_sample_verify_workspace_bytes", "tce_sample_verify_f16", "tce_draft_ngram", "tce_opt_attention_decode", "tce_prefetch", "tce_add_half", "tce_silu_mul_half", "tce_rmsnorm_half", "tce_w4a16_forward_group_rmsnorm", "tce_w4a16_forward_group", "tce_w4a16_forward_independent", "tce_w4a16_describe_independent", "tce_w4a16_forward_independent_gather", "tce_w4a16_check_zero_point_8", "tce_w4a16_awq_fp16acc", "tce_w4a16_awq_workspace_bytes",
+    "tce_w4a16_forward", "tce_w4a16_residual_rmsnorm_workspace_bytes", "tce_w4a16_forward_residual_rmsnorm", "tce_w4a16_prepack_bytes", "tce_w4a16_prepack", "tce_w4a16_prepack_group_bytes", "tce_w4a16_prepack_group", "tce_w4a16_gemm_scratch_bytes", "tce_w4a16_gemm_scratch_faults", "tce_w4a16_describe_dispatch", "tce_w8a8_describe_dispatch", "tce_reset_last_error", "tce_bmm_f16t", "tce_rope_half", "tce_softmax_half", "tce_attention_decode_f16", "tce_attention_decode_workspace_bytes", "tce_attention_decode_describe", "tce_attention_decode_step_f16", "tce_attention_decode_step_gqa_f16", "tce_attention_decode_describe_gqa", "tce_attention_decode_step_pos_f16", "tce_attention_decode_batch_workspace_bytes", "tce_attention_decode_describe_batch", "tce_attention_decode_step_batch_f16", "tce_kv_pages_pool_bytes", "tce_attention_decode_describe_paged", "tce_attention_decode_step_paged_f16", "tce_kv_pages_scatter_f16", "tce_kv_pages_gather_f16", "tce_kv_block_table_check", "tce_attention_prefill_f16", "tce_attention_prefill_workspace_bytes", "tce_attention_prefill_paged_workspace_bytes", "tce_attention_prefill_paged_f16", "tce_attention_prefill_describe_paged", "tce_kv_pages_pool_bytes_fp8", "tce_attention_decode_step_paged_fp8", "tce_attention_prefill_paged_fp8", "tce_kv_pages_scatter_fp8", "tce_kv_pages_gather_fp8", "tce_sample_workspace_bytes", "tce_sample_f16", "tce_embed_rows_f16", "tce_attention_decode_step_paged_rows_f16", "tce_attention_decode_step_paged_rows_fp8", "tce_sample_verify_workspace_bytes", "tce_sample_verify_f16", "tce_draft_ngram", "tce_opt_attention_decode", "tce_prefetch", "tce_add_half", "tce_silu_mul_half", "tce_rmsnorm_half", "tce_w4a16_forward_group_rmsnorm", "tce_w4a16_forward_group", "tce_w4a16_forward_independent", "tce_w4a16_describe_independent", "tce_w4a16_forward_independent_gather", "tce_w4a16_check_zero_point_8", "tce_w4a16_awq_fp16acc", "tce_w4a16_awq_workspace_bytes",
     "tce_w4a16_gemm_awq", "tce_w4a16_shard", "tce_comm_create", "tce_comm_export", "tce_comm_connect", "tce_comm_connect_local", "tce_allgather_f16", "tce_comm_rccl_unique_id", "tce_comm_rccl_init", "tce_allgather_rows_workspace_bytes", "tce_allgather_rows_f16", "tce_comm_status", "tce_comm_set_timeout_ms", "tce_comm_reset", "tce_comm_device", "tce_comm_destroy", "tce_w8a8_matmul", "tce_opt_softmax_q", "tce_opt_kv_append", "tce_layernorm_q", "tce_layernorm_q_w8a8_group", "tce_plan_create", "tce_plan_create_ex", "tce_plan_is_chained", "tce_plan_geometry", "tce_plan_status", "tce_plan_launch_geometry", "tce_plan_launch", "tce_plan_n_launches",
     "tce_w4a16_forward_v2", "tce_w8a8_matmul_v2", "tce_w8a8_scratch_bytes", "tce_attention_decode_step_deferred_f16", "tce_w4a16_forward_deferred_attention", "tce_plan_destroy", "tce_version", "tce_last_error", "tce_build_info", "tce_w4a16_set_gemv_config", "tce_w4a16_set_gemv_i8",
     "tce_w4a16_set_gemm_config", "tce_w4a16_algorithmic_bytes", "tce_w4a16_gemv_variant", "tce_w4a16_gemm_variant",
@@ -141,6 +141,7 @@
 
 
 _lib = None
+HAS_GROUP_COPIES = False
 
 
 def lib() -> C.CDLL:
@@ -171,6 +172,12 @@
         L.tce_w4a16_gemm_scratch_bytes.argtypes = []
         L.tce_w4a16_gemm_scratch_bytes.restype = C.c_size_t
         L.tce_w4a16_prepack.argtypes = [C.POINTER(W4A16Desc), C.c_void_p, C.c_void_p]
+        global HAS_GROUP_COPIES
+        HAS_GROUP_COPIES = hasattr(L, "tce_w4a16_prepack_group_bytes") and hasattr(L, "tce_w4a16_prepack_group")
+        if HAS_GROUP_COPIES:
+            L.tce_w4a16_prepack_group_bytes.argtypes = [C.POINTER(W4A16Desc), C.c_int]
+            L.tce_w4a16_prepack_group_bytes.restype = C.c_size_t
+            L.tce_w4a16_prepack_group.argtypes = [C.POINTER(W4A16Desc), C.c_int, C.c_void_p, C.c_void_p]
         L.tce_prefetch.argtypes = [C.c_void_p, C.c_longlong, C.c_int, C.c_void_p]
         L.tce_bmm_f16t.argtypes = [C.c_void_p, C.c_void_p, C.c_void_p, C.c_int, C.c_int, C.c_int, C.c_int, C.c_ushort, C.c_void_p]
         L.tce_rope_half.argtypes = [C.c_void_p] * 4 + [C.c_int] * 4 + [C.c_void_p]
diff --git a/tinychatengine_amd/csrc/tce_capi.hip b/tinychatengine_amd/csrc/tce_capi.hip
--- a/tinychatengine_amd/csrc/tce_capi.hip
+++ b/tinychatengine_amd/csrc/tce_capi.hip
@@ -10,6 +10,7 @@
 
 #include "tce_common.hpp"
 #include "w4a16_kernels.hpp"
+#include "w4a16_mfma_layout.hpp"
 
 namespace tce {
 int launch_w8a8(const tce_w8a8_desc &d, hipStream_t stream, hipError_t *hip_err, void *scratch = nullptr, char *describe = nullptr, int describe_len = 0);
@@ -64,6 +65,8 @@
         if (d->flags & (TCE_W4_ADD_TO_C | TCE_W4_FORCE_GEMM)) return fail(TCE_ERR_BAD_ARG, "TCE_W4_SILU_MUL_PAIRS cannot be combined with ADD_TO_C / FORCE_GEMM");
     }
     if (d->rmsnorm_gamma && (d->flags & TCE_W4_FORCE_GEMM)) return fail(TCE_ERR_BAD_ARG, "rmsnorm_gamma cannot be combined with TCE_W4_FORCE_GEMM");
+    if ((d->reserved || d->reserved2) && (!d->prepacked || !tce::pk::group_member_ok(d->N, d->reserved, d->reserved2)))
+        return fail(TCE_ERR_BAD_ARG, "group-copy fields (first tile %d, rows of the copy %d) do not describe N=%d rows of a packed copy", d->reserved, d->reserved2, d->N);
     return TCE_OK;
 }
 
@@ -696,6 +699,9 @@
         return TCE_OK;
     }
     if (g_gemv_kernel == 0 && g_debug_mode_capi == 0 && tce::gemv_i8_supports(d, 1)) {
+        if (d->reserved2 > 0)
+            std::snprintf(buf, (size_t)buf_len, "gemv-i8 rows-per-pass=%d group=%d group-copy first-tile=%d rows=%d", tce::gemv_i8_rows_per_pass(d->M, d->K, d->group_size), d->group_size, d->reserved, d->reserved2);
+        else
         std::snprintf(buf, (size_t)buf_len, "gemv-i8 rows-per-pass=%d group=%d", tce::gemv_i8_rows_per_pass(d->M, d->K, d->group_size), d->group_size);
         return TCE_OK;
     }
@@ -742,6 +748,28 @@
     const int rc = tce::launch_w4a16_prepack(*d, packed, static_cast<hipStream_t>(stream), &he);
     if (rc == TCE_ERR_HIP) return hip_fail(he, "prepack launch");
     if (rc != TCE_OK) return fail(rc, "tce_w4a16_prepack: unsupported shape");
+    return TCE_OK;
+}
+
+size_t tce_w4a16_prepack_group_bytes(const tce_w4a16_desc *descs, int count) {
+    if (!descs || count < 1 || count > TCE_MAX_GROUP) return 0;
+    return tce::prepack_group_bytes(descs, count);
+}
+
+int tce_w4a16_prepack_group(const tce_w4a16_desc *descs, int count, void *packed, void *stream) {
+    if (!descs || !packed || count < 1 || count > TCE_MAX_GROUP) return fail(TCE_ERR_BAD_ARG, "tce_w4a16_prepack_group: null argument / count not in 1..%d", TCE_MAX_GROUP);
+    for (int i = 0; i < count; ++i) {
+        const tce_w4a16_desc &d = descs[i];
+        if (!d.qweight || !d.scales || !d.zeros || d.N <= 0 || d.K <= 0) return fail(TCE_ERR_BAD_ARG, "tce_w4a16_prepack_group: null weights / non-positive N, K");
+        if (d.group_size != 128 && d.group_size != 64 && d.group_size != 32) return fail(TCE_ERR_UNSUPPORTED_GROUP, "Unsupported group size: %d", d.group_size);
+    }
+    if (tce::prepack_group_bytes(descs, count) == 0)
+        return fail(TCE_ERR_UNSUPPORTED_SHAPE, "tce_w4a16_prepack_group: the members must share K (a multiple of 128) and the group size, every N a multiple of 16: keep individual copies");
+    if (reinterpret_cast<uintptr_t>(packed) % 256 != 0) return fail(TCE_ERR_UNSUPPORTED_SHAPE, "tce_w4a16_prepack_group: the packed buffer must be 256-byte aligned");
+    hipError_t he = hipSuccess;
+    const int rc = tce::launch_w4a16_prepack_group(descs, count, packed, static_cast<hipStream_t>(stream), &he);
+    if (rc == TCE_ERR_HIP) return hip_fail(he, "prepack launch");
+    if (rc != TCE_OK) return fail(rc, "tce_w4a16_prepack_group: unsupported shape");
     return TCE_OK;
 }
 
diff --git a/tinychatengine_amd/csrc/w4a16_gemm_pk.hip b/tinychatengine_amd/csrc/w4a16_gemm_pk.hip
--- a/tinychatengine_amd/csrc/w4a16_gemm_pk.hip
+++ b/tinychatengine_amd/csrc/w4a16_gemm_pk.hip
@@ -1038,19 +1038,20 @@
     return pk::total_bytes(N, K, G);
 }
 
-int launch_w4a16_prepack(const tce_w4a16_desc &d, void *out, hipStream_t stream, hipError_t *hip_err) {
-    if (d.K % 128 != 0) return TCE_ERR_UNSUPPORTED_SHAPE;
+int launch_w4a16_prepack(const tce_w4a16_desc &d, void *out, hipStream_t stream, hipError_t *hip_err, int tile0, int rows_total) {
+    if (d.K % 128 != 0 || !pk::group_member_ok(d.N, tile0, rows_total)) return TCE_ERR_UNSUPPORTED_SHAPE;
+    const pk::PackedView pv = pk::packed_view(d.N, d.K, d.group_size, tile0, rows_total);
     const int zw = zeros_width(d.K, d.group_size);
     PrepackArgs a{};
     a.qweight = static_cast<const unsigned *>(d.qweight);
     a.scales = static_cast<const half_t *>(d.scales);
     a.zeros = static_cast<const unsigned *>(d.zeros);
     unsigned char *base = static_cast<unsigned char *>(out);
-    a.words = reinterpret_cast<unsigned *>(base);
-    a.consts = reinterpret_cast<uint2_t *>(base + pk::consts_offset(d.N, d.K));
-    a.last = reinterpret_cast<float *>(base + pk::last_offset(d.N, d.K, d.group_size));
-    a.dscales = reinterpret_cast<half_t *>(base + pk::dscales_offset(d.N, d.K, d.group_size));
-    a.dzeros = reinterpret_cast<unsigned *>(base + pk::dzeros_offset(d.N, d.K, d.group_size));
+    a.words = reinterpret_cast<unsigned *>(base + pv.words);
+    a.consts = reinterpret_cast<uint2_t *>(base + pv.consts);
+    a.last = reinterpret_cast<float *>(base + pv.last);
+    a.dscales = reinterpret_cast<half_t *>(base + pv.dscales);
+    a.dzeros = reinterpret_cast<unsigned *>(base + pv.dzeros);
     a.N = d.N;
     a.K = d.K;
     a.log2g = d.group_size == 128 ? 7 : (d.group_size == 64 ? 6 : 5);
@@ -1064,6 +1065,30 @@
     if (e != hipSuccess) {
         if (hip_err) *hip_err = e;
         return TCE_ERR_HIP;
+    }
+    return TCE_OK;
+}
+
+size_t prepack_group_bytes(const tce_w4a16_desc *descs, int count) {
+    if (!descs || count < 1) return 0;
+    long long rows = 0;
+    for (int i = 0; i < count; ++i) {
+        if (descs[i].N <= 0 || descs[i].N % 16 != 0 || descs[i].K != descs[0].K || descs[i].group_size != descs[0].group_size) return 0;
+        rows += descs[i].N;
+    }
+    if (rows >= (1LL << 31)) return 0;
+    return prepack_bytes((int)rows, descs[0].K, descs[0].group_size);
+}
+
+int launch_w4a16_prepack_group(const tce_w4a16_desc *descs, int count, void *out, hipStream_t stream, hipError_t *hip_err) {
+    if (prepack_group_bytes(descs, count) == 0) return TCE_ERR_UNSUPPORTED_SHAPE;
+    int rows = 0;
+    for (int i = 0; i < count; ++i) rows += descs[i].N;
+    int tile0 = 0;
+    for (int i = 0; i < count; ++i) {
+        const int rc = launch_w4a16_prepack(descs[i], out, stream, hip_err, tile0, rows);
+        if (rc != TCE_OK) return rc;
+        tile0 += descs[i].N / 16;
     }
     return TCE_OK;
 }
@@ -1202,8 +1227,10 @@
     PkGemmArgs g{};
     const unsigned char *base = static_cast<const unsigned char *>(packed);
     g.A = static_cast<const half_t *>(d.A);
-    g.words = reinterpret_cast<const uint4_t *>(base);
-    g.consts = reinterpret_cast<const uint2_t *>(base + pk::consts_offset(d.N, d.K));
+    if (!pk::group_member_ok(d.N, d.reserved, d.reserved2)) return TCE_ERR_UNSUPPORTED_SHAPE;
+    const pk::PackedView pv = pk::packed_view(d.N, d.K, d.group_size, d.reserved, d.reserved2);
+    g.words = reinterpret_cast<const uint4_t *>(base + pv.words);
+    g.consts = reinterpret_cast<const uint2_t *>(base + pv.consts);
     g.C = static_cast<half_t *>(d.C);
     g.M = d.M;
     g.N = d.N;
diff --git a/tinychatengine_amd/csrc/w4a16_gemv_i8.hip b/tinychatengine_amd/csrc/w4a16_gemv_i8.hip
--- a/tinychatengine_amd/csrc/w4a16_gemv_i8.hip
+++ b/tinychatengine_amd/csrc/w4a16_gemv_i8.hip
@@ -20,6 +20,7 @@
 struct I8Tail {
     I8SegRest rest[TCE_MAX_GROUP];
     I8SegHead head[TCE_MAX_GROUP - 1];
+    int mtile[TCE_MAX_GROUP];
     const float *gamma;
     float eps;
     float out_eps;
@@ -87,7 +88,7 @@
 
 template <int MB, int GPU, int ROWS, int UW, bool Z8, bool NORM, bool RNORM, int COMB, bool MIX, typename ARGS, bool STAMPS = false>
 __device__ __forceinline__ void w4a16_gemv_i8_body(const ARGS &args, unsigned char *smem, int tid, const int WK, const int U, const int K_, const int lda_, int M_, const half_t *A_,
-                                                   I8Seg seg, const int tile0, const bool gathers, const unsigned g_epoch, I8Stamps *st = nullptr) {
+                                                   I8Seg seg, const int tile0, const bool gathers, const unsigned g_epoch, I8Stamps *st = nullptr, const int nmem = 0) {
     static_assert(!MIX || (MB == 1 && GPU == 1 && ROWS == 1 && UW == 8 && !NORM && !RNORM && !COMB), "the mixed launch: one decode row, groups of 128, one tile per wave group");
     static_assert(!COMB || (MB == 1 && ROWS == 1 && GPU == 1 && UW == 8 && !NORM && !RNORM), "the deferred-attention prologue: one decode row, groups of 128, K a multiple of 1024");
     static_assert(MB * GPU <= 4, "sixteen output columns: rows x groups-per-unit x 4 planes");
@@ -315,12 +316,41 @@
     __builtin_amdgcn_wave_barrier();
     if constexpr (STAMPS) st->t[2] = __builtin_amdgcn_s_memrealtime();
 
+    half_t *mC[ROWS];
+    int mldc[ROWS], mepi[ROWS], mrow0[ROWS];
+#pragma unroll
+    for (int r = 0; r < ROWS; ++r) {
+        mC[r] = seg.C;
+        mldc[r] = seg.ldc;
+        mepi[r] = seg.epilogue;
+        mrow0[r] = 0;
+    }
+    if constexpr (!MIX) {
+        if (nmem > 0) {
+#pragma unroll
+            for (int r = 0; r < ROWS; ++r) {
+                int mi = 0;
+#pragma unroll
+                for (int i = 1; i < TCE_MAX_GROUP; ++i) mi = (i < nmem && tile0 + r >= args.mtile[i]) ? i : mi;
+                mC[r] = args.rest[mi].C;
+                mldc[r] = args.rest[mi].ldc;
+                mepi[r] = args.rest[mi].epilogue;
+                mrow0[r] = args.mtile[mi] * 16;
+            }
+        }
+    }
+    auto of_tile = [&](auto *v, int r) {
+        auto x = v[0];
+#pragma unroll
+        for (int r2 = 1; r2 < ROWS; ++r2) x = r == r2 ? v[r2] : x;
+        return x;
+    };
     half_t c_old = (half_t)0.0f;
     if constexpr (!RNORM) {
-        if (wk == 0 && (seg.epilogue & TCE_W4_ADD_TO_C) && tid < ROWS * MB * 16) {
+        if (wk == 0 && tid < ROWS * MB * 16) {
             const int i16 = tid & 15, m = (tid >> 4) % MB, r = tid / (16 * MB);
             const int row = (tile0 + r) * 16 + i16;
-            if (m0 + m < M_ && row < seg.N) c_old = seg.C[(size_t)(m0 + m) * seg.ldc + row];
+            if ((of_tile(mepi, r) & TCE_W4_ADD_TO_C) && m0 + m < M_ && row < seg.N) c_old = of_tile(mC, r)[(size_t)(m0 + m) * of_tile(mldc, r) + (row - of_tile(mrow0, r))];
         }
     }
 
@@ -428,9 +458,13 @@
             if constexpr (MB == 1) v = dpp_add_f32<0x124>(v);
             if (p_l == 0 && (j >> 2) < MB) red[((wk * ROWS + r) * MB + m_l) * 16 + kq * 4 + q] = v;
         }
-    keep_scalar(seg.C);
-    keep_scalar(seg.ldc);
-    keep_scalar(seg.epilogue);
+#pragma unroll
+    for (int r = 0; r < ROWS; ++r) {
+        keep_scalar(mC[r]);
+        keep_scalar(mldc[r]);
+        keep_scalar(mepi[r]);
+        keep_scalar(mrow0[r]);
+    }
     keep_scalar(seg.N);
     keep_scalar(M_);
     float *ws_ = nullptr, *out_gamma_ = nullptr;
@@ -463,18 +497,19 @@
         half_t hnew = (half_t)0.0f;
         (void)hnew;
         if (m0 + m < M_ && row < seg.N) {
-            half_t *crow = seg.C + (size_t)(m0 + m) * seg.ldc;
-            if (seg.epilogue & TCE_W4_SILU_MUL_PAIRS) {
-                if ((i16 & 1) == 0) crow[row >> 1] = silu_mul_half(y, y_other);
-            } else if (seg.epilogue & TCE_W4_ADD_TO_C) {
-                if constexpr (RNORM) hnew = crow[row] + y;
-                else crow[row] = c_old + y;
+            const int epi = of_tile(mepi, r), mrow = row - of_tile(mrow0, r);
+            half_t *crow = of_tile(mC, r) + (size_t)(m0 + m) * of_tile(mldc, r);
+            if (epi & TCE_W4_SILU_MUL_PAIRS) {
+                if ((i16 & 1) == 0) crow[mrow >> 1] = silu_mul_half(y, y_other);
+            } else if (epi & TCE_W4_ADD_TO_C) {
+                if constexpr (RNORM) hnew = crow[mrow] + y;
+                else crow[mrow] = c_old + y;
             } else {
-                crow[row] = y;
+                crow[mrow] = y;
             }
             if constexpr (MIX) {
                 if (gathers) {
-                    const half_t outv = (seg.epilogue & TCE_W4_ADD_TO_C) ? (half_t)(c_old + y) : y;
+                    const half_t outv = (epi & TCE_W4_ADD_TO_C) ? (half_t)(c_old + y) : y;
                     const size_t off = ((size_t)args.g.slot * 2 + (g_epoch & 1u)) * args.g.vec_bytes + ((size_t)args.g.rank * args.g.slice_elems + (size_t)row) * 2;
 #pragma unroll
                     for (int p = 0; p < kCommMaxRanks; ++p)
@@ -612,7 +647,7 @@
         st.t[5] = __builtin_amdgcn_s_memtime();
         __builtin_amdgcn_sched_barrier(0);
     }
-    const int WK = geom & 0xFF, nseg = geom >> 8;
+    const int WK = geom & 0xFF, nseg = (geom >> 8) & 0xFF, nmem = geom >> 16;
     int si = 0, block_begin = 0;
     if (nseg > 1) {
         static_assert(TCE_MAX_GROUP == 4, "the batch below names three further linears");
@@ -634,7 +669,7 @@
     }
     const I8SegRest &r = t.rest[si];
     const I8Seg seg{words, dscales, r.dzeros, r.C, N, r.ldc, r.epilogue, bytes_w, bytes_s, r.bytes_z, block_begin};
-    w4a16_gemv_i8_body<MB, GPU, ROWS, UW, Z8, NORM, RNORM, COMB, false, I8Tail, STAMPS>(t, smem_wg, (int)threadIdx.x, WK, U, K, lda, M, A, seg, ((int)blockIdx.x - block_begin) * ROWS, false, 0u, &st);
+    w4a16_gemv_i8_body<MB, GPU, ROWS, UW, Z8, NORM, RNORM, COMB, false, I8Tail, STAMPS>(t, smem_wg, (int)threadIdx.x, WK, U, K, lda, M, A, seg, ((int)blockIdx.x - block_begin) * ROWS, false, 0u, &st, nmem);
 }
 
 template <bool Z8>
@@ -673,7 +708,7 @@
 struct I8Launch {
     const void *words;
     const half_t *dscales, *A;
-    int bytes_w, bytes_s, U, lda, K, N, M, nseg;
+    int bytes_w, bytes_s, U, lda, K, N, M, nseg, nmem;
     I8Tail t;
 };
 
@@ -685,7 +720,7 @@
         const hipError_t e = hipFuncSetAttribute(reinterpret_cast<const void *>(kfn), hipFuncAttributeMaxDynamicSharedMemorySize, (int)lds);
         if (e != hipSuccess) return e;
     }
-    hipLaunchKernelGGL(kfn, dim3(blocks, m_blocks, 1), dim3(64 * wk, 1, 1), lds, stream, a.words, a.bytes_w, a.U, static_cast<const void *>(a.A), a.lda, a.K, static_cast<const void *>(a.dscales), a.bytes_s, a.N, a.M, wk | (a.nseg << 8), a.t);
+    hipLaunchKernelGGL(kfn, dim3(blocks, m_blocks, 1), dim3(64 * wk, 1, 1), lds, stream, a.words, a.bytes_w, a.U, static_cast<const void *>(a.A), a.lda, a.K, static_cast<const void *>(a.dscales), a.bytes_s, a.N, a.M, wk | (a.nseg << 8) | (a.nmem << 16), a.t);
     return hipGetLastError();
 }
 
@@ -718,11 +753,24 @@
     if (uw == 0 || (uw == 16 && (d0.M > 1 || d0.group_size != 128))) return false;
     for (int i = 0; i < count; ++i) {
         const tce_w4a16_desc &d = descs[i];
-        if (!d.prepacked || (reinterpret_cast<uintptr_t>(d.prepacked) & 255)) return false;
+        if (!d.prepacked || (reinterpret_cast<uintptr_t>(d.prepacked) & 255) || !pk::group_member_ok(d.N, d.reserved, d.reserved2)) return false;
         if ((long long)pk::nt16(d.N) * (d.K / 2) * 16 >= (1LL << 31)) return false;
         if (d.flags & TCE_W4_FORCE_GEMM) return false;
     }
     return true;
+}
+
+int gemv_i8_group_copy_members(const tce_w4a16_desc *descs, int count) {
+    if (count < 2 || count > TCE_MAX_GROUP || descs[0].reserved2 <= 0) return 0;
+    long long tiles = 0;
+    for (int i = 0; i < count; ++i) {
+        const tce_w4a16_desc &d = descs[i];
+        if (d.prepacked != descs[0].prepacked || d.reserved2 != descs[0].reserved2 || !pk::group_member_ok(d.N, d.reserved, d.reserved2)) return 0;
+        if (i > 0 && d.reserved != descs[i - 1].reserved + descs[i - 1].N / 16) return 0;
+        tiles += d.N / 16;
+    }
+    if (tiles * (descs[0].K / 2) * 16 >= (1LL << 31)) return 0;
+    return count;
 }
 
 int launch_w4a16_gemv_i8(const tce_w4a16_desc *descs, int count, hipStream_t stream, hipError_t *hip_err, const float *gamma, float eps, const I8ResidualNorm *rn,
@@ -757,13 +805,15 @@
     const long long resident = 256LL * (20 / wk);
     if (gamma && two_ok && total_tiles > resident && total_tiles * 5 <= resident * 6) rows = 2;
     if (g_i8_rows && two_ok) rows = g_i8_rows;
+    const bool shared = gemv_i8_group_copy_members(descs, count) > 0;
     int blocks = 0;
     for (int i = 0; i < count; ++i) {
         const tce_w4a16_desc &d = descs[i];
         const unsigned char *base = static_cast<const unsigned char *>(d.prepacked);
+        const pk::PackedView pv = pk::packed_view(d.N, d.K, d.group_size, d.reserved, d.reserved2);
         I8SegHead h{};
-        h.words = base;
-        h.dscales = reinterpret_cast<const half_t *>(base + pk::dscales_offset(d.N, d.K, d.group_size));
+        h.words = base + pv.words;
+        h.dscales = reinterpret_cast<const half_t *>(base + pv.dscales);
         h.bytes_w = (int)pk::words_bytes(d.N, d.K);
         h.bytes_s = (int)pk::dscales_bytes(d.N, d.K, d.group_size);
         h.N = d.N;
@@ -779,7 +829,7 @@
         }
         I8SegRest &r = a.t.rest[i];
         r.C = static_cast<half_t *>(d.C);
-        r.dzeros = reinterpret_cast<const unsigned *>(base + pk::dzeros_offset(d.N, d.K, d.group_size));
+        r.dzeros = reinterpret_cast<const unsigned *>(base + pv.dzeros);
         r.epilogue = d.flags & (TCE_W4_SILU_MUL_PAIRS | TCE_W4_ADD_TO_C);
         r.ldc = d.ldc ? d.ldc : ((r.epilogue & TCE_W4_SILU_MUL_PAIRS) ? d.N / 2 : d.N);
         r.bytes_z = (int)pk::dzeros_bytes(d.N, d.K, d.group_size);
@@ -788,6 +838,17 @@
     for (int i = count; i < TCE_MAX_GROUP; ++i) {
         a.t.rest[i] = a.t.rest[0];
         a.t.head[i - 1] = I8SegHead{a.words, a.dscales, a.bytes_w, a.bytes_s, a.N, 0};
+    }
+    if (shared) {
+        const int rows_all = (int)total_tiles * 16;
+        a.nseg = 1;
+        a.nmem = count;
+        a.N = rows_all;
+        a.bytes_w = (int)pk::words_bytes(rows_all, d0.K);
+        a.bytes_s = (int)pk::dscales_bytes(rows_all, d0.K, d0.group_size);
+        a.t.rest[0].bytes_z = (int)pk::dzeros_bytes(rows_all, d0.K, d0.group_size);
+        for (int i = 0; i < TCE_MAX_GROUP; ++i) a.t.mtile[i] = i < count ? descs[i].reserved - d0.reserved : 0;
+        blocks = (int)((total_tiles + rows - 1) / rows);
     }
     hipError_t e = hipErrorInvalidConfiguration;
     if (rn) {
@@ -874,7 +935,7 @@
     for (int i = 0; i < count; ++i) {
         const tce_w4a16_desc &d = descs[i];
         if (d.M != 1 || d.group_size != 128 || d.K % 128 != 0 || d.K > 16384 || d.rmsnorm_gamma) return false;
-        if (!d.prepacked || (reinterpret_cast<uintptr_t>(d.prepacked) & 255)) return false;
+        if (!d.prepacked || (reinterpret_cast<uintptr_t>(d.prepacked) & 255) || !pk::group_member_ok(d.N, d.reserved, d.reserved2)) return false;
         if ((long long)pk::nt16(d.N) * (d.K / 2) * 16 >= (1LL << 31)) return false;
         if (d.flags & TCE_W4_FORCE_GEMM) return false;
     }
@@ -964,9 +1025,10 @@
         m.K = d.K;
         I8Seg &s = m.seg;
         const unsigned char *base = static_cast<const unsigned char *>(d.prepacked);
-        s.words = base;
-        s.dscales = reinterpret_cast<const half_t *>(base + pk::dscales_offset(d.N, d.K, d.group_size));
-        s.dzeros = reinterpret_cast<const unsigned *>(base + pk::dzeros_offset(d.N, d.K, d.group_size));
+        const pk::PackedView pv = pk::packed_view(d.N, d.K, d.group_size, d.reserved, d.reserved2);
+        s.words = base + pv.words;
+        s.dscales = reinterpret_cast<const half_t *>(base + pv.dscales);
+        s.dzeros = reinterpret_cast<const unsigned *>(base + pv.dzeros);
         s.C = static_cast<half_t *>(d.C);
         s.N = d.N;
         s.epilogue = d.flags & (TCE_W4_SILU_MUL_PAIRS | TCE_W4_ADD_TO_C);
diff --git a/tinychatengine_amd/csrc/w4a16_gemv_i8_token.hip b/tinychatengine_amd/csrc/w4a16_gemv_i8_token.hip
--- a/tinychatengine_amd/csrc/w4a16_gemv_i8_token.hip
+++ b/tinychatengine_amd/csrc/w4a16_gemv_i8_token.hip
@@ -453,13 +453,15 @@
         for (int i = 0; i < groups[l] && ok; ++i) {
             const tce_w4a16_desc &d = descs[off + i];
             ok = d.M == 1 && d.K == d0.K && d.group_size == 128 && d.A == d0.A && d.prepacked && !(reinterpret_cast<uintptr_t>(d.prepacked) & 255) && (d.flags & TCE_W4_ZERO_POINT_IS_8) &&
-                 !(d.flags & TCE_W4_FORCE_GEMM) && !d.rmsnorm_gamma && (long long)pk::nt16(d.N) * (d.K / 2) * 16 < (1LL << 31) && !(d.flags & ~(TCE_W4_ZERO_POINT_IS_8 | TCE_W4_SILU_MUL_PAIRS | TCE_W4_ADD_TO_C));
+                 !(d.flags & TCE_W4_FORCE_GEMM) && !d.rmsnorm_gamma && (long long)pk::nt16(d.N) * (d.K / 2) * 16 < (1LL << 31) && !(d.flags & ~(TCE_W4_ZERO_POINT_IS_8 | TCE_W4_SILU_MUL_PAIRS | TCE_W4_ADD_TO_C)) &&
+                 pk::group_member_ok(d.N, d.reserved, d.reserved2);
             if ((d.flags & TCE_W4_SILU_MUL_PAIRS) && (d.N % 2 != 0 || (d.flags & TCE_W4_ADD_TO_C))) ok = false;
             if (!ok) break;
             TokSeg &sg = st.seg[i];
             const unsigned char *base = static_cast<const unsigned char *>(d.prepacked);
-            sg.words = base;
-            sg.dscales = reinterpret_cast<const half_t *>(base + pk::dscales_offset(d.N, d.K, d.group_size));
+            const pk::PackedView pv = pk::packed_view(d.N, d.K, d.group_size, d.reserved, d.reserved2);
+            sg.words = base + pv.words;
+            sg.dscales = reinterpret_cast<const half_t *>(base + pv.dscales);
             sg.C = static_cast<half_t *>(d.C);
             sg.C_tag = nullptr;
             sg.N = d.N;
diff --git a/tinychatengine_amd/csrc/w4a16_kernels.hpp b/tinychatengine_amd/csrc/w4a16_kernels.hpp
--- a/tinychatengine_amd/csrc/w4a16_kernels.hpp
+++ b/tinychatengine_amd/csrc/w4a16_kernels.hpp
@@ -92,6 +92,7 @@
                       int forced_depth, hipStream_t stream, hipError_t *hip_err, const float *gamma = nullptr, float eps = 0.f);
 
 bool gemv_i8_supports(const tce_w4a16_desc *descs, int count, bool with_norm = false);
+int gemv_i8_group_copy_members(const tce_w4a16_desc *descs, int count);
 int gemv_i8_rows_per_pass(int M, int K, int group_size);
 void set_gemv_i8_mode(int mode, int rows);
 struct I8ResidualNorm {
@@ -140,7 +141,9 @@
 int launch_w4a16_gemm(const tce_w4a16_desc &d, int forced_mt, int forced_nt, hipStream_t stream, hipError_t *hip_err);
 
 size_t prepack_bytes(int N, int K, int G);
-int launch_w4a16_prepack(const tce_w4a16_desc &d, void *out, hipStream_t stream, hipError_t *hip_err);
+int launch_w4a16_prepack(const tce_w4a16_desc &d, void *out, hipStream_t stream, hipError_t *hip_err, int tile0 = 0, int rows_total = 0);
+size_t prepack_group_bytes(const tce_w4a16_desc *descs, int count);
+int launch_w4a16_prepack_group(const tce_w4a16_desc *descs, int count, void *out, hipStream_t stream, hipError_t *hip_err);
 int launch_w4a16_gemm_pk(const tce_w4a16_desc &d, const void *packed, hipStream_t stream, hipError_t *hip_err);
 void set_gemm_pk256_auto(int on);
 void set_gemm_pk_wide_auto(int on);
diff --git a/tinychatengine_amd/csrc/w4a16_mfma_layout.hpp b/tinychatengine_amd/csrc/w4a16_mfma_layout.hpp
--- a/tinychatengine_amd/csrc/w4a16_mfma_layout.hpp
+++ b/tinychatengine_amd/csrc/w4a16_mfma_layout.hpp
@@ -28,6 +28,25 @@
 TCE_HD size_t dzeros_offset(int N, int K, int G) { return dscales_offset(N, K, G) + align256(dscales_bytes(N, K, G)); }
 TCE_HD size_t total_bytes(int N, int K, int G) { return dzeros_offset(N, K, G) + align256(dzeros_bytes(N, K, G)); }
 
+struct PackedView {
+    size_t words, consts, last, dscales, dzeros;
+};
+TCE_HD bool group_member_ok(int N, int tile0, int rows_total) {
+    if (rows_total == 0) return tile0 == 0;
+    return N > 0 && N % 16 == 0 && rows_total % 16 == 0 && tile0 >= 0 && (long long)tile0 * 16 + N <= rows_total;
+}
+TCE_HD PackedView packed_view(int N, int K, int G, int tile0, int rows_total) {
+    const int NT = rows_total > 0 ? rows_total : N;
+    const size_t t = rows_total > 0 ? (size_t)tile0 : 0;
+    PackedView v;
+    v.words = t * (K / 128) * 1024;
+    v.consts = consts_offset(NT, K) + t * (K / G) * 128;
+    v.last = last_offset(NT, K, G) + t * 64;
+    v.dscales = dscales_offset(NT, K, G) + t * (K / G) * 32;
+    v.dzeros = dzeros_offset(NT, K, G) + t * (K / G) * 8;
+    return v;
+}
+
 TCE_HD size_t word_index(int n, int k, int K) {
     const int jt = n >> 4, n16 = n & 15, kb = k >> 7, kk = k & 127;
     const int s = kk >> 5, q = (kk >> 3) & 3;
diff --git a/tinychatengine_amd/decode.py b/tinychatengine_amd/decode.py
--- a/tinychatengine_amd/decode.py
+++ b/tinychatengine_amd/decode.py
@@ -72,6 +72,9 @@
         self.lm_head = mk(shape.vocab, h, 999_983)
         self.prepacked = bool(prepack)
         if prepack:
+            for b in self.blocks:
+                Linear_half_int4.prepack_group(b["qkv"])
+                Linear_half_int4.prepack_group([b["gate"], b["up"]])
             for l in self.all_linears():
                 l.prepack()
         gx = torch.Generator(device=self.device).manual_seed(4321)
diff --git a/tinychatengine_amd/linear.py b/tinychatengine_amd/linear.py
--- a/tinychatengine_amd/linear.py
+++ b/tinychatengine_amd/linear.py
@@ -27,6 +27,7 @@
             raise ValueError("scales/zeros do not have the padded q4_6 shapes (quantize_methods.py:431-440)")
         self.zeros_are_8 = bool((zeros == -2004318072).all().item())
         self.packed = None
+        self.group_tile0, self.group_rows = 0, 0
         self._op = MatmulOperator()
 
     def prepack(self) -> "Linear_half_int4":
@@ -41,6 +42,30 @@
                                    scales=_ptr(self.scale), zeros=_ptr(self.zero_point))
                 capi.check(capi.lib().tce_w4a16_prepack(d, self.packed.data_ptr(), _stream()))
         return self
+
+    @staticmethod
+    def prepack_group(linears: list["Linear_half_int4"]) -> bool:
+        import ctypes as C
+        descs = [capi.W4A16Desc(M=1, N=l.out_features, K=l.in_features, group_size=l.group_size, qweight=_ptr(l.weight), scales=_ptr(l.scale), zeros=_ptr(l.zero_point))
+                 for l in linears]
+        arr = (capi.W4A16Desc * len(descs))(*descs)
+        need = 0
+        L = capi.lib()
+        if capi.HAS_GROUP_COPIES and len(linears) > 1 and all(l.packed is None for l in linears):
+            need = int(L.tce_w4a16_prepack_group_bytes(arr, len(descs)))
+        if not need:
+            for l in linears:
+                l.prepack()
+            return False
+        buf = torch.empty(need + 256, dtype=torch.uint8, device=linears[0].weight.device)
+        off = (-buf.data_ptr()) % 256
+        packed = buf[off:off + need]
+        capi.check(capi.lib().tce_w4a16_prepack_group(arr, len(descs), packed.data_ptr(), _stream()))
+        rows, tile0 = sum(l.out_features for l in linears), 0
+        for l in linears:
+            l._packed_storage, l.packed, l.group_tile0, l.group_rows = buf, packed, tile0, rows
+            tile0 += l.out_features // 16
+        return True
 
     @classmethod
     def from_float(cls, w: torch.Tensor, group_size: int = quantize.QK4_6):
@@ -73,6 +98,7 @@
         return capi.W4A16Desc(M=m, N=self.out_features, K=self.in_features, group_size=self.group_size, A=x.data_ptr(),
                               qweight=self.weight.data_ptr(), scales=self.scale.data_ptr(), zeros=self.zero_point.data_ptr(),
                               C=out.data_ptr(), ldc=ldc, flags=flags | (capi.TCE_W4_ZERO_POINT_IS_8 if self.zeros_are_8 else 0),
+                              reserved=self.group_tile0 if self.packed is not None else 0, reserved2=self.group_rows if self.packed is not None else 0,
                               rmsnorm_gamma=gamma.data_ptr() if gamma is not None else None, rmsnorm_eps=float(eps),
                               prepacked=self.packed.data_ptr() if self.packed is not None else None,
                               scratch=gemm_scratch(self.weight.device).data_ptr() if self.packed is not None and m > 128 else None)
```

Measured after the change: 1095 tokens/s, median of 6. 1.5% higher.
